# angeladai/sgnn

Measured on AMD Instinct MI355X. Metric: TSDF blocks/sec fwd+bwd (64^3@5% occ, bs32), higher is better.
Workload: dtype f32

## Files before the change

include/sgnn_hip.h:

```cpp
#ifndef SGNN_HIP_H
#define SGNN_HIP_H

#include <stdint.h>

#ifdef __cplusplus
extern "C" {
#endif

#define SGNN_OK 0
#define SGNN_EINVAL (-1)
#define SGNN_EHIP (-2)
#define SGNN_EOVERFLOW (-3)
#define SGNN_ENOWS (-4)

#define SGNN_STATUS_COORD_RANGE 1
#define SGNN_STATUS_DUPLICATE 2
#define SGNN_STATUS_OVERFLOW 4

typedef void *sgnn_stream_t;

const char *sgnn_last_error(void);
int sgnn_version(void);
const char *sgnn_arch(void);


int64_t sgnn_hash_capacity(int64_t n);

int sgnn_coords_from_i64(const int64_t *locs, int64_t n, int32_t *coords, int32_t *status,
                         const int64_t *n_dev, sgnn_stream_t stream);
int sgnn_coords_to_i64(const int32_t *coords, int64_t n, int64_t *locs, const int64_t *n_dev,
                       sgnn_stream_t stream);

int sgnn_hash_build(const int32_t *coords, int64_t n, uint64_t *keys, int32_t *vals, int64_t cap,
                    int32_t *status, const int64_t *n_dev, sgnn_stream_t stream);

int sgnn_hash_lookup(const uint64_t *keys, const int32_t *vals, int64_t cap, const int32_t *query,
                     int64_t m, int32_t *rows, const int64_t *m_dev, sgnn_stream_t stream);

#define SGNN_TUNE_UNKNOWN INT64_MIN
typedef struct sgnn_tune {
  int64_t conv_small;
  int64_t conv_small_rows;
  int64_t conv_unrolled;
  int64_t conv_one_round;
  int64_t conv_wide_epi;
  int64_t conv_dw_blocks;
  int64_t conv_dw_c1;
  int64_t rulebook_multi;
  int64_t scan_inline;
  int64_t chain_merged;
  int64_t prog_fusion;
  int64_t prog_lin_bn;
  int64_t prog_lin_add;
  int64_t bn_fuse;
} sgnn_tune;
int64_t sgnn_tune_set(const char *name, int64_t value);
int64_t sgnn_tune_get(const char *name);
const char *sgnn_tune_names(void);
const sgnn_tune *sgnn_tune_current(void);


int sgnn_rulebook_subm3(const uint64_t *keys, const int32_t *vals, int64_t cap,
                        const int32_t *coords, int64_t n, int32_t *nbr, int64_t ld,
                        const int64_t *n_dev, sgnn_stream_t stream);

#define SGNN_RULEBOOK_MULTI_MAX 4
int sgnn_rulebook_subm3_multi(int count, const uint64_t *const *keys, const int32_t *const *vals, const int64_t *caps,
                              const int32_t *const *coords, const int64_t *ns, int32_t *const *nbrs, const int64_t *lds,
                              const int64_t *const *n_devs, sgnn_stream_t stream);

int sgnn_rulebook_subm3_dense(const uint64_t *keys, const int32_t *vals, int64_t cap, const int32_t *coords, int64_t n,
                              int dim_z, int dim_y, int dim_x, int32_t *volume, int64_t volume_entries, int32_t *nbr,
                              int64_t ld, const int64_t *n_dev, sgnn_stream_t stream);
int sgnn_rulebook_subm3_volume(const int32_t *coords, int64_t n, int dim_z, int dim_y, int dim_x, int32_t *volume,
                               int64_t volume_entries, int32_t *nbr, int64_t ld, const int64_t *n_dev, int32_t *status,
                               sgnn_stream_t stream);

int64_t sgnn_down2_ws_bytes(int64_t nf);
int sgnn_rulebook_down2(const int32_t *fine_coords, int64_t nf, uint64_t *ckeys, int32_t *cvals,
                        int64_t ccap, int32_t *parent, int32_t *coarse_coords, int64_t *n_coarse,
                        void *ws, int64_t ws_bytes, sgnn_stream_t stream);
int sgnn_down2_tables(const int32_t *fine_coords, const int32_t *parent, int64_t nf,
                      int32_t *children, int64_t ldc, int64_t nc, int32_t *ptable, int64_t ldf,
                      const int64_t *nf_dev, const int64_t *nc_dev, sgnn_stream_t stream);

int64_t sgnn_down2_chain_ws_bytes(int64_t cap);
int sgnn_down2_chain(const int32_t *fine_coords, int64_t n0, const int64_t *n0_dev, int64_t cap, int depth,
                     void *const *ckeys, void *const *cvals, int64_t ccap, void *const *parent,
                     void *const *coarse_coords, int64_t *counts_dev, const int64_t *level_caps, int32_t *status,
                     void *ws, int64_t ws_bytes, sgnn_stream_t stream);

int64_t sgnn_down2_chain_tables_ws_bytes(int64_t cap, int depth);
int sgnn_down2_chain_tables(const int32_t *fine_coords, const int64_t *n0_dev, int64_t cap, int depth,
                            void *const *ckeys, void *const *cvals, int64_t ccap, void *const *parent,
                            void *const *coarse_coords, int64_t *counts_dev, const int64_t *level_caps,
                            void *const *children, void *const *ptable, int32_t *status, void *ws, int64_t ws_bytes,
                            sgnn_stream_t stream);

#define SGNN_CONV_TRANSPOSE_W 1
#define SGNN_CONV_FLIP_K 2
int sgnn_conv_fwd(const float *x, int64_t n_in, int cin, const float *w, int K, const int32_t *table,
                  int64_t ld, int64_t n_out, int cout, float *y, int flags, int in_shift,
                  sgnn_stream_t stream);

int sgnn_conv_fwd_ex(const float *x, int64_t n_in, int cin, const float *w, int K, const int32_t *table,
                     int64_t ld, int64_t n_out, int cout, float *y, int flags, int in_shift,
                     const int32_t *kmap, const int32_t *kadd, int in_mul, int groups, int table_rows,
                     sgnn_stream_t stream);
int sgnn_conv_bwd_weight_ex(const float *x, int64_t n_in, int cin, const float *dy, int cout,
                            const int32_t *table, int64_t ld, int K, int64_t n_out, float *dw, int in_shift,
                            const int32_t *kmap, const int32_t *kadd, int in_mul, int groups, int table_rows,
                            void *ws, int64_t ws_bytes, sgnn_stream_t stream);

int64_t sgnn_conv_stats_blocks(int64_t n_out);
int sgnn_conv_fwd_epi(const float *x, int64_t n_in, int cin, int64_t ldx, const float *w, int K,
                      const int32_t *table, int64_t ld, int64_t n_out, int cout, float *y, int64_t ldy, int flags,
                      const float *addend, int64_t ld_add, int stats, double *partial, const float *bn_x,
                      int64_t ld_bnx, const float *mean, const float *invstd, const float *gamma, const float *beta,
                      float leak, sgnn_stream_t stream);

int64_t sgnn_conv_bwd_weight_ws_bytes(int64_t n_out, int K, int cin, int cout);
int sgnn_conv_bwd_weight(const float *x, int64_t n_in, int cin, const float *dy, int cout,
                         const int32_t *table, int64_t ld, int K, int64_t n_out, float *dw, int in_shift, void *ws,
                         int64_t ws_bytes, sgnn_stream_t stream);

int sgnn_expand_weights(const float *w, int cin, int cout, float *wc, sgnn_stream_t stream);
int sgnn_expand_weights_bwd(const float *dwc, int cin, int cout, float *dw, sgnn_stream_t stream);

int64_t sgnn_bn_ws_bytes(int64_t n, int c);
int sgnn_bn_fwd(const float *x, int64_t n, int c, const float *gamma, const float *beta,
                float *running_mean, float *running_var, float eps, float momentum, int training,
                float leak, float *save_mean, float *save_invstd, float *y, void *ws,
                int64_t ws_bytes, sgnn_stream_t stream);
int sgnn_bn_bwd(const float *x, const float *dy, int64_t n, int c, const float *gamma,
                const float *beta, const float *save_mean, const float *save_invstd, int training,
                float leak, float *dx, float *dgamma, float *dbeta, void *ws, int64_t ws_bytes,
                sgnn_stream_t stream);
int sgnn_bn_bwd_add(const float *x, const float *dy, int64_t n, int c, const float *gamma, const float *beta,
                    const float *save_mean, const float *save_invstd, int training, float leak,
                    const float *addend, float *dx, float *dgamma, float *dbeta, void *ws, int64_t ws_bytes,
                    sgnn_stream_t stream);

int sgnn_bn_fwd_ex(const float *x, int64_t ldx, int64_t n, int c, const float *gamma, const float *beta,
                   float *running_mean, float *running_var, float eps, float momentum, int training, float leak,
                   float *save_mean, float *save_invstd, float *y, int64_t ldy, const double *pre_partial,
                   int64_t pre_nblk, void *ws, int64_t ws_bytes, sgnn_stream_t stream);
int sgnn_bn_bwd_ex(const float *x, int64_t ldx, const float *dy, int64_t ld_dy, int64_t n, int c, const float *gamma,
                   const float *beta, const float *save_mean, const float *save_invstd, int training, float leak,
                   const float *addend, int64_t ld_add, float *dx, int64_t ld_dx, float *dgamma, float *dbeta,
                   const double *pre_partial, int64_t pre_nblk, void *ws, int64_t ws_bytes, sgnn_stream_t stream);

int sgnn_copy_multi(void *const *dst, const void *const *src, const int64_t *bytes, int nregions, sgnn_stream_t stream);

int sgnn_gather_rows(const float *src, int c, const int32_t *idx, int64_t m, float *dst,
                     sgnn_stream_t stream);
int sgnn_gather_rows_dn(const float *src, int c, const int32_t *idx, const int64_t *m_dev, int64_t m_cap,
                        float *dst, sgnn_stream_t stream);
int sgnn_concat3_rows(const float *a, int ca, const int32_t *ia, const float *b, int cb, const int32_t *ib,
                      const float *c, int cc, const int32_t *ic, int64_t m, float *dst, sgnn_stream_t stream);
int sgnn_concat3_rows_bwd(const float *ddst, int ca, const int32_t *ia, int cb, const int32_t *ib, int cc,
                          const int32_t *ic, int64_t m, float *da, int64_t na, float *db, int64_t nb, float *dc,
                          int64_t nc, sgnn_stream_t stream);
int sgnn_scatter_rows(const float *src, int c, const int32_t *idx, int64_t m, float *dst,
                      int64_t n_dst, const int64_t *m_dev, sgnn_stream_t stream);
int sgnn_gather_sum(const float *src, int c, const int32_t *table, int64_t ld, int K,
                    int64_t n_out, float *dst, sgnn_stream_t stream);
int sgnn_repeat_rows(const float *src, int c, int64_t n, int rep, float *dst, sgnn_stream_t stream);
int sgnn_sum_groups(const float *src, int c, int64_t n, int rep, float *dst, sgnn_stream_t stream);
int sgnn_concat_rows(const float *a, int ca, const int32_t *ia, const float *b, int cb,
                     const int32_t *ib, int64_t m, float *dst, sgnn_stream_t stream);
int sgnn_concat_rows_bwd(const float *ddst, int ca, const int32_t *ia, int cb, const int32_t *ib,
                         int64_t m, float *da, int64_t na, float *db, int64_t nb,
                         sgnn_stream_t stream);
int sgnn_add(const float *a, const float *b, int64_t count, float *y, sgnn_stream_t stream);

int sgnn_expand8_coords(const int32_t *coords, int64_t n, int32_t *out, const int64_t *n_dev, sgnn_stream_t stream);
int sgnn_expand8_coords_i64(const int32_t *coords, int64_t n, int32_t *out, int64_t *locs, const int64_t *n_dev,
                            sgnn_stream_t stream);
int sgnn_dense_coords(int batch, int d0, int d1, int d2, int32_t *out, sgnn_stream_t stream);
int64_t sgnn_compact_ws_bytes(int64_t n);
int sgnn_compact_sigmoid(const float *logits, int64_t stride, int64_t n, int32_t *sel,
                         int64_t *count, void *ws, int64_t ws_bytes, sgnn_stream_t stream);
int sgnn_compact_dense(const int32_t *coords, int64_t n, const float *vol, int batch, int d0, int d1, int d2,
                       int32_t *sel, int64_t *count, void *ws, int64_t ws_bytes, sgnn_stream_t stream);
int sgnn_compact_mask(const uint8_t *mask, int64_t n, int32_t *sel, int64_t *count, void *ws,
                      int64_t ws_bytes, sgnn_stream_t stream);
int sgnn_compact_sigmoid_cap(const float *logits, int64_t stride, int64_t n, const int64_t *n_dev, int32_t *sel,
                             int64_t *count2, int64_t keep_cap, int32_t *status, void *ws, int64_t ws_bytes,
                             sgnn_stream_t stream);
int sgnn_compact_dense_cap(const int32_t *coords, int64_t n, const int64_t *n_dev, const float *vol, int batch, int d0,
                           int d1, int d2, int32_t *sel, int64_t *count2, int64_t keep_cap, int32_t *status, void *ws,
                           int64_t ws_bytes, sgnn_stream_t stream);
int sgnn_compact_sigmoid_cap_locs(const float *logits, int64_t stride, int64_t n, const int64_t *n_dev,
                                  const int32_t *coords, int32_t *sel, int32_t *locs, int64_t *count2, int64_t keep_cap,
                                  int32_t *status, void *ws, int64_t ws_bytes, sgnn_stream_t stream);
int sgnn_compact_dense_cap_locs(const int32_t *coords, int64_t n, const int64_t *n_dev, const float *vol, int batch, int d0,
                                int d1, int d2, int32_t *sel, int32_t *locs, int64_t *count2, int64_t keep_cap,
                                int32_t *status, void *ws, int64_t ws_bytes, sgnn_stream_t stream);

int sgnn_sparse_to_dense(const float *feats, const int32_t *coords, int64_t n, int c, float *dense,
                         int batch, int d0, int d1, int d2, sgnn_stream_t stream);
int sgnn_dense_to_sparse(const float *dense, const int32_t *coords, int64_t n, int c, float *feats,
                         int batch, int d0, int d1, int d2, sgnn_stream_t stream);

int64_t sgnn_linear_ws_bytes(int64_t n, int cin, int cout);
int sgnn_linear_fwd(const float *x, int64_t n, int cin, const float *w, const float *bias, int cout,
                    float *y, sgnn_stream_t stream);
int sgnn_linear_bwd(const float *x, const float *dy, int64_t n, int cin, const float *w, int cout,
                    float *dx, float *dw, float *dbias, void *ws, int64_t ws_bytes,
                    sgnn_stream_t stream);

int64_t sgnn_loss_ws_bytes(void);
int sgnn_loss_level_fwd(const int64_t *locs, const float *vals, int vstride, int occ_col, int sdf_col,
                        const float *tgt_occ, const float *tgt_sdf, const float *weights,
                        const uint8_t *known, int d0, int d1, int d2, int64_t m, int use_log,
                        int mask_mode, const int64_t *m_dev, double *sums, float *out2, void *ws, int64_t ws_bytes,
                        sgnn_stream_t stream);
int sgnn_loss_level_bwd(const int64_t *locs, const float *vals, int vstride, int occ_col, int sdf_col,
                        const float *tgt_occ, const float *tgt_sdf, const float *weights,
                        const uint8_t *known, int d0, int d1, int d2, int64_t m, int use_log,
                        int mask_mode, const int64_t *m_dev, const double *sums, const float *gout2, float *dvals,
                        sgnn_stream_t stream);

int sgnn_loss_targets(const float *sdf, const uint8_t *known, const int64_t *input_locs, int64_t n_locs,
                      const int64_t *n_locs_dev, int batch,
                      int d0, int d1, int d2, float trunc, int masking, float weight_missing_geo, int ncoarse,
                      void *const *hier_in, float *tsdf, float *hier_last, float *occ_last, float *w_last,
                      void *const *occ, void *const *w, void *const *hier, sgnn_stream_t stream);
int sgnn_loss_combine(const float *out2s, const float *coef_host, int n, float *total, float *cur,
                      sgnn_stream_t stream);
int sgnn_loss_combine_bwd(const float *g, const float *coef_host, int n, float *g2, sgnn_stream_t stream);
int64_t sgnn_loss_multi_ws_bytes(void);
int sgnn_loss_levels_fwd(const int64_t *levels, int n, const float *coef_host, double *sums, float *out2s, float *total,
                         float *cur, void *ws, int64_t ws_bytes, sgnn_stream_t stream);
int sgnn_loss_levels_bwd(const int64_t *levels, int n, const float *coef_host, const double *sums, const float *g,
                         void *const *dvals, sgnn_stream_t stream);

int64_t sgnn_prog_arena_floats(const int32_t *ops, int nops, const int32_t *bufs, int nbuf, int n_ext,
                               const int64_t *lev_n, int nlev, const int32_t *keep, int mode);
int64_t sgnn_prog_ws_bytes(const int32_t *ops, int nops, const int64_t *lev_n, int nlev);
int64_t sgnn_prog_buffer_offset(const int32_t *ops, int nops, const int32_t *bufs, int nbuf, int n_ext,
                                const int64_t *lev_n, int nlev, const int32_t *keep, int infer, int b);
int sgnn_prog_plan(const int32_t *ops, int nops, const int32_t *bufs, int nbuf, int n_ext, const int64_t *lev_n,
                   int nlev, const int32_t *keep, int mode, int32_t *out);
int sgnn_prog_forward(const int32_t *ops, const float *opf, int nops, const int32_t *bufs, int nbuf, int n_ext,
                      const int64_t *lev_n, const int64_t *lev_ld, void *const *lev_nbr,
                      void *const *lev_children, void *const *lev_ptable, void *const *lev_parent,
                      void *const *lev_cnt, int nlev, void *const *params, int nparams,
                      void *const *ext, void *const *idx, int nidx,
                      float *arena, int64_t arena_floats, const int32_t *keep, int training, void *wait_event,
                      void *ws, int64_t ws_bytes, sgnn_stream_t stream);
int sgnn_prog_backward(const int32_t *ops, const float *opf, int nops, const int32_t *bufs, int nbuf, int n_ext,
                       const int64_t *lev_n, const int64_t *lev_ld, void *const *lev_nbr,
                       void *const *lev_children, void *const *lev_ptable, void *const *lev_parent,
                       void *const *lev_cnt, int nlev, void *const *params, void *const *pgrads,
                       int nparams, void *const *ext,
                       void *const *gext, void *const *idx, int nidx, const float *arena, float *garena,
                       int64_t arena_floats, void *const *gout, const int32_t *keep, int training, void *ws,
                       int64_t ws_bytes, sgnn_stream_t stream);

int sgnn_prog_set_side_stream(sgnn_stream_t stream2, void *ws2, int64_t ws2_bytes);
int sgnn_prog_defer_join(int on);
int64_t sgnn_bf16_conv_ws_bytes(int cin, int cout, int K, int expand);
int sgnn_bf16_conv_fwd(const void *x, int64_t n_in, int cin, int64_t ldx, const float *w, int K, const int32_t *table,
                       int64_t ld, int64_t n_out, int cout, void *y, int64_t ldy, const void *addend, int64_t ld_add,
                       const int64_t *n_dev, void *ws, int64_t ws_bytes, sgnn_stream_t stream);
int sgnn_bf16_conv_expand(const void *x, int64_t n, int cin, int64_t ldx, const float *w, const int32_t *nbr, int64_t ld,
                          int cout, void *y, int64_t ldy, const int64_t *n_dev, void *ws, int64_t ws_bytes,
                          sgnn_stream_t stream);
int sgnn_bf16_bn_eval(const void *x, int64_t ldx, int64_t n, int c, const float *gamma, const float *beta,
                      const float *running_mean, const float *running_var, float eps, float leak, void *y, int64_t ldy,
                      const int64_t *n_dev, sgnn_stream_t stream);
int sgnn_bf16_gather_rows(const void *x, int64_t ldx, int c, const int32_t *idx, int64_t m, void *y, int64_t ldy,
                          const int64_t *n_dev, sgnn_stream_t stream);
int sgnn_bf16_add(const void *a, int64_t lda, const void *b, int64_t ldb, int64_t n, int c, void *y, int64_t ldy,
                  const int64_t *n_dev, sgnn_stream_t stream);
int sgnn_bf16_join(const void *a, int64_t lda, int ca, const void *b, int64_t ldb, int cb, int64_t n, void *y, int64_t ldy,
                   const int64_t *n_dev, sgnn_stream_t stream);
int sgnn_bf16_concat3(const float *a, int ca, const int32_t *ia, const float *b, int cb, const int32_t *ib, const float *c,
                      int cc, const int32_t *ic, int64_t m, void *y, int64_t ldy, const int64_t *n_dev, sgnn_stream_t stream);
int sgnn_bf16_linear(const void *x, int64_t ldx, int64_t n, int cin, const float *w, const float *bias, int cout, float *y,
                     const int64_t *n_dev, sgnn_stream_t stream);
int sgnn_bf16_to_f32(const void *x, int64_t ldx, int64_t n, int c, float *y, const int64_t *n_dev, sgnn_stream_t stream);
int sgnn_adam_flat(float *params, const float *grads, float *exp_avg, float *exp_avg_sq, int64_t n, const int64_t *seg,
                   int nseg, const float *lr_dev, float beta1, float beta2, float eps, float weight_decay,
                   float grad_scale, const int32_t *status, sgnn_stream_t stream);
int sgnn_seg_flags(const int64_t *cnt_ptrs, int nseg, float *flags, const int32_t *status, sgnn_stream_t stream);
int sgnn_status_merge(const float *overflow_flag, int32_t *status, sgnn_stream_t stream);

int sgnn_io_layout(const void *bytes, int64_t nbytes, int kind, int64_t *out);
int sgnn_io_flag_entries(const uint32_t *locs_xyz, const float *vals, const float *voxelsize,
                         const int64_t *seg, int nb, int64_t n, float truncation, int64_t max_z,
                         uint8_t *mask, sgnn_stream_t stream);
int sgnn_io_emit_entries(const uint32_t *locs_xyz, const float *vals, const float *voxelsize,
                         const int64_t *seg, int nb, const int32_t *sel, const int64_t *count,
                         int64_t n_max, int64_t *out_locs, float *out_feats, sgnn_stream_t stream);
int sgnn_io_scatter_dense(const uint32_t *locs_xyz, const float *vals, const float *voxelsize,
                          const int64_t *seg, int nb, int64_t n, int d0, int d1, int d2, int64_t max_z,
                          float *dense, sgnn_stream_t stream);

typedef struct sgnn_fuse_frame {
  float m[12];
  float intr[4];
  int32_t box[6];
  int64_t offset;
} sgnn_fuse_frame;
int sgnn_fuse_depth_raw(const uint16_t *raw, int nframes, int h_raw, int w_raw, int h, int w, float depth_shift,
                        float min_depth, float max_depth, float *out, sgnn_stream_t stream);
int sgnn_fuse_bilateral(const float *in, int nframes, int h, int w, float sigma_d, float sigma_r, float *out,
                        sgnn_stream_t stream);
int sgnn_fuse_integrate(float *sdf, uint8_t *weight, int32_t *free_ctr, int dx, int dy, int dz, const float *depth,
                        int h, int w, const sgnn_fuse_frame *frames, int nframes, int chunk, float voxel_size,
                        float depth_min, float depth_max, const float *obb, sgnn_stream_t stream);
int sgnn_fuse_flag(const float *sdf, int dx, int dy, int dz, float keep_abs, float truncation, float voxel_size,
                   int64_t max_z, uint8_t *mask, sgnn_stream_t stream);
int sgnn_fuse_emit_block(const float *sdf, int dx, int dy, const int32_t *sel, const int64_t *count, int64_t n_max,
                         uint32_t *locs_xyz, float *vals, sgnn_stream_t stream);
int sgnn_fuse_emit_rows(const float *sdf, int dx, int dy, float voxel_size, const int32_t *sel, const int64_t *count,
                        int64_t n_max, int64_t *locs, float *feats, sgnn_stream_t stream);
int sgnn_fuse_known(const float *sdf, int64_t n, float voxel_size, uint8_t *known, sgnn_stream_t stream);

int sgnn_chunk_score(const float *sdf_target, const float *sdf_input, int dx, int dy, int dz, float voxel_size,
                     float truncation, float keep_abs, int cz, int cy, int cx, int sz, int sy, int sx, int nwz, int nwy,
                     int nwx, int32_t *bricks, int32_t *table, sgnn_stream_t stream);
int sgnn_chunk_flag(const float *sdf, int dx, int dy, int dz, const int32_t *origins, int nb, int cz, int cy, int cx,
                    float keep_abs, float truncation, float voxel_size, uint8_t *mask, sgnn_stream_t stream);
int sgnn_chunk_emit_rows(const float *sdf, int dx, int dy, int dz, const int32_t *origins, int nb, int cz, int cy,
                         int cx, float voxel_size, const int32_t *sel, const int64_t *count, int64_t n_max,
                         int64_t *locs, float *feats, sgnn_stream_t stream);
int sgnn_chunk_crop(const float *sdf, int dx, int dy, int dz, const int32_t *origins, int nb, int cz, int cy, int cx,
                    int shift, float keep_abs, float voxel_size, float *out, uint8_t *known, sgnn_stream_t stream);

typedef struct sgnn_render_frame {
  float m[12];
  float intr[4];
} sgnn_render_frame;
int sgnn_render_depth(const float *verts, int nverts, const int32_t *faces, int ntri, const sgnn_render_frame *frames,
                      int nframes, int chunk, int h, int w, float z_clip, float depth_min, float depth_max,
                      int wave_pixels, float *out, int32_t *status, int64_t *counters, sgnn_stream_t stream);

int sgnn_meshdist_pack(const float *verts, int nverts, const int32_t *faces, int ntri, float *records, float *boxes,
                       uint8_t *usable, int32_t *status, sgnn_stream_t stream);
int sgnn_meshdist_count(const float *boxes, int ntri, float lox, float loy, float loz, float cell, int nx, int ny,
                        int nz, int32_t *counts, sgnn_stream_t stream);
int sgnn_meshdist_fill(const float *boxes, int ntri, float lox, float loy, float loz, float cell, int nx, int ny,
                       int nz, const int32_t *offsets, int32_t *cursor, int32_t *refs, sgnn_stream_t stream);
int sgnn_meshdist_query(const float *points, int64_t npts, const float *records, const int32_t *offsets,
                        const int32_t *refs, float lox, float loy, float loz, float hix, float hiy, float hiz,
                        float cell, int nx, int ny, int nz, float max_dist, float *dist, int32_t *face,
                        int64_t *counters, sgnn_stream_t stream);
int sgnn_mesh_sample(const float *records, const double *cum, int ntri, int last_usable, int64_t n, int64_t seed,
                     float *pts, int32_t *fid, sgnn_stream_t stream);

int sgnn_iou_counts(const int64_t *locs, const uint8_t *keep, const float *logits, int64_t lstride, int64_t m,
                    const void *tgt, int tgt_is_u8, int nb, int d0, int d1, int d2, int use_mask,
                    int64_t *counters, sgnn_stream_t stream);
int64_t sgnn_l1_tgtsurf_ws_bytes(void);
// ... 42 lines not shown
```

sgnn_amd/csrc/bn.hip:

```cpp
#include "common.h"

#define BN_MAX_BLOCKS 2048
#define BN_FLUSH 2
#ifndef BN_U
#define BN_U 2
#endif
#define BN_FUSE_BLOCKS 4096
#define BN_FUSE_MAXC 64

struct BnGeom {
  int vec;
  int cq;
  int rpb;
};

static BnGeom bn_geom(int c) {
  BnGeom g;
  g.vec = (c % 4 == 0) ? 4 : 1;
  g.cq = c / g.vec;
  g.rpb = 256 / g.cq;
  if (g.rpb < 1) g.rpb = 1;
  return g;
}

static BnGeom bn_geom_scalar(int c) {
  BnGeom g;
  g.vec = 1;
  g.cq = c;
  g.rpb = 256 / c;
  if (g.rpb < 1) g.rpb = 1;
  return g;
}

static int bn_blocks(int64_t n, const BnGeom &g) {
  int64_t b = (n + (int64_t)g.rpb * BN_FLUSH - 1) / ((int64_t)g.rpb * BN_FLUSH);
  if (b < 1) b = 1;
  if (b > BN_MAX_BLOCKS) b = BN_MAX_BLOCKS;
  return (int)b;
}

SGNN_EXPORT int64_t sgnn_bn_ws_bytes(int64_t n, int c) {
  (void)n;
  return (int64_t)BN_MAX_BLOCKS * 2 * c * (int64_t)sizeof(double) + 4 * (int64_t)c * sizeof(float) + 256;
}

template <int VEC>
__device__ __forceinline__ void load_vec(const float *p, float (&v)[VEC]) {
  if constexpr (VEC == 4) {
    const float4 t = *reinterpret_cast<const float4 *>(p);
    v[0] = t.x; v[1] = t.y; v[2] = t.z; v[3] = t.w;
  } else {
    v[0] = *p;
  }
}
template <int VEC>
__device__ __forceinline__ void store_vec(float *p, const float (&v)[VEC]) {
  if constexpr (VEC == 4) {
    *reinterpret_cast<float4 *>(p) = make_float4(v[0], v[1], v[2], v[3]);
  } else {
    *p = v[0];
  }
}

template <int VEC, int MODE, bool LIN = false>
__global__ __launch_bounds__(256) void k_bn_partial(const float *__restrict__ x, int64_t ldx,
                                                   const float *__restrict__ dy, int64_t ld_dy, int64_t n, int c,
                                                   int cq, int rpb, const float *__restrict__ mean,
                                                   const float *__restrict__ invstd,
                                                   const float *__restrict__ gamma,
                                                   const float *__restrict__ beta, float leak,
                                                   double *__restrict__ partial, const int64_t *n_dev, BnLin lin) {
  extern __shared__ double sh[];
  const int tid = threadIdx.x;
  unsigned nblk = gridDim.x;
  if (n_dev) {
    n = sgnn_dyn_n(n, n_dev);
    int64_t b = (n + (int64_t)rpb * BN_FLUSH - 1) / ((int64_t)rpb * BN_FLUSH);
    if (b < 1) b = 1;
    if (b > BN_MAX_BLOCKS) b = BN_MAX_BLOCKS;
    if (b < (int64_t)nblk) nblk = (unsigned)b;
    if (blockIdx.x >= nblk) {
      for (int o = tid; o < 2 * c; o += 256) partial[(size_t)blockIdx.x * 2 * c + o] = 0.0;
      return;
    }
  }
  const int col = tid % cq, rloc = tid / cq;
  const bool active = rloc < rpb;
  double sa[VEC], sb[VEC];
#pragma unroll
  for (int v = 0; v < VEC; ++v) sa[v] = sb[v] = 0.0;
  float m_[VEC], is_[VEC], g_[VEC], b_[VEC];
  float lw[2][VEC];
  if constexpr (LIN) {
#pragma unroll
    for (int o = 0; o < 2; ++o)
#pragma unroll
      for (int v = 0; v < VEC; ++v) lw[o][v] = (active && o < lin.nout) ? lin.w[o][col * VEC + v] : 0.f;
  }
  if (MODE == 1 && active) {
#pragma unroll
    for (int v = 0; v < VEC; ++v) {
      m_[v] = mean[col * VEC + v];
      is_[v] = invstd[col * VEC + v];
      g_[v] = gamma ? gamma[col * VEC + v] : 1.f;
      b_[v] = beta ? beta[col * VEC + v] : 0.f;
    }
  }
  if (active) {
    const int64_t step = (int64_t)nblk * rpb;
    int64_t row = (int64_t)blockIdx.x * rpb + rloc;
    while (row < n) {
      float fa[VEC], fb[VEC];
#pragma unroll
      for (int v = 0; v < VEC; ++v) fa[v] = fb[v] = 0.f;
      float xv[BN_FLUSH][VEC], dv[BN_FLUSH][VEC];
      bool keep[BN_FLUSH];
#pragma unroll
      for (int it = 0; it < BN_FLUSH; ++it) {
        const int64_t rr = row + it * step;
        keep[it] = rr < n;
        const int64_t rc = rr < n ? rr : row;
        load_vec<VEC>(x + rc * ldx + col * VEC, xv[it]);
        if constexpr (LIN) {
#pragma unroll
          for (int v = 0; v < VEC; ++v) dv[it][v] = 0.f;
#pragma unroll
          for (int o = 0; o < 2; ++o)
            if (o < lin.nout) {
              const float gv = lin.g[rc * lin.ldg + o];
#pragma unroll
              for (int v = 0; v < VEC; ++v) dv[it][v] = fmaf(gv, lw[o][v], dv[it][v]);
            }
        } else if (MODE == 1) {
          load_vec<VEC>(dy + rc * ld_dy + col * VEC, dv[it]);
        }
      }
#pragma unroll
      for (int it = 0; it < BN_FLUSH; ++it) {
        if (MODE == 0) {
#pragma unroll
          for (int v = 0; v < VEC; ++v) {
            const float xm = keep[it] ? xv[it][v] : 0.f;
            fa[v] += xm;
            fb[v] = fmaf(xm, xm, fb[v]);
          }
        } else {
#pragma unroll
          for (int v = 0; v < VEC; ++v) {
            const float xh = (xv[it][v] - m_[v]) * is_[v];
            const float yv = fmaf(xh, g_[v], b_[v]);
            const float dz = keep[it] ? (yv > 0.f ? dv[it][v] : dv[it][v] * leak) : 0.f;
            fa[v] += dz;
            fb[v] = fmaf(dz, xh, fb[v]);
          }
        }
      }
      row += (int64_t)BN_FLUSH * step;
#pragma unroll
      for (int v = 0; v < VEC; ++v) {
        sa[v] += (double)fa[v];
        sb[v] += (double)fb[v];
      }
    }
  }
  double *mine = sh + ((size_t)rloc * cq + col) * 2 * VEC;
  if (active) {
#pragma unroll
    for (int v = 0; v < VEC; ++v) {
      mine[v] = sa[v];
      mine[VEC + v] = sb[v];
    }
  }
  __syncthreads();
  const int outs = cq * VEC * 2;
  for (int o = tid; o < outs; o += 256) {
    const int which = o / (cq * VEC);
    const int ch = o % (cq * VEC);
    const int cg = ch / VEC, v = ch % VEC;
    double s = 0.0;
    for (int rr = 0; rr < rpb; ++rr) s += sh[((size_t)rr * cq + cg) * 2 * VEC + which * VEC + v];
    partial[((size_t)blockIdx.x * 2 + which) * c + ch] = s;
  }
}

__device__ __forceinline__ void bn_reduce_channel(const double *__restrict__ partial, int nblk, int c, int ch,
                                                  double *sh, double &s, double &s2) {
  double a = 0.0, b = 0.0;
  for (int blk = threadIdx.x; blk < nblk; blk += 8 * 256) {
    double va[8], vb[8];
#pragma unroll
    for (int u = 0; u < 8; ++u) {
      const int bi = blk + u * 256;
      const bool ok = bi < nblk;
      va[u] = ok ? partial[((size_t)bi * 2 + 0) * c + ch] : 0.0;
      vb[u] = ok ? partial[((size_t)bi * 2 + 1) * c + ch] : 0.0;
    }
#pragma unroll
    for (int u = 0; u < 8; ++u) {
      a += va[u];
      b += vb[u];
    }
  }
  sh[threadIdx.x] = a;
  sh[256 + threadIdx.x] = b;
  __syncthreads();
  for (int d = 128; d > 0; d >>= 1) {
    if (threadIdx.x < d) {
      sh[threadIdx.x] += sh[threadIdx.x + d];
      sh[256 + threadIdx.x] += sh[256 + threadIdx.x + d];
    }
    __syncthreads();
  }
  s = sh[0];
  s2 = sh[256];
}

__global__ __launch_bounds__(256) void k_bn_finalize_fwd(const double *__restrict__ partial, int nblk,
                                                        int64_t n, int c, float eps, float momentum,
                                                        float *__restrict__ running_mean,
                                                        float *__restrict__ running_var,
                                                        float *__restrict__ save_mean,
                                                        float *__restrict__ save_invstd, const int64_t *n_dev) {
  __shared__ double sh[512];
  n = sgnn_dyn_n(n, n_dev);
  const int ch = blockIdx.x;
  double s, s2;
  bn_reduce_channel(partial, nblk, c, ch, sh, s, s2);
  if (threadIdx.x == 0) {
    if (n <= 0) {
      save_mean[ch] = 0.f;
      save_invstd[ch] = 0.f;
      return;
    }
    const double mean = s / (double)n;
    double var = s2 / (double)n - mean * mean;
    if (var < 0.0) var = 0.0;
    save_mean[ch] = (float)mean;
    save_invstd[ch] = (float)(1.0 / sqrt(var + (double)eps));
    if (running_mean) running_mean[ch] = momentum * running_mean[ch] + (1.f - momentum) * (float)mean;
    if (running_var) {
      const double unb = var * ((double)n / (double)(n > 1 ? n - 1 : 1));
      running_var[ch] = momentum * running_var[ch] + (1.f - momentum) * (float)unb;
    }
  }
}

__global__ __launch_bounds__(256) void k_bn_eval_stats(const float *__restrict__ running_mean,
                                                      const float *__restrict__ running_var, int c, float eps,
                                                      float *__restrict__ save_mean,
                                                      float *__restrict__ save_invstd) {
  for (int ch = threadIdx.x; ch < c; ch += 256) {
    save_mean[ch] = running_mean[ch];
    save_invstd[ch] = 1.0f / sqrtf(running_var[ch] + eps);
  }
}


struct BnFuse {
  const double *partial;
  int nblk;
  float eps, momentum;
  float *running_mean, *running_var, *save_mean, *save_invstd;
  float *dgamma, *dbeta;
};

#ifndef BN_TOTALS_WIDE
#define BN_TOTALS_WIDE 1
#endif
typedef double f64x2 __attribute__((ext_vector_type(2)));
__device__ __forceinline__ void bn_fuse_totals(const BnFuse &f, int c, double *scratch, double *tot) {
  const int tid = threadIdx.x;
  const int tpc = 256 / c;
  if (BN_TOTALS_WIDE && (c & 1) == 0 && (((uintptr_t)f.partial) & 15) == 0) {
    const int hp = c >> 1;
    const int p2 = tid % hp, which = (tid / hp) & 1, part = tid / c;
    f64x2 acc = {0.0, 0.0};
    if (part < tpc) {
      constexpr int U = 32;
      for (int blk = part; blk < f.nblk; blk += U * tpc) {
        f64x2 v[U];
#pragma unroll
        for (int u = 0; u < U; ++u) {
          const int bi = blk + u * tpc;
          v[u] = bi < f.nblk ? *reinterpret_cast<const f64x2 *>(f.partial + ((size_t)bi * 2 + which) * c + 2 * p2) : f64x2{0.0, 0.0};
        }
#pragma unroll
        for (int u = 0; u < U; ++u) acc += v[u];
      }
      scratch[which * 256 + part * c + 2 * p2] = acc[0];
      scratch[which * 256 + part * c + 2 * p2 + 1] = acc[1];
    }
  } else {
    const int ch = tid % c, part = tid / c;
    double a = 0.0, b = 0.0;
    if (part < tpc) {
      for (int blk = part; blk < f.nblk; blk += 8 * tpc) {
        double va[8], vb[8];
#pragma unroll
        for (int u = 0; u < 8; ++u) {
          const int bi = blk + u * tpc;
          const bool ok = bi < f.nblk;
          va[u] = ok ? f.partial[((size_t)bi * 2 + 0) * c + ch] : 0.0;
          vb[u] = ok ? f.partial[((size_t)bi * 2 + 1) * c + ch] : 0.0;
        }
#pragma unroll
        for (int u = 0; u < 8; ++u) {
          a += va[u];
          b += vb[u];
        }
      }
      scratch[part * c + ch] = a;
      scratch[256 + part * c + ch] = b;
    }
  }
  __syncthreads();
  if (tid < c) {
    double s1 = 0.0, s2 = 0.0;
    for (int p = 0; p < tpc; ++p) {
      s1 += scratch[p * c + tid];
      s2 += scratch[256 + p * c + tid];
    }
    tot[tid] = s1;
    tot[c + tid] = s2;
  }
  __syncthreads();
}

template <int VEC, bool FUSE>
__global__ __launch_bounds__(256) void k_bn_apply(const float *__restrict__ x, int64_t ldx, int64_t n, int c, int cq,
                                                 int rpb, const float *__restrict__ mean,
                                                 const float *__restrict__ invstd,
                                                 const float *__restrict__ gamma,
                                                 const float *__restrict__ beta, float leak,
                                                 float *__restrict__ y, int64_t ldy, BnFuse fuse,
                                                 const int64_t *n_dev) {
  __shared__ float s_mean[BN_FUSE_MAXC], s_inv[BN_FUSE_MAXC];
  __shared__ double s_scratch[512], s_tot[2 * BN_FUSE_MAXC];
  n = sgnn_dyn_n(n, n_dev);
  if (n <= 0) return;
  if constexpr (FUSE) {
    bn_fuse_totals(fuse, c, s_scratch, s_tot);
    for (int ch = threadIdx.x; ch < c; ch += 256) {
      const double s1 = s_tot[ch], s2 = s_tot[c + ch];
      const double mu = s1 / (double)n;
      double var = s2 / (double)n - mu * mu;
      if (var < 0.0) var = 0.0;
      const float fm = (float)mu, fi = (float)(1.0 / sqrt(var + (double)fuse.eps));
      s_mean[ch] = fm;
      s_inv[ch] = fi;
      if (blockIdx.x == 0) {
        fuse.save_mean[ch] = fm;
        fuse.save_invstd[ch] = fi;
        if (fuse.running_mean) fuse.running_mean[ch] = fuse.momentum * fuse.running_mean[ch] + (1.f - fuse.momentum) * fm;
        if (fuse.running_var) {
          const double unb = var * ((double)n / (double)(n > 1 ? n - 1 : 1));
          fuse.running_var[ch] = fuse.momentum * fuse.running_var[ch] + (1.f - fuse.momentum) * (float)unb;
        }
      }
    }
    __syncthreads();
    mean = s_mean;
    invstd = s_inv;
  }
  const int tid = threadIdx.x;
  const int col = tid % cq, rloc = tid / cq;
  if (rloc >= rpb) return;
  float km[VEC], ki[VEC], kg[VEC], kb[VEC];
#pragma unroll
  for (int v = 0; v < VEC; ++v) {
    const int ch = col * VEC + v;
    km[v] = mean[ch];
    ki[v] = invstd[ch];
    kg[v] = gamma ? gamma[ch] : 1.f;
    kb[v] = beta ? beta[ch] : 0.f;
  }
  const int64_t step = (int64_t)gridDim.x * rpb;
  for (int64_t r0 = (int64_t)blockIdx.x * rpb + rloc; r0 < n; r0 += step * BN_U) {
    float xv[BN_U][VEC];
#pragma unroll
    for (int u = 0; u < BN_U; ++u) {
      const int64_t r = r0 + u * step;
      load_vec<VEC>(x + (r < n ? r : r0) * ldx + col * VEC, xv[u]);
    }
#pragma unroll
    for (int u = 0; u < BN_U; ++u) {
      const int64_t r = r0 + u * step;
      if (r >= n) break;
      float yv[VEC];
#pragma unroll
      for (int v = 0; v < VEC; ++v) yv[v] = sgnn_bn_act(xv[u][v], km[v], ki[v], kg[v], kb[v], leak);
      store_vec<VEC>(y + r * ldy + col * VEC, yv);
    }
  }
}

__global__ __launch_bounds__(256) void k_bn_finalize_bwd(const double *__restrict__ partial, int nblk,
                                                        int64_t n, int c, float *__restrict__ dgamma,
                                                        float *__restrict__ dbeta, float *__restrict__ coef,
                                                        const int64_t *n_dev) {
  __shared__ double sh[512];
  n = sgnn_dyn_n(n, n_dev);
  const int ch = blockIdx.x;
  double s, s2;
  bn_reduce_channel(partial, nblk, c, ch, sh, s, s2);
  if (threadIdx.x == 0) {
    if (dbeta) dbeta[ch] = (float)s;
    if (dgamma) dgamma[ch] = (float)s2;
    coef[ch] = n > 0 ? (float)(s / (double)n) : 0.f;
    coef[c + ch] = n > 0 ? (float)(s2 / (double)n) : 0.f;
  }
}

template <int VEC, bool LIN, bool FUSE>
__global__ __launch_bounds__(256) void k_bn_bwd_apply(const float *__restrict__ x, int64_t ldx,
                                                     const float *__restrict__ dy, int64_t ld_dy, int64_t n, int c,
                                                     int cq, int rpb, const float *__restrict__ mean,
                                                     const float *__restrict__ invstd,
                                                     const float *__restrict__ gamma,
                                                     const float *__restrict__ beta, float leak, int training,
                                                     const float *__restrict__ coef, float *dx, int64_t ld_dx,
                                                     BnFuse fuse, const float *addend, int64_t ld_add,
                                                     const int64_t *n_dev, BnLin lin) {
  __shared__ float s_coef[2 * BN_FUSE_MAXC];
  __shared__ double s_scratch[512], s_tot[2 * BN_FUSE_MAXC];
  n = sgnn_dyn_n(n, n_dev);
  if constexpr (FUSE) {
    bn_fuse_totals(fuse, c, s_scratch, s_tot);
    for (int ch = threadIdx.x; ch < c; ch += 256) {
      const double s1 = s_tot[ch], s2 = s_tot[c + ch];
      s_coef[ch] = n > 0 ? (float)(s1 / (double)n) : 0.f;
      s_coef[c + ch] = n > 0 ? (float)(s2 / (double)n) : 0.f;
      if (blockIdx.x == 0) {
        if (fuse.dbeta) fuse.dbeta[ch] = (float)s1;
        if (fuse.dgamma) fuse.dgamma[ch] = (float)s2;
      }
    }
    __syncthreads();
    coef = s_coef;
  }
  const int tid = threadIdx.x;
  const int col = tid % cq, rloc = tid / cq;
  if (rloc >= rpb) return;
  float km[VEC], ki[VEC], kg[VEC], kb[VEC], k4[VEC], k5[VEC];
#pragma unroll
  for (int v = 0; v < VEC; ++v) {
    const int ch = col * VEC + v;
    km[v] = mean[ch];
    ki[v] = invstd[ch];
    kg[v] = gamma ? gamma[ch] : 1.f;
    kb[v] = beta ? beta[ch] : 0.f;
    k4[v] = training ? coef[ch] : 0.f;
    k5[v] = training ? coef[c + ch] : 0.f;
  }
  float lw[2][VEC];
  if constexpr (LIN) {
#pragma unroll
    for (int o = 0; o < 2; ++o)
#pragma unroll
      for (int v = 0; v < VEC; ++v) lw[o][v] = o < lin.nout ? lin.w[o][col * VEC + v] : 0.f;
  }
  const int64_t step = (int64_t)gridDim.x * rpb;
  for (int64_t r0 = (int64_t)blockIdx.x * rpb + rloc; r0 < n; r0 += step * BN_U) {
    float xv[BN_U][VEC], dv[BN_U][VEC], av[BN_U][VEC];
#pragma unroll
    for (int u = 0; u < BN_U; ++u) {
      const int64_t r = r0 + u * step, rc = (r < n ? r : r0);
      load_vec<VEC>(x + rc * ldx + col * VEC, xv[u]);
      if constexpr (LIN) {
#pragma unroll
        for (int v = 0; v < VEC; ++v) dv[u][v] = 0.f;
#pragma unroll
        for (int o = 0; o < 2; ++o)
          if (o < lin.nout) {
            const float gv = lin.g[rc * lin.ldg + o];
#pragma unroll
            for (int v = 0; v < VEC; ++v) dv[u][v] = fmaf(gv, lw[o][v], dv[u][v]);
          }
      } else {
        load_vec<VEC>(dy + rc * ld_dy + col * VEC, dv[u]);
      }
      if (addend) load_vec<VEC>(addend + rc * ld_add + col * VEC, av[u]);
    }
#pragma unroll
    for (int u = 0; u < BN_U; ++u) {
      const int64_t r = r0 + u * step;
      if (r >= n) break;
      float ov[VEC];
#pragma unroll
      for (int v = 0; v < VEC; ++v) {
        const float xh = (xv[u][v] - km[v]) * ki[v];
        const float t = fmaf(xh, kg[v], kb[v]);
        const float dz = t > 0.f ? dv[u][v] : dv[u][v] * leak;
        float d = dz;
        if (training) d = dz - k4[v] - xh * k5[v];
        ov[v] = d * kg[v] * ki[v];
        if (addend) ov[v] += av[u][v];
      }
      store_vec<VEC>(dx + r * ld_dx + col * VEC, ov);
    }
  }
}

static bool bn_fuse_ok(int64_t nblk, int c, int apply_grid) {
  return c <= BN_FUSE_MAXC && nblk <= BN_FUSE_BLOCKS && nblk * (int64_t)apply_grid * 2 * c * (int64_t)sizeof(double) <= (48ll << 20);
}

static int bn_apply_grid(int64_t n, const BnGeom &g) {
  int64_t b = (n + (int64_t)g.rpb * BN_U - 1) / ((int64_t)g.rpb * BN_U);
  if (b < 1) b = 1;
  if (b > 4096) b = 4096;
  return (int)b;
}

int sgnn_bn_fwd_impl(const float *x, int64_t ldx, int64_t n, int c, const float *gamma, const float *beta,
                     float *running_mean, float *running_var, float eps, float momentum, int training, float leak,
                     float *save_mean, float *save_invstd, float *y, int64_t ldy, const double *pre_partial,
                     int64_t pre_nblk, void *ws, int64_t ws_bytes, sgnn_stream_t stream, const int64_t *n_dev) {
  hipStream_t s = (hipStream_t)stream;
  SGNN_CHECK_ARG(n >= 0 && c >= 1 && (c % 4 == 0 ? c <= 1024 : c <= 256) && save_mean && save_invstd);
  SGNN_CHECK_ARG(training || (running_mean && running_var));
  if (ldx <= 0) ldx = c;
  if (ldy <= 0) ldy = c;
  SGNN_CHECK_ARG(ldx >= c && ldy >= c);
  BnGeom g = bn_geom(c);
  if (g.vec == 4 && (ldx % 4 || ldy % 4 || ((uintptr_t)x & 15) || ((uintptr_t)y & 15))) g = bn_geom_scalar(c);
  if (g.cq > 256) {
    sgnn_set_error("sgnn_bn_fwd: %d channels need 16-byte aligned rows (row strides multiples of 4 floats)", c);
    return SGNN_EINVAL;
  }
  BnFuse fuse{nullptr, 0, 0.f, 0.f, nullptr, nullptr, nullptr, nullptr, nullptr, nullptr};
  if (training && n > 0) {
    SGNN_CHECK_ARG(x);
    const double *partial = pre_partial;
    int64_t nblk = pre_nblk;
    if (!partial) {
      if (!ws || ws_bytes < sgnn_bn_ws_bytes(n, c)) {
        sgnn_set_error("sgnn_bn_fwd: workspace too small");
        return SGNN_ENOWS;
      }
      nblk = bn_blocks(n, g);
      const size_t shbytes = (size_t)g.rpb * g.cq * 2 * g.vec * sizeof(double);
      if (g.vec == 4)
        SGNN_LAUNCH((k_bn_partial<4, 0>), dim3((unsigned)nblk), dim3(256), shbytes, s, x, ldx, nullptr, 0, n, c,
                           g.cq, g.rpb, nullptr, nullptr, nullptr, nullptr, 0.f, (double *)ws, n_dev, BnLin{});
      else
        SGNN_LAUNCH((k_bn_partial<1, 0>), dim3((unsigned)nblk), dim3(256), shbytes, s, x, ldx, nullptr, 0, n, c,
                           g.cq, g.rpb, nullptr, nullptr, nullptr, nullptr, 0.f, (double *)ws, n_dev, BnLin{});
      partial = (const double *)ws;
    }
    if (g_tune.bn_fuse && bn_fuse_ok(nblk, c, bn_apply_grid(n, g)))
      fuse = BnFuse{partial, (int)nblk, eps, momentum, running_mean, running_var, save_mean, save_invstd, nullptr, nullptr};
    else
      SGNN_LAUNCH(k_bn_finalize_fwd, dim3(c), dim3(256), 0, s, partial, (int)nblk, n, c, eps, momentum,
                         running_mean, running_var, save_mean, save_invstd, n_dev);
  } else if (training) {
    SGNN_HIP_TRY(hipMemsetAsync(save_mean, 0, c * sizeof(float), s));
    SGNN_HIP_TRY(hipMemsetAsync(save_invstd, 0, c * sizeof(float), s));
  } else {
    SGNN_LAUNCH(k_bn_eval_stats, dim3(1), dim3(256), 0, s, (const float *)running_mean,
                       (const float *)running_var, c, eps, save_mean, save_invstd);
  }
  if (n > 0) {
    SGNN_CHECK_ARG(x && y);
    const int grid = bn_apply_grid(n, g);
#define BN_APPLY(VECV, FUSEV)                                                                                 \
  SGNN_LAUNCH((k_bn_apply<VECV, FUSEV>), dim3(grid), dim3(256), 0, s, x, ldx, n, c, g.cq, g.rpb,              \
              (const float *)save_mean, (const float *)save_invstd, gamma, beta, leak, y, ldy, fuse, n_dev)
    if (g.vec == 4 && fuse.partial) BN_APPLY(4, true);
    else if (g.vec == 4) BN_APPLY(4, false);
    else if (fuse.partial) BN_APPLY(1, true);
    else BN_APPLY(1, false);
#undef BN_APPLY
  }
  SGNN_CHECK_LAUNCH();
  return SGNN_OK;
}

SGNN_EXPORT int sgnn_bn_fwd(const float *x, int64_t n, int c, const float *gamma, const float *beta,
                            float *running_mean, float *running_var, float eps, float momentum, int training,
                            float leak, float *save_mean, float *save_invstd, float *y, void *ws,
                            int64_t ws_bytes, sgnn_stream_t stream) {
  return sgnn_bn_fwd_impl(x, c, n, c, gamma, beta, running_mean, running_var, eps, momentum, training, leak, save_mean,
                          save_invstd, y, c, nullptr, 0, ws, ws_bytes, stream);
}

SGNN_EXPORT int sgnn_bn_fwd_ex(const float *x, int64_t ldx, int64_t n, int c, const float *gamma, const float *beta,
                               float *running_mean, float *running_var, float eps, float momentum, int training,
                               float leak, float *save_mean, float *save_invstd, float *y, int64_t ldy,
                               const double *pre_partial, int64_t pre_nblk, void *ws, int64_t ws_bytes,
                               sgnn_stream_t stream) {
  return sgnn_bn_fwd_impl(x, ldx, n, c, gamma, beta, running_mean, running_var, eps, momentum, training, leak,
                          save_mean, save_invstd, y, ldy, pre_partial, pre_nblk, ws, ws_bytes, stream);
}

SGNN_EXPORT int sgnn_bn_bwd(const float *x, const float *dy, int64_t n, int c, const float *gamma,
                            const float *beta, const float *save_mean, const float *save_invstd, int training,
                            float leak, float *dx, float *dgamma, float *dbeta, void *ws, int64_t ws_bytes,
                            sgnn_stream_t stream) {
  return sgnn_bn_bwd_impl(x, c, dy, c, n, c, gamma, beta, save_mean, save_invstd, training, leak, nullptr, c, dx, c,
                          dgamma, dbeta, nullptr, 0, ws, ws_bytes, stream);
}

SGNN_EXPORT int sgnn_bn_bwd_add(const float *x, const float *dy, int64_t n, int c, const float *gamma,
                                const float *beta, const float *save_mean, const float *save_invstd, int training,
                                float leak, const float *addend, float *dx, float *dgamma, float *dbeta, void *ws,
                                int64_t ws_bytes, sgnn_stream_t stream) {
  return sgnn_bn_bwd_impl(x, c, dy, c, n, c, gamma, beta, save_mean, save_invstd, training, leak, addend, c, dx, c,
                          dgamma, dbeta, nullptr, 0, ws, ws_bytes, stream);
}

SGNN_EXPORT int sgnn_bn_bwd_ex(const float *x, int64_t ldx, const float *dy, int64_t ld_dy, int64_t n, int c,
                               const float *gamma, const float *beta, const float *save_mean,
                               const float *save_invstd, int training, float leak, const float *addend,
                               int64_t ld_add, float *dx, int64_t ld_dx, float *dgamma, float *dbeta,
                               const double *pre_partial, int64_t pre_nblk, void *ws, int64_t ws_bytes,
                               sgnn_stream_t stream) {
  return sgnn_bn_bwd_impl(x, ldx, dy, ld_dy, n, c, gamma, beta, save_mean, save_invstd, training, leak, addend, ld_add,
                          dx, ld_dx, dgamma, dbeta, pre_partial, pre_nblk, ws, ws_bytes, stream);
}

int sgnn_bn_bwd_impl(const float *x, int64_t ldx, const float *dy, int64_t ld_dy, int64_t n, int c, const float *gamma,
                     const float *beta, const float *save_mean, const float *save_invstd, int training, float leak,
                     const float *addend, int64_t ld_add, float *dx, int64_t ld_dx, float *dgamma, float *dbeta,
                     const double *pre_partial, int64_t pre_nblk, void *ws, int64_t ws_bytes, sgnn_stream_t stream,
                     const int64_t *n_dev, const BnLin *lin) {
  hipStream_t s = (hipStream_t)stream;
  SGNN_CHECK_ARG(n >= 0 && c >= 1 && (c % 4 == 0 ? c <= 1024 : c <= 256) && save_mean && save_invstd);
  SGNN_CHECK_ARG(!lin || (lin->g && lin->nout >= 1 && lin->nout <= 2 && lin->w[0] && (lin->nout < 2 || lin->w[1]) && !pre_partial));
  if (n == 0) {
    if (dgamma) SGNN_HIP_TRY(hipMemsetAsync(dgamma, 0, c * sizeof(float), s));
    if (dbeta) SGNN_HIP_TRY(hipMemsetAsync(dbeta, 0, c * sizeof(float), s));
    return SGNN_OK;
  }
  SGNN_CHECK_ARG(x && (dy || lin) && dx);
  if (ldx <= 0) ldx = c;
  if (ld_dy <= 0) ld_dy = c;
  if (ld_dx <= 0) ld_dx = c;
  if (ld_add <= 0) ld_add = c;
  SGNN_CHECK_ARG(ldx >= c && ld_dy >= c && ld_dx >= c && ld_add >= c);
  if (!ws || ws_bytes < sgnn_bn_ws_bytes(n, c)) {
    sgnn_set_error("sgnn_bn_bwd: workspace too small");
    return SGNN_ENOWS;
  }
  BnGeom g = bn_geom(c);
  if (g.vec == 4 && (ldx % 4 || ld_dy % 4 || ld_dx % 4 || ld_add % 4 || ((uintptr_t)x & 15) || ((uintptr_t)dy & 15) ||
                     ((uintptr_t)dx & 15) || ((uintptr_t)addend & 15)))
    g = bn_geom_scalar(c);
  if (g.cq > 256) {
    sgnn_set_error("sgnn_bn_bwd: %d channels need 16-byte aligned rows (row strides multiples of 4 floats)", c);
    return SGNN_EINVAL;
  }
  const double *partial = pre_partial;
  int64_t nblk = pre_nblk;
  float *coef = (float *)((char *)ws + (size_t)BN_MAX_BLOCKS * 2 * c * sizeof(double));
  if (!partial) {
    nblk = bn_blocks(n, g);
    const size_t shbytes = (size_t)g.rpb * g.cq * 2 * g.vec * sizeof(double);
    if (lin && g.vec == 4)
      SGNN_LAUNCH((k_bn_partial<4, 1, true>), dim3((unsigned)nblk), dim3(256), shbytes, s, x, ldx, dy, ld_dy, n, c, g.cq,
                         g.rpb, save_mean, save_invstd, gamma, beta, leak, (double *)ws, n_dev, *lin);
    else if (lin)
      SGNN_LAUNCH((k_bn_partial<1, 1, true>), dim3((unsigned)nblk), dim3(256), shbytes, s, x, ldx, dy, ld_dy, n, c, g.cq,
                         g.rpb, save_mean, save_invstd, gamma, beta, leak, (double *)ws, n_dev, *lin);
    else if (g.vec == 4)
      SGNN_LAUNCH((k_bn_partial<4, 1>), dim3((unsigned)nblk), dim3(256), shbytes, s, x, ldx, dy, ld_dy, n, c, g.cq,
                         g.rpb, save_mean, save_invstd, gamma, beta, leak, (double *)ws, n_dev, BnLin{});
    else
      SGNN_LAUNCH((k_bn_partial<1, 1>), dim3((unsigned)nblk), dim3(256), shbytes, s, x, ldx, dy, ld_dy, n, c, g.cq,
                         g.rpb, save_mean, save_invstd, gamma, beta, leak, (double *)ws, n_dev, BnLin{});
    partial = (const double *)ws;
  }
  BnFuse fuse{nullptr, 0, 0.f, 0.f, nullptr, nullptr, nullptr, nullptr, nullptr, nullptr};
  if (g_tune.bn_fuse && bn_fuse_ok(nblk, c, bn_apply_grid(n, g)))
    fuse = BnFuse{partial, (int)nblk, 0.f, 0.f, nullptr, nullptr, nullptr, nullptr, dgamma, dbeta};
  else
    SGNN_LAUNCH(k_bn_finalize_bwd, dim3(c), dim3(256), 0, s, partial, (int)nblk, n, c, dgamma, dbeta, coef, n_dev);
  const int grid = bn_apply_grid(n, g);
#define BN_BWD_APPLY(VECV, LINV, FUSEV)                                                                                       \
  SGNN_LAUNCH((k_bn_bwd_apply<VECV, LINV, FUSEV>), dim3(grid), dim3(256), 0, s, x, ldx, dy, ld_dy, n, c, g.cq, g.rpb, save_mean, \
              save_invstd, gamma, beta, leak, training, (const float *)coef, dx, ld_dx, fuse, addend, ld_add, n_dev,              \
              LINV ? *lin : BnLin{})
  const bool fz = fuse.partial != nullptr;
  if (lin && g.vec == 4) { if (fz) BN_BWD_APPLY(4, true, true); else BN_BWD_APPLY(4, true, false); }
  else if (lin) { if (fz) BN_BWD_APPLY(1, true, true); else BN_BWD_APPLY(1, true, false); }
  else if (g.vec == 4) { if (fz) BN_BWD_APPLY(4, false, true); else BN_BWD_APPLY(4, false, false); }
  else { if (fz) BN_BWD_APPLY(1, false, true); else BN_BWD_APPLY(1, false, false); }
#undef BN_BWD_APPLY
  SGNN_CHECK_LAUNCH();
  return SGNN_OK;
}
```

sgnn_amd/csrc/common.h:

```cpp
#pragma once
#include <hip/hip_runtime.h>
#include <stdint.h>
#include <stdio.h>
#include "../../include/sgnn_hip.h"

#define SGNN_EXPORT extern "C" __attribute__((visibility("default")))

extern "C" int sgnn_stamp(const char *label, sgnn_stream_t stream);
extern sgnn_tune g_tune;

void sgnn_set_error(const char *fmt, ...);
int sgnn_prof_begin_launch(int kind, int64_t n_out, int cin, int cout, int K, int flags, hipStream_t s);
void sgnn_prof_end_launch(int slot, hipStream_t s);

__device__ __forceinline__ float sgnn_bn_act(float x, float mean, float invstd, float gamma, float beta, float leak) {
  const float xh = (x - mean) * invstd;
  const float t = fmaf(xh, gamma, beta);
  return t > 0.f ? t : t * leak;
}

struct ConvEpi {
  int64_t ldx, ldy, ld_add;
  const float *addend;
  int stats;
  double *partial;
  const float *bn_x;
  int64_t ld_bnx;
  const float *mean, *invstd, *gamma, *beta;
  float leak;
  const int64_t *n_dev;
};

int sgnn_conv_fwd_impl(const float *x, int64_t n_in, int cin, const float *w, int K, const int32_t *table, int64_t ld,
                       int64_t n_out, int cout, float *y, int flags, int in_shift, const int32_t *kmap,
                       const int32_t *kadd, int in_mul, int groups, int table_rows, const ConvEpi *epi,
                       sgnn_stream_t stream);
int64_t sgnn_conv_grid_blocks(int64_t n_out, int cin, int cout, int K);
struct BnLin {
  const float *g;
  int64_t ldg;
  const float *w[2];
  int nout;
};
int sgnn_bn_fwd_impl(const float *x, int64_t ldx, int64_t n, int c, const float *gamma, const float *beta,
                     float *running_mean, float *running_var, float eps, float momentum, int training, float leak,
                     float *save_mean, float *save_invstd, float *y, int64_t ldy, const double *pre_partial,
                     int64_t pre_nblk, void *ws, int64_t ws_bytes, sgnn_stream_t stream, const int64_t *n_dev = nullptr);
int sgnn_bn_bwd_impl(const float *x, int64_t ldx, const float *dy, int64_t ld_dy, int64_t n, int c, const float *gamma,
                     const float *beta, const float *save_mean, const float *save_invstd, int training, float leak,
                     const float *addend, int64_t ld_add, float *dx, int64_t ld_dx, float *dgamma, float *dbeta,
                     const double *pre_partial, int64_t pre_nblk, void *ws, int64_t ws_bytes, sgnn_stream_t stream,
                     const int64_t *n_dev = nullptr, const struct BnLin *lin = nullptr);
bool sgnn_conv_epi_supported(int cin, int cout);
bool dw_shape_ok(int cin, int cout);
#define DW_BATCH_MAX 28
struct DwDesc {
  const float *partial;
  float *dw;
  int64_t nblk, elems;
  int blk0;
};
struct DwBatch {
  DwDesc d[DW_BATCH_MAX];
  int n;
};
extern DwBatch *sgnn_dw_batch;
int sgnn_dw_batch_flush(DwBatch *b, hipStream_t s);
int sgnn_gather_rows_ld(const float *src, int64_t ld_src, int c, const int32_t *idx, int64_t m, float *dst,
                        int64_t ld_dst, sgnn_stream_t stream, const int64_t *n_dev = nullptr);
int sgnn_gather_sum_ld(const float *src, int64_t ld_src, int c, const int32_t *table, int64_t ld, int K, int64_t n_out,
                       float *dst, int64_t ld_dst, sgnn_stream_t stream, const int64_t *n_dev = nullptr);
int sgnn_add_ld(const float *a, int64_t lda, const float *b, int64_t ldb, int64_t n, int c, float *y, int64_t ldy,
                sgnn_stream_t stream, const int64_t *n_dev = nullptr);
int sgnn_fill32(void *p, uint32_t pattern, int64_t words, hipStream_t s);
int sgnn_fill32_multi(void *const *p, const int64_t *words, int nregions, uint32_t pattern, hipStream_t s);
int sgnn_copy_words(void *dst, const void *src, int64_t words, hipStream_t s);
int sgnn_sum_groups_dn(const float *src, int c, int64_t n, int rep, float *dst, sgnn_stream_t stream, const int64_t *n_dev);
int sgnn_concat_rows_dn(const float *a, int ca, const int32_t *ia, const float *b, int cb, const int32_t *ib, int64_t m,
                        float *dst, sgnn_stream_t stream, const int64_t *n_dev);
int sgnn_concat_rows_bwd_dn(const float *ddst, int ca, const int32_t *ia, int cb, const int32_t *ib, int64_t m, float *da,
                            int64_t na, float *db, int64_t nb, sgnn_stream_t stream, const int64_t *n_dev);
int sgnn_concat3_rows_dn(const float *a, int ca, const int32_t *ia, const float *b, int cb, const int32_t *ib,
                         const float *c, int cc, const int32_t *ic, int64_t m, float *dst, sgnn_stream_t stream,
                         const int64_t *n_dev);
int sgnn_concat3_rows_bwd_dn(const float *ddst, int ca, const int32_t *ia, int cb, const int32_t *ib, int cc,
                             const int32_t *ic, int64_t m, float *da, int64_t na, float *db, int64_t nb, float *dc,
                             int64_t nc, sgnn_stream_t stream, const int64_t *n_dev);
int sgnn_conv_bwd_weight_impl(const float *x, int64_t n_in, int cin, int64_t ldx, const float *dy, int cout, int64_t ld_dy,
                              const int32_t *table, int64_t ld, int K, int64_t n_out, float *dw, int in_shift,
                              const int32_t *kmap, const int32_t *kadd, int in_mul, int groups, int table_rows, void *ws,
                              int64_t ws_bytes, sgnn_stream_t stream, const int64_t *n_dev = nullptr);
int sgnn_expand_maps(const int32_t **S, const int32_t **ST, const int32_t **PAR);
int sgnn_linear_fwd_rows(const float *x, int64_t n, int cin, const float *const *w, const float *const *b, int cout,
                         float *y, sgnn_stream_t stream, const int64_t *n_dev = nullptr);
int sgnn_linear_bwd_rows(const float *x, const float *dy, int64_t n, int cin, const float *const *w, int cout,
                         float *dx, float *const *dw, float *const *db, void *ws, int64_t ws_bytes,
                         sgnn_stream_t stream, const int64_t *n_dev = nullptr, const float *addend = nullptr,
                         int64_t ld_add = 0);

extern long long sgnn_launch_counter;
#define SGNN_LAUNCH(...)           \
  do {                             \
    ++sgnn_launch_counter;         \
    hipLaunchKernelGGL(__VA_ARGS__); \
  } while (0)

#define SGNN_CHECK_ARG(cond)                                                    \
  do {                                                                          \
    if (!(cond)) {                                                              \
      sgnn_set_error("%s: invalid argument: %s", __func__, #cond);              \
      return SGNN_EINVAL;                                                       \
    }                                                                           \
  } while (0)

#define SGNN_CHECK_LAUNCH()                                                     \
  do {                                                                          \
    hipError_t e_ = hipGetLastError();                                          \
    if (e_ != hipSuccess) {                                                     \
      sgnn_set_error("%s: HIP error: %s", __func__, hipGetErrorString(e_));     \
      return SGNN_EHIP;                                                         \
    }                                                                           \
  } while (0)

#define SGNN_HIP_TRY(expr)                                                      \
  do {                                                                          \
    hipError_t e_ = (expr);                                                     \
    if (e_ != hipSuccess) {                                                     \
      sgnn_set_error("%s: %s failed: %s", __func__, #expr, hipGetErrorString(e_)); \
      return SGNN_EHIP;                                                         \
    }                                                                           \
  } while (0)

__device__ __forceinline__ int64_t sgnn_dyn_n(int64_t n_host, const int64_t *n_dev) {
  if (!n_dev) return n_host;
  const int64_t v = *n_dev;
  return v < n_host ? (v < 0 ? 0 : v) : n_host;
}

static inline int sgnn_grid_for(int64_t work, int block, int cap = 1 << 20) {
  int64_t g = (work + block - 1) / block;
  if (g < 1) g = 1;
  if (g > cap) g = cap;
  return (int)g;
}

__device__ __forceinline__ unsigned sgnn_xcd_tile(unsigned b, unsigned nwg) {
  const unsigned q = nwg >> 3, r = nwg & 7u, xcd = b & 7u, i = b >> 3;
  return (xcd < r ? xcd * (q + 1) : r * (q + 1) + (xcd - r) * q) + i;
}

#define SGNN_EMPTY_KEY 0xFFFFFFFFFFFFFFFFull

__device__ __forceinline__ uint64_t sgnn_pack_key(int z, int y, int x, int b) {
  return ((uint64_t)(uint32_t)b << 48) | ((uint64_t)(uint32_t)z << 32) | ((uint64_t)(uint32_t)y << 16) |
         (uint64_t)(uint32_t)x;
}

__device__ __forceinline__ uint64_t sgnn_hash64(uint64_t k) {
  k ^= k >> 33;
  k *= 0xff51afd7ed558ccdull;
  k ^= k >> 33;
  k *= 0xc4ceb9fe1a85ec53ull;
  k ^= k >> 33;
  return k;
}

__device__ __forceinline__ int32_t sgnn_hash_find(const uint64_t *__restrict__ keys,
                                                  const int32_t *__restrict__ vals, uint64_t mask,
                                                  uint64_t key) {
  uint64_t slot = sgnn_hash64(key) & mask;
  while (true) {
    uint64_t k = keys[slot];
    if (k == key) return vals[slot];
    if (k == SGNN_EMPTY_KEY) return -1;
    slot = (slot + 1) & mask;
  }
}

__device__ __forceinline__ uint8_t sgnn_known_code(float s, float vs) {
  if (s < -vs) {
    const float q = __fdiv_rn(-s, vs);
    return !(q < 2147483648.0f) ? 2 : (uint8_t)max(2, min(255, (int)q + 1));
  }
  return s <= vs ? 1 : 0;
}

__device__ __forceinline__ int sgnn_block_rank256(bool flag, int *lds4, int &total) {
  const int lane = threadIdx.x & 63, wave = threadIdx.x >> 6;
  unsigned long long bal = __ballot(flag);
  int prefix = __popcll(bal & ((1ull << lane) - 1ull));
  if (lane == 0) lds4[wave] = __popcll(bal);
  __syncthreads();
  int w0 = lds4[0], w1 = lds4[1], w2 = lds4[2], w3 = lds4[3];
  __syncthreads();
  int base = (wave > 0 ? w0 : 0) + (wave > 1 ? w1 : 0) + (wave > 2 ? w2 : 0);
  total = w0 + w1 + w2 + w3;
  return base + prefix;
}
```

sgnn_amd/csrc/conv.hip:

```cpp
#include <stdlib.h>
#include "common.h"

#include "conv_common.h"

#define CONV_SMALL_GRID ((int64_t)((g_tune.conv_small_rows + CONV_ROWS_PER_BLOCK - 1) / CONV_ROWS_PER_BLOCK))

template <int CIN, int COUT, int M, bool EX, bool WEPI>
__device__ __forceinline__ void conv_fwd_body(const float *__restrict__ x, int64_t n_in,
                                              const float *__restrict__ w, const int32_t *__restrict__ table,
                                              int64_t ld, int K, int64_t n_out, float *y, int flags,
                                              int in_shift, const ConvEx &ex, const ConvEpi &epi, int wg_cap) {
  using C = ConvCfg<CIN, COUT>;
  constexpr int V = C::V, CINP = C::CINP, NT = C::NT, KC = C::KC;
  constexpr int RPW = 16 * M;
  __shared__ __attribute__((aligned(16))) float wl[KC * C::PER_K];
  __shared__ double sred[4 * 2 * NT * 16];
  static_assert(!WEPI || (NT == 1 && M == 4 && !EX && COUT % 4 == 0), "wide epilogue: one column tile of whole 16-byte chunks");
  __shared__ float ecst[WEPI ? 64 : 1];

  const int tid = threadIdx.x, lane = tid & 63, wave = tid >> 6;
  const int r = lane & 15, q = lane >> 4;
  const unsigned groups = EX ? (unsigned)ex.groups : 1u;
  unsigned nwg = gridDim.x;
  if (epi.n_dev) n_out = sgnn_dyn_n(n_out, epi.n_dev);
  int J = 1;
  if constexpr (!EX) {
    if (wg_cap > 0) {
      const int64_t w1 = (n_out + 4 * RPW - 1) / (4 * RPW);
      J = (int)((w1 + wg_cap - 1) / wg_cap);
      if (J < 1) J = 1;
    }
  }
  if (epi.n_dev || J > 1) {
    const int64_t rows_wg = (int64_t)4 * RPW * J;
    nwg = (unsigned)((n_out + rows_wg - 1) / rows_wg) * groups;
    if (blockIdx.x >= nwg) {
      if (!EX && epi.stats)
        for (int o = tid; o < 2 * COUT; o += 256) epi.partial[(size_t)blockIdx.x * 2 * COUT + o] = 0.0;
      return;
    }
  }
  const unsigned lin = sgnn_xcd_tile(blockIdx.x, nwg);
  const unsigned tile = lin / groups, grp = lin % groups;
  int64_t row0 = ((int64_t)tile * J * 4 + wave) * RPW;
  const int32_t *kmap = nullptr, *kadd_g = nullptr;
  if constexpr (EX) {
    w += (int64_t)grp * K * CIN * COUT;
    kmap = ex.kmap ? ex.kmap + grp * K : nullptr;
    kadd_g = ex.kadd ? ex.kadd + grp * K : nullptr;
  }
  const int table_rows = EX ? ex.table_rows : K;
  const bool transpose = flags & SGNN_CONV_TRANSPOSE_W, flip = flags & SGNN_CONV_FLIP_K;

  const uint32_t ldx4 = (uint32_t)epi.ldx * 4u;
  const __amdgpu_buffer_rsrc_t rs_x = make_rsrc(x, (uint32_t)(((n_in - 1) * epi.ldx + CIN) * 4));
  const __amdgpu_buffer_rsrc_t rs_t = make_rsrc(table, (uint32_t)((int64_t)table_rows * ld * 4));
  uint32_t lane_off = (uint32_t)(row0 + (lane & (RPW - 1))) * 4u;
  const uint32_t ld4 = (uint32_t)ld * 4u;
  int perm[M];
#pragma unroll
  for (int m = 0; m < M; ++m) perm[m] = (m * 16 + r) * 4;

  f32x4 acc[M][NT];
  double s1[NT], s2[NT];
#pragma unroll
  for (int nt = 0; nt < NT; ++nt) s1[nt] = s2[nt] = 0.0;
  if constexpr (WEPI) conv_epi_wide_constants<COUT>(ecst, epi, epi.stats);

  auto load_idx = [&](int k) -> int32_t {
    if constexpr (EX) {
      const int trow = kmap ? kmap[k] : k;
      int32_t id = (int32_t)__builtin_amdgcn_raw_buffer_load_b32(rs_t, lane_off, trow * ld4, 0);
      return (id >> in_shift) * ex.in_mul + ((kadd_g && id >= 0) ? kadd_g[k] : 0);
    } else {
      return (int32_t)__builtin_amdgcn_raw_buffer_load_b32(rs_t, lane_off, k * ld4, 0) >> in_shift;
    }
  };
  auto gather = [&](int32_t iv, float(&a)[M][V]) {
#pragma unroll
    for (int m = 0; m < M; ++m) {
      const int32_t id = __builtin_amdgcn_ds_bpermute(perm[m], iv);
      buf_load_floats<V>(rs_x, (uint32_t)id * ldx4 + (uint32_t)(q * V * 4), a[m]);
    }
  };
  auto stage = [&](int k) {
    conv_stage_weights<CIN, COUT>(wl, w, K, k, (K - k) < KC ? (K - k) : KC, transpose, flip);
  };
  auto load_b = [&](int kk, float(&b)[NT][V]) {
#pragma unroll
    for (int nt = 0; nt < NT; ++nt) {
      const float *bp = wl + (kk * NT * 16 + nt * 16 + r) * CINP + q * V;
#pragma unroll
      for (int s = 0; s < V; ++s) b[nt][s] = bp[s];
    }
  };
  auto mma_b = [&](float(&a)[M][V], const float(&b)[NT][V]) {
    if constexpr (CINP != CIN) {
#pragma unroll
      for (int m = 0; m < M; ++m)
#pragma unroll
        for (int s = 0; s < V; ++s)
          if (3 * V + s >= CIN) a[m][s] = (q >= conv_first_pad_quarter<CIN, V>(s)) ? 0.f : a[m][s];
    }
#pragma unroll
    for (int s = 0; s < V; ++s)
#pragma unroll
      for (int m = 0; m < M; ++m)
#pragma unroll
        for (int nt = 0; nt < NT; ++nt)
          acc[m][nt] = __builtin_amdgcn_mfma_f32_16x16x4f32(a[m][s], b[nt][s], acc[m][nt], 0, 0, 0);
  };
  auto mma = [&](int kk, float(&a)[M][V]) {
    float b[NT][V];
    load_b(kk, b);
    mma_b(a, b);
  };

  const int klast = K - 1;
  auto idx_at = [&](int k) { return load_idx(k < klast ? k : klast); };
  for (int j = 0; j < J; ++j) {
  if (j > 0) {
    const int64_t wg_row0 = ((int64_t)tile * J + j) * 4 * RPW;
    if (wg_row0 >= n_out) break;
    row0 = wg_row0 + wave * RPW;
    lane_off = (uint32_t)(row0 + (lane & (RPW - 1))) * 4u;
  }
  const bool restage = j == 0 || K > KC;
  EpiRows<WEPI ? M : 1> erows;
#pragma unroll
  for (int m = 0; m < M; ++m)
#pragma unroll
    for (int nt = 0; nt < NT; ++nt) acc[m][nt] = f32x4{0.f, 0.f, 0.f, 0.f};
  if constexpr (V <= 4 && (NT >= 2 || M == 1)) {
    float a0[M][V], a1[M][V], a2[M][V];
    for (int k0 = 0; k0 < K; k0 += KC) {
      const int kc = (K - k0) < KC ? (K - k0) : KC;
      if (restage) stage(k0);
      gather(idx_at(k0), a0);
      gather(idx_at(k0 + 1), a1);
      int32_t iv2 = idx_at(k0 + 2), iv3 = idx_at(k0 + 3), iv4 = idx_at(k0 + 4);
      int kk = 0;
      for (; kk + 2 < kc; kk += 3) {
        gather(iv2, a2);
        iv2 = idx_at(k0 + kk + 5);
        __builtin_amdgcn_sched_barrier(0);
        mma(kk, a0);
        __builtin_amdgcn_sched_barrier(0);
        gather(iv3, a0);
        iv3 = idx_at(k0 + kk + 6);
        __builtin_amdgcn_sched_barrier(0);
        mma(kk + 1, a1);
        __builtin_amdgcn_sched_barrier(0);
        gather(iv4, a1);
        iv4 = idx_at(k0 + kk + 7);
        __builtin_amdgcn_sched_barrier(0);
        mma(kk + 2, a2);
        __builtin_amdgcn_sched_barrier(0);
      }
      if (kk < kc) mma(kk, a0);
      if (kk + 1 < kc) mma(kk + 1, a1);
    }
  } else {
    float a0[M][V], a1[M][V], b0[NT][V], b1[NT][V];
    for (int k0 = 0; k0 < (WEPI ? 1 : K); k0 += KC) {
      const int kc = (K - k0) < KC ? (K - k0) : KC;
      if (restage) stage(k0);
      int32_t iv1 = idx_at(k0 + 1), iv2 = idx_at(k0 + 2);
      gather(idx_at(k0), a0);
      load_b(0, b0);
      int kk = 0;
      for (; kk + 1 < kc; kk += 2) {
        gather(iv1, a1);
        const int32_t iv3 = idx_at(k0 + kk + 3);
        load_b(kk + 1, b1);
        __builtin_amdgcn_sched_barrier(0);
        mma_b(a0, b0);
        __builtin_amdgcn_sched_barrier(0);
        gather(iv2, a0);
        iv1 = iv3;
        iv2 = idx_at(k0 + kk + 4);
        load_b(kk + 2 < kc ? kk + 2 : kc - 1, b0);
        __builtin_amdgcn_sched_barrier(0);
        mma_b(a1, b1);
        __builtin_amdgcn_sched_barrier(0);
      }
      if constexpr (WEPI) {
        __builtin_amdgcn_sched_barrier(0);
        if constexpr (SGNN_WEPI_EARLY != 0) conv_epi_wide_prefetch<COUT, M>(erows, row0, n_out, epi, epi.stats, x, SGNN_WEPI_EARLY);
        __builtin_amdgcn_sched_barrier(0);
      }
      if (kk < kc) mma_b(a0, b0);
    }
  }

  if constexpr (WEPI)
    conv_epi_wide_finish<COUT, M>(acc, erows, row0, n_out, y, epi, epi.stats, ecst, s1, s2, x);
  else
    conv_epilogue_rows<COUT, M, NT>(acc, row0, n_out, groups, grp, y, epi, EX ? 0 : epi.stats, x, s1, s2);
  }
  conv_epilogue_stats<COUT, NT>(s1, s2, epi, EX ? 0 : epi.stats, sred, blockIdx.x);
}

template <int CIN, int COUT, int M, bool EX>
__global__ __launch_bounds__(256) void k_conv_fwd(const float *__restrict__ x, int64_t n_in,
                                                 const float *__restrict__ w, const int32_t *__restrict__ table,
                                                 int64_t ld, int K, int64_t n_out, float *y, int flags,
                                                 int in_shift, ConvEx ex, ConvEpi epi, int wg_cap) {
  conv_fwd_body<CIN, COUT, M, EX, false>(x, n_in, w, table, ld, K, n_out, y, flags, in_shift, ex, epi, wg_cap);
}

template <int CIN, int COUT>
__global__ __launch_bounds__(256) __attribute__((amdgpu_waves_per_eu(4, 8))) void k_conv_fwd_w(
    const float *__restrict__ x, int64_t n_in, const float *__restrict__ w, const int32_t *__restrict__ table, int64_t ld,
    int K, int64_t n_out, float *y, int flags, int in_shift, ConvEx ex, ConvEpi epi, int wg_cap) {
  conv_fwd_body<CIN, COUT, CONV_MREP, false, true>(x, n_in, w, table, ld, K, n_out, y, flags, in_shift, ex, epi, wg_cap);
}

template <int CIN, int COUT>
__global__ __launch_bounds__(256) void k_conv_small(const float *__restrict__ x, int64_t n_in,
                                                   const float *__restrict__ w, const int32_t *__restrict__ table,
                                                   int64_t ld, int K, int64_t n_out, float *y, int flags, int in_shift,
                                                   ConvEpi epi) {
  using C = ConvCfg<CIN, COUT>;
  constexpr int V = C::V, CINP = C::CINP, NT = C::NT;
  constexpr int KW = 7;
  __shared__ float red[4][NT * 256];
  __shared__ double sred[4][2][NT * 16];
  const int tid = threadIdx.x, lane = tid & 63, wave = tid >> 6;
  const int r = lane & 15, q = lane >> 4;
  const int64_t row0 = (int64_t)blockIdx.x * 16;
  if (epi.n_dev) {
    n_out = sgnn_dyn_n(n_out, epi.n_dev);
    if (row0 >= n_out) {
      if (epi.stats)
        for (int o = tid; o < 2 * COUT; o += 256) epi.partial[(size_t)blockIdx.x * 2 * COUT + o] = 0.0;
      return;
    }
  }
  const bool transpose = flags & SGNN_CONV_TRANSPOSE_W, flip = flags & SGNN_CONV_FLIP_K;
  const int per = (K + 3) >> 2;
  const int k0 = wave * per;
  const int nk = (K - k0) < per ? ((K - k0) > 0 ? (K - k0) : 0) : per;

  const uint32_t ldx4 = (uint32_t)epi.ldx * 4u, ldy4 = (uint32_t)epi.ldy * 4u;
  const __amdgpu_buffer_rsrc_t rs_x = make_rsrc(x, (uint32_t)(((n_in - 1) * epi.ldx + CIN) * 4));
  const __amdgpu_buffer_rsrc_t rs_t = make_rsrc(table, (uint32_t)((int64_t)K * ld * 4));
  const __amdgpu_buffer_rsrc_t rs_y = make_rsrc(y, (uint32_t)(((n_out - 1) * epi.ldy + COUT) * 4));
  const uint32_t lane_off = (uint32_t)(row0 + r) * 4u;
  const uint32_t ld4 = (uint32_t)ld * 4u;

  int32_t id[KW];
#pragma unroll
  for (int kk = 0; kk < KW; ++kk) {
    const int k = k0 + (kk < nk ? kk : (nk > 0 ? nk - 1 : 0));
    id[kk] = (int32_t)__builtin_amdgcn_raw_buffer_load_b32(rs_t, lane_off, (k < K ? k : K - 1) * ld4, 0) >> in_shift;
  }
  float a[KW][V];
#pragma unroll
  for (int kk = 0; kk < KW; ++kk) buf_load_floats<V>(rs_x, (uint32_t)id[kk] * ldx4 + (uint32_t)(q * V * 4), a[kk]);
  float b[KW][NT][V];
  if (transpose) {
    const __amdgpu_buffer_rsrc_t rs_w = make_rsrc(w, (uint32_t)((int64_t)K * CIN * COUT * 4));
#pragma unroll
    for (int kk = 0; kk < KW; ++kk) {
      const int k = k0 + kk;
      const int ks = flip ? (K - 1 - k) : k;
#pragma unroll
      for (int nt = 0; nt < NT; ++nt) {
        const int n = nt * 16 + r;
        const bool okw = kk < nk && n < COUT;
        buf_load_floats<V>(rs_w, okw ? (uint32_t)((ks * COUT + n) * CIN + q * V) * 4u : 0xFFFFF800u, b[kk][nt]);
        if constexpr (CINP != CIN) {
#pragma unroll
          for (int s = 0; s < V; ++s)
            if (3 * V + s >= CIN) b[kk][nt][s] = (q >= conv_first_pad_quarter<CIN, V>(s)) ? 0.f : b[kk][nt][s];
        }
      }
    }
  } else if constexpr (V == 4 && CIN <= 16 && (CIN * COUT) % 4 == 0) {
    constexpr int SL = CIN * COUT, G4 = SL / 4, NL = (G4 + 63) / 64;
    static_assert(SL <= NT * 256, "the weight slice must fit the wave's partial-tile buffer");
    float *ws = red[wave];
    const __amdgpu_buffer_rsrc_t rs_w = make_rsrc(w, (uint32_t)((int64_t)K * SL * 4));
    float g[KW][NL][4];
#pragma unroll
    for (int kk = 0; kk < KW; ++kk) {
      const int k = k0 + kk;
      const int ks = flip ? (K - 1 - k) : k;
#pragma unroll
      for (int l = 0; l < NL; ++l) {
        const int e4 = l * 64 + lane;
        buf_load_floats<4>(rs_w, (kk < nk && e4 < G4) ? (uint32_t)(ks * SL + e4 * 4) * 4u : 0xFFFFF800u, g[kk][l]);
      }
    }
    auto wave_sync = [] {
      __builtin_amdgcn_fence(__ATOMIC_RELEASE, "wavefront");
      __builtin_amdgcn_wave_barrier();
      __builtin_amdgcn_fence(__ATOMIC_ACQUIRE, "wavefront");
    };
#pragma unroll
    for (int kk = 0; kk < KW; ++kk) {
      wave_sync();
#pragma unroll
      for (int l = 0; l < NL; ++l) {
        const int e4 = l * 64 + lane;
        if (e4 < G4) {
#pragma unroll
          for (int j = 0; j < 4; ++j) ws[e4 * 4 + j] = g[kk][l][j];
        }
      }
      wave_sync();
#pragma unroll
      for (int nt = 0; nt < NT; ++nt) {
        const int n = nt * 16 + r;
#pragma unroll
        for (int s = 0; s < V; ++s) {
          const int c = q * V + s;
          b[kk][nt][s] = (c < CIN && n < COUT) ? ws[c * COUT + n] : 0.f;
        }
      }
    }
  } else {
#pragma unroll
    for (int kk = 0; kk < KW; ++kk) {
      const int k = k0 + kk;
      const int ks = flip ? (K - 1 - k) : k;
#pragma unroll
      for (int nt = 0; nt < NT; ++nt) {
        const int n = nt * 16 + r;
#pragma unroll
        for (int s = 0; s < V; ++s) {
          const int c = q * V + s;
          float v = 0.f;
          if (kk < nk && c < CIN && n < COUT) v = w[((int64_t)ks * CIN + c) * COUT + n];
          b[kk][nt][s] = v;
        }
      }
    }
  }
  if constexpr (CINP != CIN) {
#pragma unroll
    for (int kk = 0; kk < KW; ++kk)
#pragma unroll
      for (int s = 0; s < V; ++s)
        if (3 * V + s >= CIN) a[kk][s] = (q >= conv_first_pad_quarter<CIN, V>(s)) ? 0.f : a[kk][s];
  }
  f32x4 acc[2][NT];
#pragma unroll
  for (int h = 0; h < 2; ++h)
#pragma unroll
    for (int nt = 0; nt < NT; ++nt) acc[h][nt] = f32x4{0.f, 0.f, 0.f, 0.f};
#pragma unroll
  for (int kk = 0; kk < KW; ++kk) {
    if (kk < nk) {
#pragma unroll
      for (int s = 0; s < V; ++s)
#pragma unroll
        for (int nt = 0; nt < NT; ++nt)
          acc[kk & 1][nt] = __builtin_amdgcn_mfma_f32_16x16x4f32(a[kk][s], b[kk][nt][s], acc[kk & 1][nt], 0, 0, 0);
    }
  }
#pragma unroll
  for (int nt = 0; nt < NT; ++nt)
#pragma unroll
    for (int i = 0; i < 4; ++i) red[wave][nt * 256 + (q * 4 + i) * 16 + r] = acc[0][nt][i] + acc[1][nt][i];
  __syncthreads();

  const bool has_add = epi.addend != nullptr;
  const __amdgpu_buffer_rsrc_t rs_a =
      make_rsrc(has_add ? epi.addend : x, has_add ? (uint32_t)(((n_out - 1) * epi.ld_add + COUT) * 4) : 0u);
  const uint32_t lda4 = (uint32_t)epi.ld_add * 4u;
  const int stats = epi.stats;
  const __amdgpu_buffer_rsrc_t rs_b =
      make_rsrc(stats == 2 ? epi.bn_x : x, stats == 2 ? (uint32_t)(((n_out - 1) * epi.ld_bnx + COUT) * 4) : 0u);
  const uint32_t ldb4 = (uint32_t)epi.ld_bnx * 4u;
  const int orow_l = tid >> 4, ocol_l = tid & 15;
  const int64_t row = row0 + orow_l;
#pragma unroll
  for (int nt = 0; nt < NT; ++nt) {
    const int col = nt * 16 + ocol_l;
    const bool ok = col < COUT && row < n_out;
    const int e = nt * 256 + orow_l * 16 + ocol_l;
    float v = (red[0][e] + red[1][e]) + (red[2][e] + red[3][e]);
    const uint32_t orow = (uint32_t)row;
    if (has_add) v += __uint_as_float(__builtin_amdgcn_raw_buffer_load_b32(rs_a, ok ? orow * lda4 + col * 4u : 0xFFFFFFFFu, 0, 0));
    __builtin_amdgcn_raw_buffer_store_b32(__float_as_uint(v), rs_y, ok ? orow * ldy4 + col * 4u : 0xFFFFFFFFu, 0, 0);
    if (stats) {
      double f1 = 0.0, f2 = 0.0;
      if (stats == 1) {
        f1 = ok ? (double)v : 0.0;
        f2 = f1 * f1;
      } else {
        float cm = 0.f, ci = 0.f, cg = 1.f, cb = 0.f;
        if (col < COUT) {
          cm = epi.mean[col];
          ci = epi.invstd[col];
          cg = epi.gamma ? epi.gamma[col] : 1.f;
          cb = epi.beta ? epi.beta[col] : 0.f;
        }
        const float xb = __uint_as_float(__builtin_amdgcn_raw_buffer_load_b32(rs_b, ok ? orow * ldb4 + col * 4u : 0xFFFFFFFFu, 0, 0));
        const float xh = (xb - cm) * ci;
        const float t = fmaf(xh, cg, cb);
        const float dz = ok ? (t > 0.f ? v : v * epi.leak) : 0.f;
        f1 = (double)dz;
        f2 = (double)dz * (double)xh;
      }
      f1 += __shfl_xor(f1, 16); f2 += __shfl_xor(f2, 16);
      f1 += __shfl_xor(f1, 32); f2 += __shfl_xor(f2, 32);
      if (lane < 16) {
        sred[wave][0][nt * 16 + lane] = f1;
        sred[wave][1][nt * 16 + lane] = f2;
      }
    }
  }
  if (stats) {
    __syncthreads();
    for (int o = tid; o < 2 * NT * 16; o += 256) {
      const int which = o / (NT * 16), col = o % (NT * 16);
      if (col < COUT)
        epi.partial[((size_t)blockIdx.x * 2 + which) * COUT + col] =
            (sred[0][which][col] + sred[1][which][col]) + (sred[2][which][col] + sred[3][which][col]);
    }
  }
}

__global__ __launch_bounds__(256) void k_conv_fwd_generic(const float *__restrict__ x, int cin,
                                                         const float *__restrict__ w, int K,
                                                         const int32_t *__restrict__ table, int64_t ld,
                                                         int64_t n_out, int cout, float *__restrict__ y,
                                                         int flags, int in_shift, ConvEx ex, const int64_t *n_dev) {
  n_out = sgnn_dyn_n(n_out, n_dev);
  const int64_t t = (int64_t)blockIdx.x * 256 + threadIdx.x;
  if (t >= n_out * ex.groups * cout) return;
  const int64_t orow = t / cout;
  const int n = (int)(t - orow * cout);
  const int64_t row = orow / ex.groups;
  const int grp = (int)(orow - row * ex.groups);
  w += (int64_t)grp * K * cin * cout;
  const bool transpose = flags & SGNN_CONV_TRANSPOSE_W, flip = flags & SGNN_CONV_FLIP_K;
  float acc = 0.f;
  for (int k = 0; k < K; ++k) {
    const int32_t idx = table[(int64_t)(ex.kmap ? ex.kmap[grp * K + k] : k) * ld + row];
    if (idx < 0) continue;
    const float *xr = x + ((int64_t)(idx >> in_shift) * ex.in_mul + (ex.kadd ? ex.kadd[grp * K + k] : 0)) * cin;
    const int ks = flip ? (K - 1 - k) : k;
    for (int c = 0; c < cin; ++c) {
      const float wv = transpose ? w[((int64_t)ks * cout + n) * cin + c] : w[((int64_t)ks * cin + c) * cout + n];
      acc = fmaf(xr[c], wv, acc);
    }
  }
  y[t] = acc;
}

#define CONV_EX_CASES(X) \
  X(48, 16) X(16, 48) X(24, 8) X(8, 24) X(16, 24) X(24, 16) X(24, 32) X(32, 24) X(64, 32) X(32, 64) X(56, 28) X(28, 56)

#define CONV_FWD_CASES(X) \
  X(1, 8) X(8, 8) X(8, 12) X(12, 12) X(12, 16) X(16, 16) X(34, 16) X(30, 16) X(26, 16) X(48, 16) \
  X(8, 1) X(12, 8) X(16, 12) X(16, 34) X(16, 30) X(16, 26) X(16, 48) X(32, 16) X(16, 32) X(4, 16) X(16, 4) \
  X(16, 24) X(24, 16) X(24, 32) X(32, 24) X(64, 32) X(32, 64) X(56, 28) X(28, 56) X(32, 32) X(28, 16) X(16, 28)

int64_t sgnn_conv_grid_blocks(int64_t n_out, int cin, int cout, int K) {
  const int64_t grid4 = (n_out + CONV_ROWS_PER_BLOCK - 1) / CONV_ROWS_PER_BLOCK;
  if (grid4 < CONV_SMALL_GRID) return (n_out + 15) / 16;
  return grid4;
}


bool sgnn_conv_u_supported(int cin, int cout, int K);
bool sgnn_conv_u_launch(const float *x, int64_t n_in, int cin, const float *w, int K, const int32_t *table, int64_t ld,
                        int64_t n_out, int cout, float *y, int flags, int in_shift, const ConvEpi &epi, hipStream_t s);

bool conv_wide_epi_ok(const ConvEpi &epi, const float *y, int K) {
  if (!g_tune.conv_wide_epi || K > 27 || (epi.ldy & 3) || ((uintptr_t)y & 15)) return false;
  if (epi.addend && ((epi.ld_add & 3) || ((uintptr_t)epi.addend & 15))) return false;
  if (epi.stats == 2 && ((epi.ld_bnx & 3) || ((uintptr_t)epi.bn_x & 15))) return false;
  return true;
}
template <int CI, int CO, bool EXV>
static void conv_launch_big(unsigned grid4, hipStream_t s, const float *x, int64_t n_in, const float *w, const int32_t *table,
                            int64_t ld, int K, int64_t n_out, float *y, int flags, int in_shift, const ConvEx &ex,
                            const ConvEpi &epi) {
  if constexpr (!EXV && CO % 4 == 0 && CO <= 16 && CI <= 16) {
    static_assert(ConvCfg<CI, CO>::KC >= 27, "one weight chunk holds a 3x3x3 filter");
    if (conv_wide_epi_ok(epi, y, K)) {
      SGNN_LAUNCH((k_conv_fwd_w<CI, CO>), dim3(grid4), dim3(256), 0, s, x, n_in, w, table, ld, K, n_out, y, flags, in_shift,
                  ex, epi, !g_tune.conv_one_round ? 0 : conv_wg_capacity<k_conv_fwd_w<CI, CO>>());
      return;
    }
  }
  SGNN_LAUNCH((k_conv_fwd<CI, CO, CONV_MREP, EXV>), dim3(grid4), dim3(256), 0, s, x, n_in, w, table, ld, K, n_out, y,
              flags, in_shift, ex, epi,
              (EXV || !g_tune.conv_one_round) ? 0 : conv_wg_capacity<k_conv_fwd<CI, CO, CONV_MREP, EXV>>());
}

bool sgnn_conv_epi_supported(int cin, int cout) {
#define X(CI, CO) \
  if (cin == CI && cout == CO) return true;
  CONV_FWD_CASES(X)
#undef X
  return false;
}

int sgnn_conv_fwd_impl(const float *x, int64_t n_in, int cin, const float *w, int K, const int32_t *table, int64_t ld,
                       int64_t n_out, int cout, float *y, int flags, int in_shift, const int32_t *kmap,
                       const int32_t *kadd, int in_mul, int groups, int table_rows, const ConvEpi *epi_in,
                       sgnn_stream_t stream) {
  SGNN_CHECK_ARG(cin >= 1 && cout >= 1 && K >= 1 && K <= 64 && n_out >= 0 && ld >= n_out && in_shift >= 0 &&
                 in_shift < 31 && in_mul >= 1 && groups >= 1 && groups <= 64 && table_rows >= 1 &&
                 table_rows <= 64 && (kmap || table_rows >= K));
  if (n_out == 0) return SGNN_OK;
  SGNN_CHECK_ARG(x && w && table && y && n_in >= 1);
  SGNN_CHECK_ARG(ld % CONV_ROWS_PER_BLOCK == 0);
  ConvEpi epi{};
  if (epi_in) epi = *epi_in;
  if (epi.ldx <= 0) epi.ldx = cin;
  if (epi.ldy <= 0) epi.ldy = cout;
  if (epi.ld_add <= 0) epi.ld_add = cout;
  if (epi.ld_bnx <= 0) epi.ld_bnx = cout;
  const bool plain = !kmap && !kadd && in_mul == 1 && groups == 1 && table_rows == K;
  const bool has_epi = epi.ldx != cin || epi.ldy != cout || epi.addend || epi.stats;
  SGNN_CHECK_ARG(epi.ldx >= cin && epi.ldx <= 1024 && epi.ldy >= cout && epi.ldy <= 1024 && epi.ld_add >= cout &&
                 epi.ld_add <= 1024 && epi.ld_bnx >= cout && epi.ld_bnx <= 1024);
  SGNN_CHECK_ARG(epi.stats >= 0 && epi.stats <= 2 && (!epi.stats || (plain && epi.partial)));
  SGNN_CHECK_ARG(epi.stats != 2 || (epi.bn_x && epi.mean && epi.invstd));
  SGNN_CHECK_ARG(!epi.stats || K <= 28);
  const int64_t lmax = epi.ldy > epi.ld_add ? (epi.ldy > epi.ld_bnx ? epi.ldy : epi.ld_bnx)
                                            : (epi.ld_add > epi.ld_bnx ? epi.ld_add : epi.ld_bnx);
  if (n_in * epi.ldx * 4 > 0xFFFFF000ll || n_out * groups * lmax * 4 > 0xFFFFF000ll ||
      (int64_t)table_rows * ld * 4 > 0xFFFFF000ll) {
    sgnn_set_error("sgnn_conv_fwd: a slab exceeds the 4 GiB raw-buffer window (n_in=%lld cin=%d n_out=%lld cout=%d)",
                   (long long)n_in, cin, (long long)n_out, cout);
    return SGNN_EOVERFLOW;
  }
  hipStream_t s = (hipStream_t)stream;
  const ConvEx ex{kmap, kadd, in_mul, groups, table_rows};
  const unsigned grid4 = (unsigned)((n_out + CONV_ROWS_PER_BLOCK - 1) / CONV_ROWS_PER_BLOCK) * (unsigned)groups;
  const unsigned grid1 = (unsigned)((n_out + 63) / 64) * (unsigned)groups;
  const bool small = grid4 < CONV_SMALL_GRID;
  bool done = false;
  const int prof = sgnn_prof_begin_launch(0, n_out * groups, cin, cout, K, flags, s);
#define LAUNCH_FWD(CI, CO, EXV)                                                                         \
  do {                                                                                                  \
    if (small && !EXV && K <= 28 && (g_tune.conv_small || epi.stats))                                      \
      SGNN_LAUNCH((k_conv_small<CI, CO>), dim3((unsigned)((n_out + 15) / 16)), dim3(256), 0, s,         \
                         x, n_in, w, table, ld, K, n_out, y, flags, in_shift, epi);                     \
    else if (small)                                                                                     \
      SGNN_LAUNCH((k_conv_fwd<CI, CO, 1, EXV>), dim3(grid1), dim3(256), 0, s, x, n_in, w, table,        \
                         ld, K, n_out, y, flags, in_shift, ex, epi, 0);                                 \
    else                                                                                                \
      conv_launch_big<CI, CO, EXV>(grid4, s, x, n_in, w, table, ld, K, n_out, y, flags, in_shift, ex, epi); \
    done = true;                                                                                        \
  } while (0)
  if (plain && !small && g_tune.conv_unrolled && sgnn_conv_u_supported(cin, cout, K))
    done = sgnn_conv_u_launch(x, n_in, cin, w, K, table, ld, n_out, cout, y, flags, in_shift, epi, s);
#define X(CI, CO) \
  if (!done && plain && cin == CI && cout == CO) LAUNCH_FWD(CI, CO, false);
  CONV_FWD_CASES(X)
#undef X
#define X(CI, CO) \
  if (!done && !plain && cin == CI && cout == CO) LAUNCH_FWD(CI, CO, true);
  CONV_EX_CASES(X)
#undef X
  if (!done) {
    if (has_epi) {
      sgnn_set_error("sgnn_conv_fwd_epi: strided / fused epilogues need one of the compiled (cin, cout) shapes, got (%d, %d)", cin, cout);
      return SGNN_EINVAL;
    }
    const int64_t total = n_out * groups * cout;
    SGNN_LAUNCH(k_conv_fwd_generic, dim3((unsigned)((total + 255) / 256)), dim3(256), 0, s, x, cin, w, K,
                       table, ld, n_out, cout, y, flags, in_shift, ex, epi.n_dev);
  }
  sgnn_prof_end_launch(prof, s);
  SGNN_CHECK_LAUNCH();
  return SGNN_OK;
}

SGNN_EXPORT int sgnn_conv_fwd_ex(const float *x, int64_t n_in, int cin, const float *w, int K, const int32_t *table,
                                 int64_t ld, int64_t n_out, int cout, float *y, int flags, int in_shift,
                                 const int32_t *kmap, const int32_t *kadd, int in_mul, int groups,
                                 int table_rows, sgnn_stream_t stream) {
  return sgnn_conv_fwd_impl(x, n_in, cin, w, K, table, ld, n_out, cout, y, flags, in_shift, kmap, kadd, in_mul,
                            groups, table_rows, nullptr, stream);
}

SGNN_EXPORT int sgnn_conv_fwd(const float *x, int64_t n_in, int cin, const float *w, int K, const int32_t *table,
                              int64_t ld, int64_t n_out, int cout, float *y, int flags, int in_shift,
                              sgnn_stream_t stream) {
  return sgnn_conv_fwd_impl(x, n_in, cin, w, K, table, ld, n_out, cout, y, flags, in_shift, nullptr, nullptr, 1, 1,
                            K, nullptr, stream);
}

SGNN_EXPORT int64_t sgnn_conv_stats_blocks(int64_t n_out) { return n_out > 0 ? sgnn_conv_grid_blocks(n_out, 0, 0, 0) : 0; }

SGNN_EXPORT int sgnn_conv_fwd_epi(const float *x, int64_t n_in, int cin, int64_t ldx, const float *w, int K,
                                  const int32_t *table, int64_t ld, int64_t n_out, int cout, float *y, int64_t ldy,
                                  int flags, const float *addend, int64_t ld_add, int stats, double *partial,
                                  const float *bn_x, int64_t ld_bnx, const float *mean, const float *invstd,
                                  const float *gamma, const float *beta, float leak, sgnn_stream_t stream) {
  ConvEpi epi{ldx, ldy, ld_add, addend, stats, partial, bn_x, ld_bnx, mean, invstd, gamma, beta, leak, nullptr};
  return sgnn_conv_fwd_impl(x, n_in, cin, w, K, table, ld, n_out, cout, y, flags, 0, nullptr, nullptr, 1, 1, K, &epi,
                            stream);
}

__device__ int32_t g_expand_maps[192];

int sgnn_expand_maps(const int32_t **S, const int32_t **ST, const int32_t **PAR) {
  static const int32_t *base = nullptr;
  if (!base) {
    int32_t host[192];
    for (int g = 0; g < 8; ++g)
      for (int i = 0; i < 8; ++i) {
        const int o0 = ((i >> 2) & 1) - 1 + ((g >> 2) & 1), o1 = ((i >> 1) & 1) - 1 + ((g >> 1) & 1),
                  o2 = (i & 1) - 1 + (g & 1);
        const int srow = (o0 + 1) * 9 + (o1 + 1) * 3 + (o2 + 1);
        host[g * 8 + i] = srow;
        host[64 + g * 8 + i] = 26 - srow;
        host[128 + g * 8 + i] = g;
      }
    SGNN_HIP_TRY(hipMemcpyToSymbol(HIP_SYMBOL(g_expand_maps), host, sizeof(host)));
    void *p = nullptr;
    SGNN_HIP_TRY(hipGetSymbolAddress(&p, HIP_SYMBOL(g_expand_maps)));
    base = (const int32_t *)p;
  }
  *S = base;
  *ST = base + 64;
  *PAR = base + 128;
  return SGNN_OK;
}

__device__ __forceinline__ void axis_taps(int j, int i, int &lo, int &hi) {
  if (j == 0) { lo = i ? 0 : -1; hi = i ? 1 : -1; }
  else        { lo = i ? 1 : -1; hi = i ? 1 : 0; }
}

__global__ __launch_bounds__(256) void k_expand_weights(const float *__restrict__ w, int cc, float *__restrict__ wc) {
  const int t = blockIdx.x * 256 + threadIdx.x;
  if (t >= 64 * cc) return;
  const int gi = t / cc, e = t - gi * cc, g = gi >> 3, i = gi & 7;
  int l0, h0, l1, h1, l2, h2;
  axis_taps((g >> 2) & 1, (i >> 2) & 1, l0, h0);
  axis_taps((g >> 1) & 1, (i >> 1) & 1, l1, h1);
  axis_taps(g & 1, i & 1, l2, h2);
  float acc = 0.f;
  for (int dz = l0; dz <= h0; ++dz)
    for (int dy = l1; dy <= h1; ++dy)
      for (int dx = l2; dx <= h2; ++dx) acc += w[(size_t)((dz + 1) * 9 + (dy + 1) * 3 + (dx + 1)) * cc + e];
  wc[t] = acc;
}

__global__ __launch_bounds__(256) void k_expand_weights_bwd(const float *__restrict__ dwc, int cc,
                                                           float *__restrict__ dw) {
  const int t = blockIdx.x * 256 + threadIdx.x;
  if (t >= 27 * cc) return;
  const int tap = t / cc, e = t - tap * cc;
  const int d0 = tap / 9 - 1, d1 = (tap / 3) % 3 - 1, d2 = tap % 3 - 1;
  float acc = 0.f;
  for (int g = 0; g < 8; ++g) {
    const int j0 = (g >> 2) & 1, j1 = (g >> 1) & 1, j2 = g & 1;
    const int i0 = j0 ? (d0 > 0) : (d0 >= 0), i1 = j1 ? (d1 > 0) : (d1 >= 0), i2 = j2 ? (d2 > 0) : (d2 >= 0);
    acc += dwc[(size_t)(g * 8 + i0 * 4 + i1 * 2 + i2) * cc + e];
  }
  dw[t] = acc;
}

SGNN_EXPORT int sgnn_expand_weights(const float *w, int cin, int cout, float *wc, sgnn_stream_t stream) {
  SGNN_CHECK_ARG(w && wc && cin >= 1 && cout >= 1);
  const int cc = cin * cout;
  SGNN_LAUNCH(k_expand_weights, dim3((64 * cc + 255) / 256), dim3(256), 0, (hipStream_t)stream, w, cc, wc);
  SGNN_CHECK_LAUNCH();
  return SGNN_OK;
}

SGNN_EXPORT int sgnn_expand_weights_bwd(const float *dwc, int cin, int cout, float *dw, sgnn_stream_t stream) {
  SGNN_CHECK_ARG(dwc && dw && cin >= 1 && cout >= 1);
  const int cc = cin * cout;
  SGNN_LAUNCH(k_expand_weights_bwd, dim3((27 * cc + 255) / 256), dim3(256), 0, (hipStream_t)stream, dwc, cc, dw);
  SGNN_CHECK_LAUNCH();
  return SGNN_OK;
}

template <int CIN, int COUT>
struct DwCfg {
  static constexpr int MT = (CIN + 15) / 16, NT = (COUT + 15) / 16;
  static constexpr int KPB = (MT * NT == 1) ? 9 : ((MT * NT <= 3) ? 5 : 3);
};

#ifndef DW_PAIR
#define DW_PAIR 1
#endif
template <int CIN, int COUT, bool EX, int KPBT = 0>
__global__ __launch_bounds__(256) void k_conv_dw(const float *__restrict__ x, int64_t n_in,
                                                const float *__restrict__ dy, const int32_t *__restrict__ table,
                                                int64_t ld, int K, int64_t n_out, float *__restrict__ partial,
                                                int64_t rows_per_block, int in_shift, ConvEx ex, int64_t ldx,
                                                int64_t ld_dy, const int64_t *n_dev) {
  if (n_dev) {
    n_out = sgnn_dyn_n(n_out, n_dev);
    const int64_t per = (n_out + gridDim.x - 1) / gridDim.x;
    rows_per_block = ((per + 255) / 256) * 256;
    if (rows_per_block < 256) rows_per_block = 256;
  }
  constexpr int MT = (CIN + 15) / 16, NT = (COUT + 15) / 16;
  constexpr int DW_KPB = KPBT > 0 ? KPBT : DwCfg<CIN, COUT>::KPB;
  constexpr int V = (CIN + 3) / 4, CINP = 4 * V;
  constexpr int W = (COUT + 3) / 4, COUTP = 4 * W;
  constexpr int XS = 64 * CINP, YS = 64 * COUTP;
  constexpr bool PAIR = DW_PAIR && MT * NT == 1 && CIN == 8 && KPBT == 0 && !EX;
  constexpr int XT = PAIR ? 2 : 1;
  constexpr int RED = DW_KPB * MT * 16 * NT * 16;
  constexpr int LDS_FLOATS = (4 * (XT * XS + YS) > RED) ? 4 * (XT * XS + YS) : RED;
  __shared__ __attribute__((aligned(16))) float lds[LDS_FLOATS];

  const int tid = threadIdx.x, lane = tid & 63, wave = tid >> 6;
  const int i16 = lane & 15, q = lane >> 4;
  const unsigned lin = sgnn_xcd_tile(blockIdx.y * gridDim.x + blockIdx.x, gridDim.x * gridDim.y);
  const unsigned bx = lin / gridDim.y, by = lin % gridDim.y;
  const unsigned groups = EX ? (unsigned)ex.groups : 1u;
  const unsigned kgroups = gridDim.y / groups;
  const unsigned grp = by / kgroups;
  const int k0 = (by % kgroups) * DW_KPB;
  const int32_t *kmap = (EX && ex.kmap) ? ex.kmap + grp * K : nullptr;
  const int table_rows = EX ? ex.table_rows : K;
  const int kc = (K - k0) < DW_KPB ? (K - k0) : DW_KPB;
  const int64_t blk_row0 = (int64_t)bx * rows_per_block;
  int64_t blk_row1 = blk_row0 + rows_per_block;
  if (blk_row1 > n_out) blk_row1 = n_out;

  const uint32_t ldx4 = (uint32_t)ldx * 4u;
  const __amdgpu_buffer_rsrc_t rs_x = make_rsrc(x, (uint32_t)(((n_in - 1) * ldx + CIN) * 4));
  const __amdgpu_buffer_rsrc_t rs_t = make_rsrc(table, (uint32_t)((int64_t)table_rows * ld * 4));
  const __amdgpu_buffer_rsrc_t rs_dy = make_rsrc(dy, (uint32_t)(((n_out * groups - 1) * ld_dy + COUT) * 4));
  const uint32_t ld4 = (uint32_t)ld * 4u;
  float *xs = lds + wave * (XT * XS + YS);
  float *ys = xs + XT * XS;

  constexpr int NP = (DW_KPB + 1) / 2;
  f32x4 accp[PAIR ? NP : 1];
#pragma unroll
  for (int p = 0; p < (PAIR ? NP : 1); ++p) accp[p] = f32x4{0.f, 0.f, 0.f, 0.f};
  f32x4 acc[DW_KPB][MT][NT];
#pragma unroll
  for (int kk = 0; kk < DW_KPB; ++kk)
#pragma unroll
    for (int mt = 0; mt < MT; ++mt)
#pragma unroll
      for (int nt = 0; nt < NT; ++nt) acc[kk][mt][nt] = f32x4{0.f, 0.f, 0.f, 0.f};

  constexpr bool RCX = (CIN == 16 || CIN == 8);
  constexpr int LPR = RCX ? CIN / 4 : 1, RPI = 64 / LPR, NI = RCX ? LPR : 4, GW = RCX ? 4 : V;
  const int rc_row = lane / LPR, rc_chunk = lane % LPR;
  auto gather = [&](int32_t iv, float(&g)[NI][GW]) {
#pragma unroll
    for (int m = 0; m < NI; ++m) {
      const int32_t id = __builtin_amdgcn_ds_bpermute((RCX ? m * RPI + rc_row : m * 16 + i16) * 4, iv);
      buf_load_floats<GW>(rs_x, (uint32_t)id * ldx4 + (uint32_t)(RCX ? rc_chunk * 16 : q * V * 4), g[m]);
    }
  };
  auto norm_rows = [&](float(&g)[NI][GW]) {
    if constexpr (CINP != CIN) {
#pragma unroll
      for (int m = 0; m < NI; ++m)
#pragma unroll
        for (int s = 0; s < GW; ++s)
          if (3 * V + s >= CIN) g[m][s] = (q == 3) ? 0.f : g[m][s];
    }
  };
  auto store_rows = [&](const float(&g)[NI][GW]) {
#pragma unroll
    for (int m = 0; m < NI; ++m) {
      float *p = RCX ? xs + (m * RPI + rc_row) * CINP + rc_chunk * 4 : xs + (m * 16 + i16) * CINP + q * V;
#pragma unroll
      for (int s = 0; s < GW; ++s) p[s] = g[m][s];
    }
  };
  auto store_rows_to = [&](const float(&g)[NI][GW], float *tile) {
#pragma unroll
    for (int m = 0; m < NI; ++m) {
      float *p = tile + (m * RPI + rc_row) * CINP + rc_chunk * 4;
#pragma unroll
      for (int s = 0; s < GW; ++s) p[s] = g[m][s];
    }
  };
  auto mma_pair = [&](int p, const float(&b)[16][NT]) {
    const float *src = xs + (i16 >> 3) * XS + (i16 & 7);
#pragma unroll
    for (int t = 0; t < 16; ++t) {
      const float a = ((i16 & 7) < CINP) ? src[(4 * t + q) * CINP] : 0.f;
      accp[p] = __builtin_amdgcn_mfma_f32_16x16x4f32(a, b[t][0], accp[p], 0, 0, 0);
    }
  };
  auto mma_chunk = [&](int kk, const float(&b)[16][NT]) {
#pragma unroll
    for (int t = 0; t < 16; ++t) {
      float a[MT];
#pragma unroll
      for (int mt = 0; mt < MT; ++mt) {
        const int ch = mt * 16 + i16;
        a[mt] = (ch < CINP) ? xs[(4 * t + q) * CINP + ch] : 0.f;
      }
#pragma unroll
      for (int mt = 0; mt < MT; ++mt)
#pragma unroll
        for (int nt = 0; nt < NT; ++nt)
          acc[kk][mt][nt] = __builtin_amdgcn_mfma_f32_16x16x4f32(a[mt], b[t][nt], acc[kk][mt][nt], 0, 0, 0);
    }
  };

  for (int64_t base = blk_row0 + wave * 64; base < blk_row1; base += 256) {
    int32_t idxv[DW_KPB];
#pragma unroll
    for (int kk = 0; kk < DW_KPB; ++kk) {
      const int ko = k0 + (kk < kc ? kk : kc - 1);
      int32_t id;
      if constexpr (EX) {
        const int trow = kmap ? kmap[ko] : ko;
        id = (int32_t)__builtin_amdgcn_raw_buffer_load_b32(rs_t, (uint32_t)(base + lane) * 4u, trow * ld4, 0);
        id = (id >> in_shift) * ex.in_mul + ((ex.kadd && id >= 0) ? ex.kadd[grp * K + ko] : 0);
      } else {
        id = (int32_t)__builtin_amdgcn_raw_buffer_load_b32(rs_t, (uint32_t)(base + lane) * 4u, ko * ld4, 0) >> in_shift;
      }
      idxv[kk] = (kk < kc) ? id : -1;
    }
    if constexpr (COUT == 16 || COUT == 8) {
      constexpr int LY = COUT / 4, RY = 64 / LY;
      const int yr = lane / LY, yc = lane % LY;
      float g[LY][4];
#pragma unroll
      for (int m = 0; m < LY; ++m) {
        const int64_t row = base + m * RY + yr;
        const uint32_t off = (row < blk_row1) ? (uint32_t)((row * groups + grp) * ld_dy + yc * 4) * 4u : 0xFFFFF800u;
        buf_load_floats<4>(rs_dy, off, g[m]);
      }
#pragma unroll
      for (int m = 0; m < LY; ++m) {
        float *p = ys + (m * RY + yr) * COUTP + yc * 4;
#pragma unroll
        for (int s = 0; s < 4; ++s) p[s] = g[m][s];
      }
    } else {
      float g[4][W];
#pragma unroll
      for (int m = 0; m < 4; ++m) {
        const int64_t row = base + m * 16 + i16;
        const uint32_t off =
            (row < blk_row1) ? (uint32_t)((row * groups + grp) * ld_dy + q * W) * 4u : 0xFFFFF800u;
        buf_load_floats<W>(rs_dy, off, g[m]);
        if constexpr (COUTP != COUT) {
#pragma unroll
          for (int s = 0; s < W; ++s)
            if (3 * W + s >= COUT) g[m][s] = (q == 3) ? 0.f : g[m][s];
        }
      }
#pragma unroll
      for (int m = 0; m < 4; ++m) {
        float *p = ys + (m * 16 + i16) * COUTP + q * W;
#pragma unroll
// ... 391 lines not shown
```

sgnn_amd/csrc/prog.hip:

```cpp
#include <mutex>
#include <vector>
#include "common.h"

enum {
  OP_CONV_SUBM = 0, OP_CONV_DOWN = 1, OP_UNPOOL = 2, OP_BN = 3, OP_ADD = 4, OP_JOIN = 5,
  OP_CONCAT_IN = 6,
  OP_EXPAND = 7,
  OP_LINEAR = 8
};
#define OPW 12
#define EXPAND_DX_SPLIT 4

extern "C" int sgnn_expand_weights(const float *w, int cin, int cout, float *wc, sgnn_stream_t stream);
extern "C" int sgnn_expand_weights_bwd(const float *dwc, int cin, int cout, float *dw, sgnn_stream_t stream);
int64_t sgnn_bf16_wfrag_bytes(int cin, int cout, int K, int groups);
int sgnn_bf16_conv_prepare(const float *w, int cin, int cout, int K, int groups, void *wf, sgnn_stream_t stream);
int sgnn_bf16_conv_run(const void *x, int64_t n_in, int cin, int64_t ldx, const float *w, const void *wf, int K,
                       const int32_t *table, int64_t ld, int64_t n_out, int cout, void *y, int64_t ldy,
                       const void *addend, int64_t ld_add, const int32_t *kmap, int groups, int table_rows,
                       const int64_t *n_dev, sgnn_stream_t stream);
int sgnn_bf16_conv_expand_impl(const void *x, int64_t n, int cin, int64_t ldx, const float *w, const int32_t *nbr,
                               int64_t ld, int cout, void *y, int64_t ldy, const int64_t *n_dev, void *ws,
                               sgnn_stream_t stream);
int sgnn_bf16_linear_rows(const void *x, int64_t ldx, int64_t n, int cin, const float *const *w, const float *const *b,
                          int cout, float *y, const int64_t *n_dev, sgnn_stream_t stream);

namespace {

struct Op {
  int32_t type, in0, in1, out, par, lev, cin, cout, in2, ia, ib, ic;
  bool is_conv() const { return type == OP_CONV_SUBM || type == OP_CONV_DOWN; }
  int K() const { return type == OP_CONV_DOWN ? 8 : 27; }
  int out_class() const { return type == OP_CONV_DOWN ? lev + 1 : lev; }
  template <class F>
  void for_inputs(F f) const {
    f(in0);
    if (type == OP_ADD || type == OP_JOIN || type == OP_CONCAT_IN) f(in1);
    if (type == OP_CONCAT_IN) f(in2);
  }
};
static_assert(sizeof(Op) == sizeof(int32_t[OPW]), "Op mirrors one record of the caller's int32 array");

struct View {
  const int32_t *ops;
  const float *opf;
  int nops;
  const int32_t *bufs;
  int nbuf, n_ext;
  const int64_t *lev_n, *lev_ld;
  void *const *lev_nbr, *const *lev_children, *const *lev_ptable, *const *lev_parent;
  int nlev;
  const Op &op(int i) const { return reinterpret_cast<const Op *>(ops)[i]; }
};

enum Kind { TRAINING, INFERENCE, INFERENCE_BF16 };

Kind kind_of_mode(int mode) { return mode == 3 ? INFERENCE_BF16 : mode == 2 ? INFERENCE : TRAINING; }

inline int64_t round64(int64_t v) { return (v + 63) & ~int64_t(63); }

struct ConvSetup {
  bool ok = false;
  int K = 0, cnt_class = 0;
  int64_t n = 0, n_out = 0;
  const int32_t *tab_f = nullptr, *tab_b = nullptr;
  int64_t ld_f = 0, ld_b = 0;
  int flags_b = 0;
  ConvSetup(const View &v, const Op &o) {
    const bool down = o.type == OP_CONV_DOWN;
    K = o.K();
    cnt_class = o.out_class();
    ok = o.lev >= 0 && cnt_class < v.nlev;
    if (!ok) return;
    n = v.lev_n[o.lev];
    n_out = v.lev_n[cnt_class];
    if (!v.lev_ld) return;
    tab_f = (const int32_t *)(down ? v.lev_children[o.lev] : v.lev_nbr[o.lev]);
    ld_f = v.lev_ld[cnt_class];
    tab_b = (const int32_t *)(down ? v.lev_ptable[o.lev] : v.lev_nbr[o.lev]);
    ld_b = v.lev_ld[o.lev];
    flags_b = down ? SGNN_CONV_TRANSPOSE_W : (SGNN_CONV_TRANSPOSE_W | SGNN_CONV_FLIP_K);
  }
};

std::vector<int> count_readers(const View &v) {
  std::vector<int> r(v.nbuf, 0);
  for (int i = 0; i < v.nops; ++i)
    v.op(i).for_inputs([&](int b) {
      if (b >= 0 && b < v.nbuf) ++r[b];
    });
  return r;
}

#define g_fuse (g_tune.prog_fusion != 0)
#define g_lin_add (g_tune.prog_lin_add != 0)
#define g_lin_bn (g_tune.prog_lin_bn != 0)
struct Plan {
  std::vector<int> add_dst;
  std::vector<int> add_src;
  std::vector<char> skip;
  std::vector<int> root, col;
  std::vector<int64_t> ld;
  std::vector<char> join_view;
  std::vector<int> lin_bn;
  Kind kind = TRAINING;
  std::vector<char> f32;
  bool bf16() const { return kind == INFERENCE_BF16; }
};

inline int64_t round8(int64_t v) { return (v + 7) & ~int64_t(7); }

bool strided_conv_ok(const Op &o) {
  return sgnn_conv_epi_supported(o.cin, o.cout) && sgnn_conv_epi_supported(o.cout, o.cin) && dw_shape_ok(o.cin, o.cout);
}

void make_plan(const View &v, const int32_t *keep, Plan &P, Kind kind) {
  P.kind = kind;
  P.f32.assign(v.nbuf, P.bf16() ? 0 : 1);
  if (P.bf16())
    for (int i = 0; i < v.nops; ++i)
      if (v.op(i).type == OP_LINEAR && v.op(i).out >= 0 && v.op(i).out < v.nbuf) P.f32[v.op(i).out] = 1;
  auto row_ld = [&](int r) -> int64_t { return P.f32[r] ? v.bufs[2 * r + 1] : round8(v.bufs[2 * r + 1]); };
  P.add_dst.assign(v.nops, -1);
  P.add_src.assign(v.nops, -1);
  P.skip.assign(v.nops, 0);
  P.join_view.assign(v.nops, 0);
  P.lin_bn.assign(v.nops, -1);
  P.root.resize(v.nbuf);
  P.col.assign(v.nbuf, 0);
  P.ld.resize(v.nbuf);
  for (int b = 0; b < v.nbuf; ++b) {
    P.root[b] = b;
    P.ld[b] = row_ld(b);
  }
  if (!g_fuse) return;
  std::vector<int> readers = count_readers(v);
  if (keep)
    for (int b = 0; b < v.nbuf; ++b)
      if (keep[b]) ++readers[b];
  if (g_lin_bn)
    for (int i = 0; i < v.nops; ++i) {
      const Op &o = v.op(i);
      if (o.type != OP_LINEAR || o.cout > 2 || readers[o.in0] != 1) continue;
      for (int j = 0; j < i; ++j) {
        const Op &b = v.op(j);
        if (b.type == OP_BN && b.out == o.in0 && b.lev == o.lev) P.lin_bn[i] = j;
      }
    }
  for (int i = 0; i + 1 < v.nops; ++i) {
    const Op &o = v.op(i), &a = v.op(i + 1);
    if (!o.is_conv() || a.type != OP_ADD) continue;
    if (!sgnn_conv_epi_supported(o.cin, o.cout) || ConvSetup(v, o).n_out <= 0 || readers[o.out] != 1) continue;
    if ((a.in0 != o.out && a.in1 != o.out) || a.in0 == a.in1) continue;
    P.add_dst[i] = a.out;
    P.add_src[i] = a.in0 == o.out ? a.in1 : a.in0;
    P.skip[i + 1] = 1;
  }
  std::vector<int> prod(v.nbuf, -1), last_reader(v.nbuf, -1);
  std::vector<char> strided_ok(v.nbuf, 1);
  for (int i = 0; i < v.nops; ++i) {
    const Op &o = v.op(i);
    if (!P.skip[i]) prod[P.add_dst[i] >= 0 ? P.add_dst[i] : o.out] = i;
    auto reads = [&](int b, bool ok) {
      if (b < 0) return;
      last_reader[b] = i;
      if (!ok) strided_ok[b] = 0;
    };
    auto join_read = [&](int b) { return last_reader[b] >= 0 && v.op(last_reader[b]).type == OP_JOIN; };
    switch (o.type) {
      case OP_CONV_SUBM:
      case OP_CONV_DOWN: reads(o.in0, strided_conv_ok(o)); break;
      case OP_BN:
      case OP_UNPOOL: reads(o.in0, true); break;
      case OP_JOIN:
        reads(o.in0, !join_read(o.in0));
        reads(o.in1, !join_read(o.in1));
        break;
      case OP_ADD: reads(o.in0, P.skip[i] != 0); reads(o.in1, P.skip[i] != 0); break;
      default: o.for_inputs([&](int b) { reads(b, false); }); break;
    }
  }
  for (int i = 0; i < v.nops; ++i) {
    const Op &o = v.op(i);
    if (o.type != OP_JOIN || v.lev_n[o.lev] <= 0) continue;
    bool ok = true;
    for (int side = 0; side < 2 && ok; ++side) {
      const int q = side ? o.in1 : o.in0;
      ok = q >= v.n_ext && !(keep && keep[q]) && P.root[q] == q && strided_ok[q] && last_reader[q] == i && prod[q] >= 0;
      if (!ok) break;
      const Op &p = v.op(prod[q]);
      ok = (p.is_conv() && strided_conv_ok(p)) || p.type == OP_BN || p.type == OP_UNPOOL;
    }
    if (!ok || o.in0 == o.in1) continue;
    if (P.bf16() && (o.cin & 1)) continue;
    P.join_view[i] = 1;
    P.skip[i] = 1;
    P.root[o.in0] = o.out;
    P.col[o.in0] = 0;
    P.root[o.in1] = o.out;
    P.col[o.in1] = o.cin;
  }
  for (int b = 0; b < v.nbuf; ++b) {
    int r = b, c = 0;
    while (P.root[r] != r) {
      c += P.col[r];
      r = P.root[r];
    }
    P.root[b] = r;
    P.col[b] = c;
    P.ld[b] = row_ld(r);
  }
}

struct Layout {
  std::vector<int64_t> buf_off, buf_floats, aux_off;
  int64_t max_buf = 0, total = 0, fwd_total = 0, scratch0 = 0, scratch1 = 0, bextra = 0;
  std::vector<char> shadow;
  std::vector<int> first;
};

int64_t aux_floats(const Op &o, Kind kind) {
  const int64_t slices = round64(64 * (int64_t)o.cin * o.cout);
  if (kind == INFERENCE_BF16) {
    if (o.is_conv()) return round64(sgnn_bf16_wfrag_bytes(o.cin, o.cout, o.K(), 1) / 4);
    return o.type == OP_EXPAND ? slices + round64(sgnn_bf16_wfrag_bytes(o.cin, o.cout, 8, 8) / 4) : 0;
  }
  return o.type == OP_BN ? round64(2 * (int64_t)o.cin) : o.type == OP_EXPAND ? slices : 0;
}

int64_t place_aux(const View &v, Kind kind, Layout &L, int64_t off) {
  for (int i = 0; i < v.nops; ++i) {
    const int64_t a = aux_floats(v.op(i), kind);
    if (a <= 0) continue;
    L.aux_off[i] = off;
    off += a;
  }
  return off;
}

int make_layout_infer(const View &v, const Plan &P, const int32_t *keep, Layout &L) {
  const int never = v.nops + 1;
  std::vector<int> first(v.nbuf, never), last(v.nbuf, -1);
  auto in_arena = [&](int b) { return b >= v.n_ext || L.shadow[b]; };
  for (int i = 0; i < v.nops; ++i) {
    auto touch = [&](int b) {
      if (b < 0 || b >= v.nbuf || !in_arena(b)) return;
      const int r = P.root[b];
      if (i < first[r]) first[r] = i;
      if (i > last[r]) last[r] = i;
    };
    v.op(i).for_inputs(touch);
    touch(P.add_dst[i] >= 0 ? P.add_dst[i] : v.op(i).out);
  }
  for (int b = v.n_ext; b < v.nbuf; ++b)
    if (keep && keep[b]) last[P.root[b]] = never;
  std::vector<std::pair<int64_t, int64_t>> free_list;
  int64_t top = place_aux(v, P.kind, L, 0);
  auto release = [&](int64_t o, int64_t n) {
    if (n <= 0) return;
    size_t k = 0;
    while (k < free_list.size() && free_list[k].first < o) ++k;
    free_list.insert(free_list.begin() + k, std::make_pair(o, n));
    if (k + 1 < free_list.size() && free_list[k].first + free_list[k].second == free_list[k + 1].first) {
      free_list[k].second += free_list[k + 1].second;
      free_list.erase(free_list.begin() + k + 1);
    }
    if (k > 0 && free_list[k - 1].first + free_list[k - 1].second == free_list[k].first) {
      free_list[k - 1].second += free_list[k].second;
      free_list.erase(free_list.begin() + k);
    }
  };
  auto take = [&](int64_t n) -> int64_t {
    if (n <= 0) return 0;
    size_t best = free_list.size();
    for (size_t k = 0; k < free_list.size(); ++k)
      if (free_list[k].second >= n && (best == free_list.size() || free_list[k].second < free_list[best].second)) best = k;
    if (best < free_list.size()) {
      const int64_t o = free_list[best].first;
      free_list[best].first += n;
      free_list[best].second -= n;
      if (free_list[best].second == 0) free_list.erase(free_list.begin() + best);
      return o;
    }
    if (!free_list.empty() && free_list.back().first + free_list.back().second == top) {
      const int64_t o = free_list.back().first;
      free_list.pop_back();
      top = o + n;
      return o;
    }
    const int64_t o = top;
    top += n;
    return o;
  };
  for (int i = 0; i < v.nops; ++i) {
    for (int b = 0; b < v.nbuf; ++b)
      if (in_arena(b) && P.root[b] == b && L.buf_off[b] >= 0 && last[b] == i - 1) release(L.buf_off[b], round64(L.buf_floats[b]));
    for (int b = 0; b < v.nbuf; ++b)
      if (in_arena(b) && P.root[b] == b && first[b] == i) L.buf_off[b] = take(round64(L.buf_floats[b]));
  }
  for (int b = v.n_ext; b < v.nbuf; ++b) {
    if (P.root[b] == b && L.buf_off[b] < 0) L.buf_off[b] = 0;
  }
  for (int b = v.n_ext; b < v.nbuf; ++b)
    if (P.root[b] != b) L.buf_off[b] = P.bf16() ? L.buf_off[P.root[b]] : L.buf_off[P.root[b]] + P.col[b];
  L.first = first;
  L.fwd_total = L.total = top;
  L.scratch0 = L.scratch1 = L.bextra = top;
  return 0;
}

int make_layout(const View &v, const Plan &P, Layout &L, const int32_t *keep) {
  L.buf_off.assign(v.nbuf, -1);
  L.buf_floats.resize(v.nbuf);
  L.aux_off.assign(v.nops, -1);
  L.shadow.assign(v.nbuf, 0);
  for (int b = 0; b < v.nbuf; ++b) {
    const int lev = v.bufs[2 * b], ch = v.bufs[2 * b + 1];
    if (lev < 0 || lev >= v.nlev || ch < 1) return -1;
    const int64_t elems = v.lev_n[lev] * (int64_t)(P.root[b] == b ? P.ld[b] : ch);
    L.buf_floats[b] = P.f32[b] ? elems : (elems + 1) / 2;
    if (L.buf_floats[b] > L.max_buf) L.max_buf = L.buf_floats[b];
  }
  if (P.kind != TRAINING) {
    if (P.bf16())
      for (int i = 0; i < v.nops; ++i) {
        if (v.op(i).type == OP_CONCAT_IN) continue;
        v.op(i).for_inputs([&](int b) {
          if (b >= 0 && b < v.n_ext) L.shadow[b] = 1;
        });
      }
    return make_layout_infer(v, P, keep, L);
  }
  int64_t off = 0;
  for (int b = v.n_ext; b < v.nbuf; ++b) {
    if (P.root[b] != b) continue;
    L.buf_off[b] = off;
    off += round64(L.buf_floats[b]);
  }
  for (int b = v.n_ext; b < v.nbuf; ++b)
    if (P.root[b] != b) L.buf_off[b] = L.buf_off[P.root[b]] + P.col[b];
  off = place_aux(v, TRAINING, L, off);
  int64_t bextra = 0;
  for (int i = 0; i < v.nops; ++i) {
    const Op &o = v.op(i);
    if (o.type != OP_EXPAND) continue;
    const int64_t need = aux_floats(o, TRAINING) + round64(v.lev_n[o.lev] * EXPAND_DX_SPLIT * (int64_t)o.cin);
    if (need > bextra) bextra = need;
  }
  L.fwd_total = off;
  L.scratch0 = off;
  off += round64(L.max_buf);
  L.scratch1 = off;
  off += round64(L.max_buf);
  L.bextra = off;
  off += bextra;
  L.total = off;
  return 0;
}

inline int64_t expand_dwc_bytes(int cin, int cout) { return (64 * (int64_t)cin * cout * 4 + 255) & ~int64_t(255); }

int64_t dw_slice(const View &v, int i) {
  const Op &o = v.op(i);
  int64_t w = 0;
  if (o.is_conv()) w = sgnn_conv_bwd_weight_ws_bytes(ConvSetup(v, o).n_out, o.K(), o.cin, o.cout);
  if (o.type == OP_EXPAND)
    w = ((sgnn_conv_bwd_weight_ws_bytes(v.lev_n[o.lev], 64, o.cin, o.cout) + 255) & ~int64_t(255)) + expand_dwc_bytes(o.cin, o.cout);
  return (w + 255) & ~int64_t(255);
}

int64_t dw_ws_need(const View &v) {
  int64_t need = 0;
  for (int i = 0; i < v.nops; ++i) need += dw_slice(v, i);
  return need;
}

int64_t ws_main(const View &v) {
  int64_t need = 0;
  for (int i = 0; i < v.nops; ++i) {
    const Op &o = v.op(i);
    int64_t w = 0;
    if (o.type == OP_BN) w = sgnn_bn_ws_bytes(v.lev_n[o.lev], o.cin);
    if (o.type == OP_LINEAR) w = sgnn_linear_ws_bytes(v.lev_n[o.lev], o.cin, o.cout);
    if (w > need) need = w;
  }
  const int64_t dw = dw_ws_need(v);
  if (dw > need) need = dw;
  return (need + 255) & ~int64_t(255);
}

int64_t ws_stats(const View &v) {
  int64_t need = 0;
  for (int i = 0; i < v.nops; ++i) {
    const Op &o = v.op(i);
    if (!o.is_conv()) continue;
    const ConvSetup cs(v, o);
    const int64_t a = ((cs.n_out > 0 ? cs.n_out : 1) + 15) / 16 * 2 * o.cout * (int64_t)sizeof(double);
    const int64_t b = ((cs.n > 0 ? cs.n : 1) + 15) / 16 * 2 * o.cin * (int64_t)sizeof(double);
    if (a > need) need = a;
    if (b > need) need = b;
  }
  return (need + 255) & ~int64_t(255);
}

int64_t ws_need(const View &v) { return ws_main(v) + ws_stats(v); }

struct SideLane {
  hipStream_t stream = nullptr;
  void *ws = nullptr;
  int64_t ws_bytes = 0;
  hipEvent_t fork = nullptr, join = nullptr;
} g_side;
std::mutex g_side_mu;
bool g_defer_join = false;

#define PROG_TRY(call)           \
  do {                           \
    const int rc_ = (call);      \
    if (rc_ != SGNN_OK) return rc_; \
  } while (0)

struct Ctx {
  View v;
  void *const *params, *const *idx, *const *lev_cnt;
  int nparams, nidx, training;
  void *ws;
  int64_t ws_bytes;
  sgnn_stream_t stream;
  Plan P;
  Layout L;
  std::vector<const double *> pre;
  std::vector<int64_t> pre_nblk;
  double *stats_ws;

  bool prepare(Kind kind, const int32_t *keep) {
    make_plan(v, keep, P, kind);
    if (make_layout(v, P, L, keep) != 0) return false;
    pre = std::vector<const double *>(v.nops, nullptr);
    pre_nblk = std::vector<int64_t>(v.nops, 0);
    stats_ws = (double *)((char *)ws + ws_main(v));
    return true;
  }
  int ch(int b) const { return b < 0 ? 0 : v.bufs[2 * b + 1]; }
  int cls(int b) const { return v.bufs[2 * b]; }
  int64_t rows(int b) const { return v.lev_n[cls(b)]; }
  int64_t ld(int b) const { return P.ld[b]; }
  float *param(int p) const { return (p >= 0 && p < nparams) ? (float *)params[p] : nullptr; }
  const int32_t *index(int i) const { return (i >= 0 && i < nidx && idx) ? (const int32_t *)idx[i] : nullptr; }
  const int64_t *count(int c) const { return (lev_cnt && c >= 0 && c < v.nlev) ? (const int64_t *)lev_cnt[c] : nullptr; }
  int wait_once(void *&wait_event) const {
    if (!wait_event) return SGNN_OK;
    sgnn_stamp("down-wait<", stream);
    SGNN_HIP_TRY(hipStreamWaitEvent((hipStream_t)stream, (hipEvent_t)wait_event, 0));
    sgnn_stamp("down-wait>", stream);
    wait_event = nullptr;
    return SGNN_OK;
  }
};

}

SGNN_EXPORT int sgnn_prog_set_side_stream(sgnn_stream_t stream2, void *ws2, int64_t ws2_bytes) {
  std::lock_guard<std::mutex> hold(g_side_mu);
  if (stream2 && !g_side.fork) {
    SGNN_HIP_TRY(hipEventCreateWithFlags(&g_side.fork, hipEventDisableTiming));
    SGNN_HIP_TRY(hipEventCreateWithFlags(&g_side.join, hipEventDisableTiming));
  }
  g_side.stream = (hipStream_t)stream2;
  g_side.ws = stream2 ? ws2 : nullptr;
  g_side.ws_bytes = stream2 ? ws2_bytes : 0;
  return SGNN_OK;
}

SGNN_EXPORT int sgnn_prog_defer_join(int on) {
  const int prev = g_defer_join ? 1 : 0;
  g_defer_join = on != 0;
  return prev;
}

SGNN_EXPORT int64_t sgnn_prog_arena_floats(const int32_t *ops, int nops, const int32_t *bufs, int nbuf, int n_ext,
                                           const int64_t *lev_n, int nlev, const int32_t *keep, int mode) {
  View v{ops, nullptr, nops, bufs, nbuf, n_ext, lev_n, nullptr, nullptr, nullptr, nullptr, nullptr, nlev};
  if (mode < 0 || mode > 3) return -1;
  Plan P;
  make_plan(v, keep, P, kind_of_mode(mode));
  Layout L;
  if (make_layout(v, P, L, keep) != 0) return -1;
  return mode == 0 ? L.total : L.fwd_total;
}

SGNN_EXPORT int64_t sgnn_prog_ws_bytes(const int32_t *ops, int nops, const int64_t *lev_n, int nlev) {
  View v{ops, nullptr, nops, nullptr, 0, 0, lev_n, nullptr, nullptr, nullptr, nullptr, nullptr, nlev};
  return ws_need(v);
}

SGNN_EXPORT int64_t sgnn_prog_buffer_offset(const int32_t *ops, int nops, const int32_t *bufs, int nbuf, int n_ext,
                                            const int64_t *lev_n, int nlev, const int32_t *keep, int infer, int b) {
  View v{ops, nullptr, nops, bufs, nbuf, n_ext, lev_n, nullptr, nullptr, nullptr, nullptr, nullptr, nlev};
  if (infer < 0 || infer > 2) return -1;
  const Kind kind = infer == 2 ? INFERENCE_BF16 : infer == 1 ? INFERENCE : TRAINING;
  Plan P;
  make_plan(v, keep, P, kind);
  Layout L;
  if (make_layout(v, P, L, keep) != 0 || b < 0 || b >= nbuf || b < n_ext) return -1;
  return P.root[b] == b ? L.buf_off[b] : -1;
}

SGNN_EXPORT int sgnn_prog_plan(const int32_t *ops, int nops, const int32_t *bufs, int nbuf, int n_ext, const int64_t *lev_n,
                               int nlev, const int32_t *keep, int mode, int32_t *out) {
  SGNN_CHECK_ARG(ops && bufs && lev_n && out && nops >= 0 && nbuf >= 1 && nlev >= 1 && n_ext >= 0 && n_ext <= nbuf &&
                 mode >= 0 && mode <= 3);
  View v{ops, nullptr, nops, bufs, nbuf, n_ext, lev_n, nullptr, nullptr, nullptr, nullptr, nullptr, nlev};
  Plan P;
  make_plan(v, keep, P, kind_of_mode(mode));
  for (int i = 0; i < nops; ++i) {
    out[4 * i] = P.skip[i];
    out[4 * i + 1] = P.add_dst[i];
    out[4 * i + 2] = P.join_view[i];
    out[4 * i + 3] = P.lin_bn[i];
  }
  for (int b = 0; b < nbuf; ++b) {
    out[4 * nops + 3 * b] = P.root[b];
    out[4 * nops + 3 * b + 1] = P.col[b];
    out[4 * nops + 3 * b + 2] = (int32_t)P.ld[b];
  }
  return SGNN_OK;
}

static int forward_bf16(const Ctx &c, void *const *ext, float *arena, void *wait_event) {
  const View &v = c.v;
  const Plan &PL = c.P;
  const Layout &L = c.L;
  const sgnn_stream_t stream = c.stream;
  const int n_ext = v.n_ext, nbuf = v.nbuf, nlev = v.nlev;
  auto B = [&](int b) -> void * {
    if (b < 0) return nullptr;
    if (b < n_ext && !L.shadow[b]) return ext[b];
    const int r = PL.root[b];
    return (char *)arena + 4 * L.buf_off[r] + (PL.f32[r] ? 4 : 2) * (int64_t)PL.col[b];
  };
  auto EXT = [&](int b) -> const float * { return b < 0 ? nullptr : (const float *)ext[b]; };
  for (int i = 0; i < v.nops; ++i) {
    const Op &o = v.op(i);
    const int in0 = o.in0, in1 = o.in1, out = o.out, par = o.par, lev = o.lev, cin = o.cin, cout = o.cout;
    SGNN_CHECK_ARG(out >= n_ext && out < nbuf && lev >= 0 && lev < nlev && in0 < nbuf && in1 < nbuf);
    SGNN_CHECK_ARG(o.type == OP_CONCAT_IN || in0 >= 0);
    SGNN_CHECK_ARG(o.type == OP_LINEAR || !PL.f32[out]);
    const int64_t n = v.lev_n[lev];
    for (int b = 0; b < n_ext; ++b)
      if (L.shadow[b] && L.first[b] == i)
        PROG_TRY(sgnn_bf16_concat3(EXT(b), c.ch(b), nullptr, nullptr, 0, nullptr, nullptr, 0, nullptr, c.rows(b), B(b), c.ld(b),
                                   c.count(c.cls(b)), stream));
    if (PL.skip[i]) continue;
    if (o.type == OP_CONV_DOWN) PROG_TRY(c.wait_once(wait_event));
    switch (o.type) {
      case OP_CONV_SUBM:
      case OP_CONV_DOWN: {
        const ConvSetup cs(v, o);
        SGNN_CHECK_ARG(cs.ok);
        int dst = out;
        const void *addend = nullptr;
        int64_t ld_add = 0;
        if (PL.add_dst[i] >= 0) {
          addend = B(PL.add_src[i]);
          ld_add = c.ld(PL.add_src[i]);
          dst = PL.add_dst[i];
        }
        void *wf = arena + L.aux_off[i];
        PROG_TRY(sgnn_bf16_conv_prepare(c.param(par), cin, cout, cs.K, 1, wf, stream));
        PROG_TRY(sgnn_bf16_conv_run(B(in0), c.rows(in0), cin, c.ld(in0), c.param(par), wf, cs.K, cs.tab_f, cs.ld_f, cs.n_out, cout,
                                    B(dst), c.ld(dst), addend, ld_add, nullptr, 1, cs.K, c.count(cs.cnt_class), stream));
        break;
      }
      case OP_UNPOOL:
        SGNN_CHECK_ARG(lev + 1 < nlev);
        PROG_TRY(sgnn_bf16_gather_rows(B(in0), c.ld(in0), cin, (const int32_t *)v.lev_parent[lev], n, B(out), c.ld(out),
                                       c.count(lev), stream));
        break;
      case OP_BN:
        PROG_TRY(sgnn_bf16_bn_eval(B(in0), c.ld(in0), n, cin, c.param(par), c.param(par + 1), c.param(par + 2), c.param(par + 3),
                                   v.opf[4 * i], v.opf[4 * i + 2], B(out), c.ld(out), c.count(lev), stream));
        break;
      case OP_ADD:
        SGNN_CHECK_ARG(in1 >= 0);
        PROG_TRY(sgnn_bf16_add(B(in0), c.ld(in0), B(in1), c.ld(in1), n, cin, B(out), c.ld(out), c.count(lev), stream));
        break;
      case OP_JOIN:
        SGNN_CHECK_ARG(in1 >= 0);
        PROG_TRY(sgnn_bf16_join(B(in0), c.ld(in0), cin, B(in1), c.ld(in1), cout, n, B(out), c.ld(out), c.count(lev), stream));
        break;
      case OP_CONCAT_IN: {
        const int in2 = o.in2;
        SGNN_CHECK_ARG(in2 < nbuf && in0 < n_ext && in1 < n_ext && in2 < n_ext && c.ch(in0) + c.ch(in1) + c.ch(in2) == c.ch(out));
        PROG_TRY(sgnn_bf16_concat3(EXT(in0), c.ch(in0), c.index(o.ia), EXT(in1), c.ch(in1), c.index(o.ib), EXT(in2), c.ch(in2),
                                   c.index(o.ic), n, B(out), c.ld(out), c.count(lev), stream));
        break;
      }
      case OP_EXPAND:
        SGNN_CHECK_ARG(c.rows(out) == 8 * n);
        PROG_TRY(sgnn_bf16_conv_expand_impl(B(in0), n, cin, c.ld(in0), c.param(par), (const int32_t *)v.lev_nbr[lev], v.lev_ld[lev],
                                            cout, B(out), c.ld(out), c.count(lev), arena + L.aux_off[i], stream));
        break;
      case OP_LINEAR: {
        SGNN_CHECK_ARG(cout >= 1 && cout <= 4 && PL.f32[out] && c.ld(out) == cout);
        const float *w[4] = {}, *b[4] = {};
        for (int q = 0; q < cout; ++q) {
          w[q] = c.param(par + 2 * q);
          b[q] = c.param(par + 2 * q + 1);
        }
        PROG_TRY(sgnn_bf16_linear_rows(B(in0), c.ld(in0), n, cin, w, b, cout, (float *)B(out), c.count(lev), stream));
        break;
      }
      default:
        sgnn_set_error("sgnn_prog_forward: unknown op %d", o.type);
        return SGNN_EINVAL;
    }
  }
  return SGNN_OK;
}

SGNN_EXPORT int sgnn_prog_forward(const int32_t *ops, const float *opf, int nops, const int32_t *bufs, int nbuf, int n_ext,
                                  const int64_t *lev_n, const int64_t *lev_ld, void *const *lev_nbr,
                                  void *const *lev_children, void *const *lev_ptable, void *const *lev_parent,
                                  void *const *lev_cnt, int nlev, void *const *params, int nparams,
                                  void *const *ext, void *const *idx,
                                  int nidx, float *arena, int64_t arena_floats, const int32_t *keep, int training,
                                  void *wait_event, void *ws, int64_t ws_bytes, sgnn_stream_t stream) {
  SGNN_CHECK_ARG(ops && opf && bufs && lev_n && lev_ld && params && arena && nops >= 0 && nbuf >= 1 && nlev >= 1 &&
                 n_ext >= 0 && n_ext <= nbuf && (n_ext == 0 || ext));
  const Kind kind = (training & 4) ? INFERENCE_BF16 : (training & 2) ? INFERENCE : TRAINING;
  if ((training & 4) && (training & 3) != 2) {
    sgnn_set_error("sgnn_prog_forward: bf16 storage needs the inference layout in eval mode (training = 2 | 4)");
    return SGNN_EINVAL;
  }
  training &= 1;
  Ctx c{View{ops, opf, nops, bufs, nbuf, n_ext, lev_n, lev_ld, lev_nbr, lev_children, lev_ptable, lev_parent, nlev},
        params, idx, lev_cnt, nparams, nidx, training, ws, ws_bytes, stream};
  SGNN_CHECK_ARG(c.prepare(kind, keep));
  const View &v = c.v;
  const Plan &PL = c.P;
  const Layout &L = c.L;
  if (arena_floats < L.fwd_total) {
    sgnn_set_error("sgnn_prog_forward: arena too small (%lld < %lld floats)", (long long)arena_floats,
                   (long long)L.fwd_total);
    return SGNN_ENOWS;
  }
  if (ws_bytes < ws_need(v)) {
    sgnn_set_error("sgnn_prog_forward: workspace too small");
    return SGNN_ENOWS;
  }
  if (kind == INFERENCE_BF16) return forward_bf16(c, ext, arena, wait_event);
  auto B = [&](int b) -> float * { return b < 0 ? nullptr : (b < n_ext ? (float *)ext[b] : arena + L.buf_off[b]); };
  for (int i = 0; i < nops; ++i) {
    const Op &o = v.op(i);
    const int in0 = o.in0, in1 = o.in1, out = o.out, par = o.par, lev = o.lev, cin = o.cin, cout = o.cout;
    SGNN_CHECK_ARG(out >= n_ext && out < nbuf && lev >= 0 && lev < nlev && in0 < nbuf && in1 < nbuf);
    SGNN_CHECK_ARG(o.type == OP_CONCAT_IN || in0 >= 0);
    const int64_t n = lev_n[lev];
    if (PL.skip[i]) continue;
    if (o.type == OP_CONV_DOWN) PROG_TRY(c.wait_once(wait_event));
    switch (o.type) {
      case OP_CONV_SUBM:
      case OP_CONV_DOWN: {
        const ConvSetup cs(v, o);
        SGNN_CHECK_ARG(cs.ok);
        ConvEpi epi{};
        int dst_buf = out;
        if (PL.add_dst[i] >= 0) {
          epi.addend = B(PL.add_src[i]);
          epi.ld_add = c.ld(PL.add_src[i]);
          dst_buf = PL.add_dst[i];
        }
        const int j = i + 1 + (PL.add_dst[i] >= 0 ? 1 : 0);
        if (g_fuse && training && cs.n_out > 0 && j < nops && v.op(j).type == OP_BN && v.op(j).in0 == dst_buf &&
            sgnn_conv_epi_supported(cin, cout)) {
          epi.stats = 1;
          epi.partial = c.stats_ws;
          c.pre[j] = c.stats_ws;
          c.pre_nblk[j] = sgnn_conv_grid_blocks(cs.n_out, cin, cout, cs.K);
        }
        epi.ldx = c.ld(in0);
        epi.ldy = c.ld(dst_buf);
        epi.n_dev = c.count(cs.cnt_class);
        PROG_TRY(sgnn_conv_fwd_impl(B(in0), n, cin, c.param(par), cs.K, cs.tab_f, cs.ld_f, cs.n_out, cout, B(dst_buf), 0, 0,
                                    nullptr, nullptr, 1, 1, cs.K, &epi, stream));
        break;
      }
      case OP_UNPOOL:
        SGNN_CHECK_ARG(lev + 1 < nlev);
        PROG_TRY(sgnn_gather_rows_ld(B(in0), c.ld(in0), cin, (const int32_t *)lev_parent[lev], n, B(out), c.ld(out), stream,
                                     c.count(lev)));
        break;
      case OP_BN: {
        float *save = arena + L.aux_off[i];
        PROG_TRY(sgnn_bn_fwd_impl(B(in0), c.ld(in0), n, cin, c.param(par), c.param(par + 1), c.param(par + 2), c.param(par + 3),
                                  opf[4 * i], opf[4 * i + 1], training, opf[4 * i + 2], save, save + cin, B(out), c.ld(out),
                                  c.pre[i], c.pre_nblk[i], ws, ws_bytes, stream, c.count(lev)));
        break;
      }
      case OP_ADD:
        SGNN_CHECK_ARG(in1 >= 0);
        PROG_TRY(sgnn_add_ld(B(in0), c.ld(in0), B(in1), c.ld(in1), n, cin, B(out), c.ld(out), stream, c.count(lev)));
        break;
      case OP_JOIN:
        SGNN_CHECK_ARG(in1 >= 0 && c.ld(in0) == cin && c.ld(in1) == cout && c.ld(out) == cin + cout);
        PROG_TRY(sgnn_concat_rows_dn(B(in0), cin, nullptr, B(in1), cout, nullptr, n, B(out), stream, c.count(lev)));
        break;
      case OP_CONCAT_IN: {
        const int in2 = o.in2;
        SGNN_CHECK_ARG(in2 < nbuf && c.ch(in0) + c.ch(in1) + c.ch(in2) == c.ch(out) && c.ld(out) == c.ch(out));
        PROG_TRY(sgnn_concat3_rows_dn(B(in0), c.ch(in0), c.index(o.ia), B(in1), c.ch(in1), c.index(o.ib), B(in2), c.ch(in2),
                                      c.index(o.ic), n, B(out), stream, c.count(lev)));
        break;
      }
      case OP_EXPAND: {
        SGNN_CHECK_ARG(c.rows(out) == 8 * n && c.ld(in0) == cin && c.ld(out) == cout);
        const int32_t *S, *ST, *PAR;
        PROG_TRY(sgnn_expand_maps(&S, &ST, &PAR));
        float *wc = arena + L.aux_off[i];
        PROG_TRY(sgnn_expand_weights(c.param(par), cin, cout, wc, stream));
        ConvEpi xepi{};
        xepi.n_dev = c.count(lev);
        PROG_TRY(sgnn_conv_fwd_impl(B(in0), n, cin, wc, 8, (const int32_t *)lev_nbr[lev], lev_ld[lev], n, cout, B(out), 0,
                                    0, S, nullptr, 1, 8, 27, &xepi, stream));
        break;
      }
      case OP_LINEAR: {
        SGNN_CHECK_ARG(cout >= 1 && cout <= 4 && c.ld(in0) == cin);
        const float *w[4] = {}, *b[4] = {};
        for (int q = 0; q < cout; ++q) {
          w[q] = c.param(par + 2 * q);
          b[q] = c.param(par + 2 * q + 1);
        }
        PROG_TRY(sgnn_linear_fwd_rows(B(in0), n, cin, w, b, cout, B(out), stream, c.count(lev)));
        break;
      }
      default:
        sgnn_set_error("sgnn_prog_forward: unknown op %d", o.type);
        return SGNN_EINVAL;
    }
  }
  return SGNN_OK;
}

namespace {

struct Grads {
  enum State : char { NONE, HELD, ALIAS, CALLER };
  const Ctx &c;
  void *const *pgrads, *const *ext, *const *gext, *const *gout;
  const float *arena;
  float *garena;
  std::vector<State> state;
  std::vector<int> alias;
  std::vector<int> lazy_lin;
  std::vector<char> viewed;
  float *scratch[2];

  Grads(const Ctx &c_, void *const *pgrads_, void *const *ext_, void *const *gext_, void *const *gout_, const float *arena_,
        float *garena_)
      : c(c_), pgrads(pgrads_), ext(ext_), gext(gext_), gout(gout_), arena(arena_), garena(garena_),
        state(c_.v.nbuf, NONE), alias(c_.v.nbuf, -1), lazy_lin(c_.v.nbuf, -1), viewed(c_.v.nbuf, 0),
        scratch{garena_ + c_.L.scratch0, garena_ + c_.L.scratch1} {
    for (int b = 0; b < c.v.nbuf; ++b)
      if (c.P.root[b] != b) viewed[b] = viewed[c.P.root[b]] = 1;
  }
  const float *X(int b) const { return b < 0 ? nullptr : (b < c.v.n_ext ? (const float *)ext[b] : arena + c.L.buf_off[b]); }
  float *G(int b) const { return b < c.v.n_ext ? (float *)gext[b] : garena + c.L.buf_off[b]; }
  float *PG(int p) const { return (p >= 0 && p < c.nparams) ? (float *)pgrads[p] : nullptr; }
  bool wants(int b) const { return b >= c.v.n_ext || gext[b] != nullptr; }
  bool has(int b) const { return state[b] != NONE; }
  const float *held(int b) const { return state[b] == CALLER ? (const float *)gout[b] : G(b); }
  int64_t held_ld(int b) const { return state[b] == CALLER ? (int64_t)c.ch(b) : c.ld(b); }
  const float *read(int b) const { return state[b] == ALIAS ? held(alias[b]) : held(b); }
  int64_t read_ld(int b) const { return state[b] == ALIAS ? held_ld(alias[b]) : held_ld(b); }
  void written(int b) {
    state[b] = HELD;
    alias[b] = -1;
  }
  float *target(int b, int which) const { return state[b] == HELD ? scratch[which] : G(b); }
  int64_t target_ld(int b, const float *t) const { return t == G(b) ? c.ld(b) : c.ch(b); }
  int commit(int b, float *wrote) {
    const int64_t n = c.rows(b);
    const int ch = c.ch(b);
    const int64_t *cnt = c.count(c.cls(b));
    if (wrote != G(b)) return sgnn_add_ld(G(b), c.ld(b), wrote, ch, n, ch, G(b), c.ld(b), c.stream, cnt);
    if (state[b] == ALIAS || state[b] == CALLER) {
      const float *other = read(b);
      const int64_t ldo = read_ld(b);
      written(b);
      return sgnn_add_ld(G(b), c.ld(b), other, ldo, n, ch, G(b), c.ld(b), c.stream, cnt);
    }
    written(b);
    return SGNN_OK;
  }
  int adopt_outputs() {
    for (int b = c.v.n_ext; b < c.v.nbuf; ++b) {
      if (!gout[b]) continue;
      if (viewed[b] || !g_fuse) {
        if (c.L.buf_floats[b] > 0) PROG_TRY(sgnn_copy_words(G(b), gout[b], c.L.buf_floats[b], (hipStream_t)c.stream));
        state[b] = HELD;
      } else {
        state[b] = CALLER;
      }
    }
    return SGNN_OK;
  }
  int finish_externals() {
    for (int b = 0; b < c.v.n_ext; ++b) {
      if (!gext[b] || c.L.buf_floats[b] == 0) continue;
      if (state[b] == ALIAS)
        PROG_TRY(sgnn_copy_words(G(b), read(b), c.L.buf_floats[b], (hipStream_t)c.stream));
      else if (state[b] == NONE)
        PROG_TRY(sgnn_fill32(G(b), 0u, c.L.buf_floats[b], (hipStream_t)c.stream));
    }
    return SGNN_OK;
  }
};

struct Lane {
  struct PendingExpand { const float *dwc; int cin, cout; float *dw; };
  std::unique_lock<std::mutex> lock;
  hipStream_t hs;
  bool side, forked = false;
  char *ws;
  int64_t off = 0;
  DwBatch batch{};
  std::vector<PendingExpand> pending_expand;

  Lane(const Ctx &c, hipStream_t hs_) : lock(g_side_mu, std::try_to_lock), hs(hs_) {
    side = lock.owns_lock() && g_side.stream && g_side.stream != hs && g_side.ws && g_side.ws_bytes >= dw_ws_need(c.v);
    ws = (char *)(side ? g_side.ws : c.ws);
    sgnn_dw_batch = side ? &batch : nullptr;
  }
  ~Lane() { sgnn_dw_batch = nullptr; }
  hipStream_t stream() const { return side ? g_side.stream : hs; }
  hipStream_t fork() {
    if (!side) return hs;
    (void)hipEventRecord(g_side.fork, hs);
    (void)hipStreamWaitEvent(g_side.stream, g_side.fork, 0);
    forked = true;
    return g_side.stream;
  }
  int finish() {
    PROG_TRY(sgnn_dw_batch_flush(&batch, stream()));
    for (const PendingExpand &pe : pending_expand)
      PROG_TRY(sgnn_expand_weights_bwd(pe.dwc, pe.cin, pe.cout, pe.dw, (sgnn_stream_t)stream()));
    if (forked && !g_defer_join) {
      SGNN_HIP_TRY(hipEventRecord(g_side.join, g_side.stream));
      SGNN_HIP_TRY(hipStreamWaitEvent(hs, g_side.join, 0));
    }
    return SGNN_OK;
  }
};

int bwd_unreached(const Ctx &c, const Grads &g, const Op &o) {
  const hipStream_t hs = (hipStream_t)c.stream;
  if (o.is_conv() || o.type == OP_EXPAND) PROG_TRY(sgnn_fill32(g.PG(o.par), 0u, (int64_t)o.K() * o.cin * o.cout, hs));
  if (o.type == OP_BN) {
    void *zp[2] = {g.PG(o.par), g.PG(o.par + 1)};
    const int64_t zw[2] = {o.cin, o.cin};
    PROG_TRY(sgnn_fill32_multi(zp, zw, 2, 0u, hs));
  }
  if (o.type == OP_LINEAR)
    for (int q = 0; q < o.cout; ++q) {
      void *zp[2] = {g.PG(o.par + 2 * q), g.PG(o.par + 2 * q + 1)};
      const int64_t zw[2] = {o.cin, 1};
      PROG_TRY(sgnn_fill32_multi(zp, zw, 2, 0u, hs));
    }
  return SGNN_OK;
}

int bwd_conv(Ctx &c, Grads &g, Lane &lane, int i) {
  const Op &o = c.v.op(i);
  const ConvSetup cs(c.v, o);
  SGNN_CHECK_ARG(cs.ok);
  const int in0 = o.in0, cin = o.cin, cout = o.cout;
  const float *dy = g.read(o.out);
  const int64_t ld_dy = g.read_ld(o.out);
  const hipStream_t ls = lane.fork();
  if (g.wants(in0)) {
    if (g_fuse && sgnn_conv_epi_supported(cout, cin) && cs.n > 0) {
      ConvEpi epi{};
      if (g.has(in0)) {
        epi.addend = g.read(in0);
        epi.ld_add = g.read_ld(in0);
      }
      if (i > 0 && c.v.op(i - 1).type == OP_BN && c.v.op(i - 1).out == in0 && c.v.op(i - 1).cin == cin) {
        const Op &bo = c.v.op(i - 1);
        const float *save = g.arena + c.L.aux_off[i - 1];
        epi.stats = 2;
        epi.partial = c.stats_ws;
        epi.bn_x = g.X(bo.in0);
        epi.ld_bnx = c.ld(bo.in0);
        epi.mean = save;
        epi.invstd = save + cin;
        epi.gamma = c.param(bo.par);
        epi.beta = c.param(bo.par + 1);
        epi.leak = c.v.opf[4 * (i - 1) + 2];
        c.pre[i - 1] = c.stats_ws;
        c.pre_nblk[i - 1] = sgnn_conv_grid_blocks(cs.n, cout, cin, cs.K);
      }
      epi.ldx = ld_dy;
      epi.ldy = c.ld(in0);
      epi.n_dev = c.count(o.lev);
      PROG_TRY(sgnn_conv_fwd_impl(dy, cs.n_out, cout, c.param(o.par), cs.K, cs.tab_b, cs.ld_b, cs.n, cin, g.G(in0), cs.flags_b, 0,
                                  nullptr, nullptr, 1, 1, cs.K, &epi, c.stream));
      g.written(in0);
    } else {
      SGNN_CHECK_ARG(ld_dy == cout);
      float *t = g.target(in0, 0);
      ConvEpi pepi{};
      pepi.n_dev = c.count(o.lev);
      PROG_TRY(sgnn_conv_fwd_impl(dy, cs.n_out, cout, c.param(o.par), cs.K, cs.tab_b, cs.ld_b, cs.n, cin, t, cs.flags_b, 0, nullptr,
                                  nullptr, 1, 1, cs.K, &pepi, c.stream));
      PROG_TRY(g.commit(in0, t));
    }
  }
  const int64_t slice = dw_slice(c.v, i);
  PROG_TRY(sgnn_conv_bwd_weight_impl(g.X(in0), cs.n, cin, c.ld(in0), dy, cout, ld_dy, cs.tab_f, cs.ld_f, cs.K, cs.n_out,
                                     g.PG(o.par), 0, nullptr, nullptr, 1, 1, cs.K, lane.ws + lane.off, slice, (sgnn_stream_t)ls,
                                     c.count(cs.cnt_class)));
  if (ls != lane.hs) sgnn_stamp("dw>", (sgnn_stream_t)ls);
  lane.off += slice;
  return SGNN_OK;
}

int bwd_unpool(Ctx &c, Grads &g, Lane &, int i) {
  const Op &o = c.v.op(i);
  if (!g.wants(o.in0)) return SGNN_OK;
  float *t = g.target(o.in0, 0);
  PROG_TRY(sgnn_gather_sum_ld(g.read(o.out), g.read_ld(o.out), o.cin, (const int32_t *)c.v.lev_children[o.lev],
                              c.v.lev_ld[o.lev + 1], 8, c.v.lev_n[o.lev + 1], t, g.target_ld(o.in0, t), c.stream,
                              c.count(o.lev + 1)));
  return g.commit(o.in0, t);
}

int bwd_bn(Ctx &c, Grads &g, Lane &, int i) {
  const Op &o = c.v.op(i);
  const int in0 = o.in0, cin = o.cin;
  const float *save = g.arena + c.L.aux_off[i];
  const float *addend = nullptr;
  int64_t ld_add = cin;
  if (g.wants(in0) && g.has(in0)) {
    addend = g.read(in0);
    ld_add = g.read_ld(in0);
  }
  float *t = g.wants(in0) ? g.G(in0) : g.scratch[0];
  BnLin bl{};
  const bool lazy = g.lazy_lin[o.out] >= 0;
  if (lazy) {
    const Op &lo = c.v.op(g.lazy_lin[o.out]);
    bl.g = g.read(lo.out);
    bl.ldg = g.read_ld(lo.out);
    bl.nout = lo.cout;
    for (int q = 0; q < lo.cout; ++q) bl.w[q] = c.param(lo.par + 2 * q);
  }
  PROG_TRY(sgnn_bn_bwd_impl(g.X(in0), c.ld(in0), lazy ? nullptr : g.read(o.out), g.read_ld(o.out), c.v.lev_n[o.lev], cin,
                            c.param(o.par), c.param(o.par + 1), save, save + cin, c.training, c.v.opf[4 * i + 2], addend, ld_add,
                            t, g.wants(in0) ? c.ld(in0) : cin, g.PG(o.par), g.PG(o.par + 1), c.pre[i], c.pre_nblk[i], c.ws,
                            c.ws_bytes, c.stream, c.count(o.lev), lazy ? &bl : nullptr));
  if (g.wants(in0)) g.written(in0);
  return SGNN_OK;
}

int bwd_add(Ctx &c, Grads &g, Lane &, int i) {
  const Op &o = c.v.op(i);
  const int64_t n = c.v.lev_n[o.lev];
  const float *dy = g.read(o.out);
  const int64_t ld_dy = g.read_ld(o.out);
  const int src = g.state[o.out] == Grads::ALIAS ? g.alias[o.out] : o.out;
  for (int b : {o.in0, o.in1}) {
    if (!g.wants(b)) continue;
    if (g.state[b] == Grads::HELD) {
      PROG_TRY(sgnn_add_ld(g.G(b), c.ld(b), dy, ld_dy, n, o.cin, g.G(b), c.ld(b), c.stream, c.count(o.lev)));
    } else if (g.has(b)) {
      PROG_TRY(sgnn_add_ld(g.read(b), g.read_ld(b), dy, ld_dy, n, o.cin, g.G(b), c.ld(b), c.stream, c.count(o.lev)));
      g.written(b);
    } else {
      g.state[b] = Grads::ALIAS;
      g.alias[b] = src;
    }
  }
  return SGNN_OK;
}

int bwd_join(Ctx &c, Grads &g, Lane &, int i) {
  const Op &o = c.v.op(i);
  const int in0 = o.in0, in1 = o.in1;
  if (c.P.join_view[i]) {
    if (g.state[o.out] != Grads::HELD || g.has(in0) || g.has(in1)) {
      sgnn_set_error("sgnn_prog_backward: in-place JoinTable met an unexpected gradient state");
      return SGNN_EINVAL;
    }
    g.written(in0);
    g.written(in1);
    return SGNN_OK;
  }
  const int64_t n = c.v.lev_n[o.lev];
  SGNN_CHECK_ARG(g.read_ld(o.out) == o.cin + o.cout && c.ld(in0) == o.cin && c.ld(in1) == o.cout);
// ... 136 lines not shown
```

sgnn_amd/csrc/tune.hip:

```cpp
#include <string.h>
#include "common.h"

sgnn_tune g_tune = {
     1,
     160 * 256,
     1,
     1,
     1,
     256,
     1,
     1,
     1,
     1,
     1,
     1,
     1,
     1,
};

namespace {
struct Field {
  const char *name;
  int64_t sgnn_tune::*ptr;
  int64_t lo, hi;
  bool boolean;
};
const Field kFields[] = {
    {"conv_small", &sgnn_tune::conv_small, 0, 1, true},
    {"conv_small_rows", &sgnn_tune::conv_small_rows, 0, (int64_t)1 << 36, false},
    {"conv_unrolled", &sgnn_tune::conv_unrolled, 0, 1, true},
    {"conv_one_round", &sgnn_tune::conv_one_round, 0, 1, true},
    {"conv_wide_epi", &sgnn_tune::conv_wide_epi, 0, 1, true},
    {"conv_dw_blocks", &sgnn_tune::conv_dw_blocks, 1, 4096, false},
    {"conv_dw_c1", &sgnn_tune::conv_dw_c1, 0, 1, true},
    {"rulebook_multi", &sgnn_tune::rulebook_multi, 0, 1, true},
    {"scan_inline", &sgnn_tune::scan_inline, 0, 1, true},
    {"chain_merged", &sgnn_tune::chain_merged, 0, 1, true},
    {"prog_fusion", &sgnn_tune::prog_fusion, 0, 1, true},
    {"prog_lin_bn", &sgnn_tune::prog_lin_bn, 0, 1, true},
    {"prog_lin_add", &sgnn_tune::prog_lin_add, 0, 1, true},
    {"bn_fuse", &sgnn_tune::bn_fuse, 0, 1, true},
};
const Field *find(const char *name) {
  if (!name) return nullptr;
  for (const Field &f : kFields)
    if (strcmp(f.name, name) == 0) return &f;
  return nullptr;
}
}

SGNN_EXPORT int64_t sgnn_tune_get(const char *name) {
  const Field *f = find(name);
  if (!f) {
    sgnn_set_error("sgnn_tune_get: no switch named '%s' (sgnn_tune_names lists them)", name ? name : "(null)");
    return SGNN_TUNE_UNKNOWN;
  }
  return g_tune.*(f->ptr);
}

SGNN_EXPORT int64_t sgnn_tune_set(const char *name, int64_t value) {
  const Field *f = find(name);
  if (!f) {
    sgnn_set_error("sgnn_tune_set: no switch named '%s' (sgnn_tune_names lists them)", name ? name : "(null)");
    return SGNN_TUNE_UNKNOWN;
  }
  const int64_t prev = g_tune.*(f->ptr);
  if (f->boolean) value = value != 0;
  if (value < f->lo || value > f->hi) {
    sgnn_set_error("sgnn_tune_set: %s = %lld is outside [%lld, %lld]", name, (long long)value, (long long)f->lo, (long long)f->hi);
    return SGNN_TUNE_UNKNOWN;
  }
  g_tune.*(f->ptr) = value;
  return prev;
}

SGNN_EXPORT const char *sgnn_tune_names(void) {
  static char buf[512];
  if (!buf[0]) {
    size_t n = 0;
    for (const Field &f : kFields) n += (size_t)snprintf(buf + n, sizeof(buf) - n, "%s%s", n ? "," : "", f.name);
  }
  return buf;
}

SGNN_EXPORT const sgnn_tune *sgnn_tune_current(void) { return &g_tune; }
```

Baseline: 5448.

## Fold training BatchNorm apply into the following small submanifold conv kernel

When a training-mode BN feeds directly into a small submanifold conv at the same level, the BN apply kernel is skipped. The conv kernel itself reduces the BN partial stats, applies normalization and activation to its gathered inputs, and writes the BN output rows. This removes one kernel launch and one full read/write pass over the activations. In exchange, every conv block redundantly reduces the stats partials, and a second stats workspace is added for the case where the conv's own epilogue stats would collide with the first.

Result: faster. 5532, median of 6 (+1.6%).

```diff
diff --git a/include/sgnn_hip.h b/include/sgnn_hip.h
--- a/include/sgnn_hip.h
+++ b/include/sgnn_hip.h
@@ -53,6 +53,7 @@
   int64_t prog_lin_bn;
   int64_t prog_lin_add;
   int64_t bn_fuse;
+  int64_t prog_bn_conv_fold;
 } sgnn_tune;
 int64_t sgnn_tune_set(const char *name, int64_t value);
 int64_t sgnn_tune_get(const char *name);
diff --git a/sgnn_amd/csrc/bn.hip b/sgnn_amd/csrc/bn.hip
--- a/sgnn_amd/csrc/bn.hip
+++ b/sgnn_amd/csrc/bn.hip
@@ -1,12 +1,11 @@
 #include "common.h"
+#include "bn_fuse.h"
 
 #define BN_MAX_BLOCKS 2048
 #define BN_FLUSH 2
 #ifndef BN_U
 #define BN_U 2
 #endif
-#define BN_FUSE_BLOCKS 4096
-#define BN_FUSE_MAXC 64
 
 struct BnGeom {
   int vec;
@@ -256,76 +255,6 @@
 }
 
 
-struct BnFuse {
-  const double *partial;
-  int nblk;
-  float eps, momentum;
-  float *running_mean, *running_var, *save_mean, *save_invstd;
-  float *dgamma, *dbeta;
-};
-
-#ifndef BN_TOTALS_WIDE
-#define BN_TOTALS_WIDE 1
-#endif
-typedef double f64x2 __attribute__((ext_vector_type(2)));
-__device__ __forceinline__ void bn_fuse_totals(const BnFuse &f, int c, double *scratch, double *tot) {
-  const int tid = threadIdx.x;
-  const int tpc = 256 / c;
-  if (BN_TOTALS_WIDE && (c & 1) == 0 && (((uintptr_t)f.partial) & 15) == 0) {
-    const int hp = c >> 1;
-    const int p2 = tid % hp, which = (tid / hp) & 1, part = tid / c;
-    f64x2 acc = {0.0, 0.0};
-    if (part < tpc) {
-      constexpr int U = 32;
-      for (int blk = part; blk < f.nblk; blk += U * tpc) {
-        f64x2 v[U];
-#pragma unroll
-        for (int u = 0; u < U; ++u) {
-          const int bi = blk + u * tpc;
-          v[u] = bi < f.nblk ? *reinterpret_cast<const f64x2 *>(f.partial + ((size_t)bi * 2 + which) * c + 2 * p2) : f64x2{0.0, 0.0};
-        }
-#pragma unroll
-        for (int u = 0; u < U; ++u) acc += v[u];
-      }
-      scratch[which * 256 + part * c + 2 * p2] = acc[0];
-      scratch[which * 256 + part * c + 2 * p2 + 1] = acc[1];
-    }
-  } else {
-    const int ch = tid % c, part = tid / c;
-    double a = 0.0, b = 0.0;
-    if (part < tpc) {
-      for (int blk = part; blk < f.nblk; blk += 8 * tpc) {
-        double va[8], vb[8];
-#pragma unroll
-        for (int u = 0; u < 8; ++u) {
-          const int bi = blk + u * tpc;
-          const bool ok = bi < f.nblk;
-          va[u] = ok ? f.partial[((size_t)bi * 2 + 0) * c + ch] : 0.0;
-          vb[u] = ok ? f.partial[((size_t)bi * 2 + 1) * c + ch] : 0.0;
-        }
-#pragma unroll
-        for (int u = 0; u < 8; ++u) {
-          a += va[u];
-          b += vb[u];
-        }
-      }
-      scratch[part * c + ch] = a;
-      scratch[256 + part * c + ch] = b;
-    }
-  }
-  __syncthreads();
-  if (tid < c) {
-    double s1 = 0.0, s2 = 0.0;
-    for (int p = 0; p < tpc; ++p) {
-      s1 += scratch[p * c + tid];
-      s2 += scratch[256 + p * c + tid];
-    }
-    tot[tid] = s1;
-    tot[c + tid] = s2;
-  }
-  __syncthreads();
-}
-
 template <int VEC, bool FUSE>
 __global__ __launch_bounds__(256) void k_bn_apply(const float *__restrict__ x, int64_t ldx, int64_t n, int c, int cq,
                                                  int rpb, const float *__restrict__ mean,
@@ -340,24 +269,7 @@
   if (n <= 0) return;
   if constexpr (FUSE) {
     bn_fuse_totals(fuse, c, s_scratch, s_tot);
-    for (int ch = threadIdx.x; ch < c; ch += 256) {
-      const double s1 = s_tot[ch], s2 = s_tot[c + ch];
-      const double mu = s1 / (double)n;
-      double var = s2 / (double)n - mu * mu;
-      if (var < 0.0) var = 0.0;
-      const float fm = (float)mu, fi = (float)(1.0 / sqrt(var + (double)fuse.eps));
-      s_mean[ch] = fm;
-      s_inv[ch] = fi;
-      if (blockIdx.x == 0) {
-        fuse.save_mean[ch] = fm;
-        fuse.save_invstd[ch] = fi;
-        if (fuse.running_mean) fuse.running_mean[ch] = fuse.momentum * fuse.running_mean[ch] + (1.f - fuse.momentum) * fm;
-        if (fuse.running_var) {
-          const double unb = var * ((double)n / (double)(n > 1 ? n - 1 : 1));
-          fuse.running_var[ch] = fuse.momentum * fuse.running_var[ch] + (1.f - fuse.momentum) * (float)unb;
-        }
-      }
-    }
+    bn_fuse_finalize_fwd(fuse, c, n, s_tot, s_mean, s_inv);
     __syncthreads();
     mean = s_mean;
     invstd = s_inv;
@@ -501,10 +413,6 @@
   }
 }
 
-static bool bn_fuse_ok(int64_t nblk, int c, int apply_grid) {
-  return c <= BN_FUSE_MAXC && nblk <= BN_FUSE_BLOCKS && nblk * (int64_t)apply_grid * 2 * c * (int64_t)sizeof(double) <= (48ll << 20);
-}
-
 static int bn_apply_grid(int64_t n, const BnGeom &g) {
   int64_t b = (n + (int64_t)g.rpb * BN_U - 1) / ((int64_t)g.rpb * BN_U);
   if (b < 1) b = 1;
@@ -515,8 +423,10 @@
 int sgnn_bn_fwd_impl(const float *x, int64_t ldx, int64_t n, int c, const float *gamma, const float *beta,
                      float *running_mean, float *running_var, float eps, float momentum, int training, float leak,
                      float *save_mean, float *save_invstd, float *y, int64_t ldy, const double *pre_partial,
-                     int64_t pre_nblk, void *ws, int64_t ws_bytes, sgnn_stream_t stream, const int64_t *n_dev) {
+                     int64_t pre_nblk, void *ws, int64_t ws_bytes, sgnn_stream_t stream, const int64_t *n_dev,
+                     ConvBnFold *fold, int64_t fold_grid) {
   hipStream_t s = (hipStream_t)stream;
+  if (fold) fold->fuse.partial = nullptr;
   SGNN_CHECK_ARG(n >= 0 && c >= 1 && (c % 4 == 0 ? c <= 1024 : c <= 256) && save_mean && save_invstd);
   SGNN_CHECK_ARG(training || (running_mean && running_var));
   if (ldx <= 0) ldx = c;
@@ -560,6 +470,11 @@
     SGNN_LAUNCH(k_bn_eval_stats, dim3(1), dim3(256), 0, s, (const float *)running_mean,
                        (const float *)running_var, c, eps, save_mean, save_invstd);
   }
+  if (fold && fuse.partial && y && bn_fuse_ok(fuse.nblk, c, fold_grid)) {
+    *fold = ConvBnFold{fuse, gamma, beta, leak, y, ldy};
+    SGNN_CHECK_LAUNCH();
+    return SGNN_OK;
+  }
   if (n > 0) {
     SGNN_CHECK_ARG(x && y);
     const int grid = bn_apply_grid(n, g);
diff --git a/sgnn_amd/csrc/bn_fuse.h b/sgnn_amd/csrc/bn_fuse.h
--- /dev/null
+++ b/sgnn_amd/csrc/bn_fuse.h
@@ -0,0 +1,110 @@
+#pragma once
+#include "common.h"
+
+#define BN_FUSE_BLOCKS 4096
+#define BN_FUSE_MAXC 64
+
+
+struct BnFuse {
+  const double *partial;
+  int nblk;
+  float eps, momentum;
+  float *running_mean, *running_var, *save_mean, *save_invstd;
+  float *dgamma, *dbeta;
+};
+
+struct ConvBnFold {
+  BnFuse fuse;
+  const float *gamma, *beta;
+  float leak;
+  float *y;
+  int64_t ldy;
+};
+
+static inline bool bn_fuse_ok(int64_t nblk, int c, int64_t apply_grid) {
+  return c <= BN_FUSE_MAXC && nblk <= BN_FUSE_BLOCKS && nblk * apply_grid * 2 * c * (int64_t)sizeof(double) <= (48ll << 20);
+}
+
+#ifndef BN_TOTALS_WIDE
+#define BN_TOTALS_WIDE 1
+#endif
+typedef double f64x2 __attribute__((ext_vector_type(2)));
+__device__ __forceinline__ void bn_fuse_totals(const BnFuse &f, int c, double *scratch, double *tot) {
+  const int tid = threadIdx.x;
+  const int tpc = 256 / c;
+  if (BN_TOTALS_WIDE && (c & 1) == 0 && (((uintptr_t)f.partial) & 15) == 0) {
+    const int hp = c >> 1;
+    const int p2 = tid % hp, which = (tid / hp) & 1, part = tid / c;
+    f64x2 acc = {0.0, 0.0};
+    if (part < tpc) {
+      constexpr int U = 32;
+      for (int blk = part; blk < f.nblk; blk += U * tpc) {
+        f64x2 v[U];
+#pragma unroll
+        for (int u = 0; u < U; ++u) {
+          const int bi = blk + u * tpc;
+          v[u] = bi < f.nblk ? *reinterpret_cast<const f64x2 *>(f.partial + ((size_t)bi * 2 + which) * c + 2 * p2) : f64x2{0.0, 0.0};
+        }
+#pragma unroll
+        for (int u = 0; u < U; ++u) acc += v[u];
+      }
+      scratch[which * 256 + part * c + 2 * p2] = acc[0];
+      scratch[which * 256 + part * c + 2 * p2 + 1] = acc[1];
+    }
+  } else {
+    const int ch = tid % c, part = tid / c;
+    double a = 0.0, b = 0.0;
+    if (part < tpc) {
+      for (int blk = part; blk < f.nblk; blk += 8 * tpc) {
+        double va[8], vb[8];
+#pragma unroll
+        for (int u = 0; u < 8; ++u) {
+          const int bi = blk + u * tpc;
+          const bool ok = bi < f.nblk;
+          va[u] = ok ? f.partial[((size_t)bi * 2 + 0) * c + ch] : 0.0;
+          vb[u] = ok ? f.partial[((size_t)bi * 2 + 1) * c + ch] : 0.0;
+        }
+#pragma unroll
+        for (int u = 0; u < 8; ++u) {
+          a += va[u];
+          b += vb[u];
+        }
+      }
+      scratch[part * c + ch] = a;
+      scratch[256 + part * c + ch] = b;
+    }
+  }
+  __syncthreads();
+  if (tid < c) {
+    double s1 = 0.0, s2 = 0.0;
+    for (int p = 0; p < tpc; ++p) {
+      s1 += scratch[p * c + tid];
+      s2 += scratch[256 + p * c + tid];
+    }
+    tot[tid] = s1;
+    tot[c + tid] = s2;
+  }
+  __syncthreads();
+}
+
+__device__ __forceinline__ void bn_fuse_finalize_fwd(const BnFuse &fuse, int c, int64_t n, const double *tot, float *s_mean,
+                                                     float *s_inv) {
+  for (int ch = threadIdx.x; ch < c; ch += 256) {
+    const double s1 = tot[ch], s2 = tot[c + ch];
+    const double mu = s1 / (double)n;
+    double var = s2 / (double)n - mu * mu;
+    if (var < 0.0) var = 0.0;
+    const float fm = (float)mu, fi = (float)(1.0 / sqrt(var + (double)fuse.eps));
+    s_mean[ch] = fm;
+    s_inv[ch] = fi;
+    if (blockIdx.x == 0) {
+      fuse.save_mean[ch] = fm;
+      fuse.save_invstd[ch] = fi;
+      if (fuse.running_mean) fuse.running_mean[ch] = fuse.momentum * fuse.running_mean[ch] + (1.f - fuse.momentum) * fm;
+      if (fuse.running_var) {
+        const double unb = var * ((double)n / (double)(n > 1 ? n - 1 : 1));
+        fuse.running_var[ch] = fuse.momentum * fuse.running_var[ch] + (1.f - fuse.momentum) * (float)unb;
+      }
+    }
+  }
+}
diff --git a/sgnn_amd/csrc/common.h b/sgnn_amd/csrc/common.h
--- a/sgnn_amd/csrc/common.h
+++ b/sgnn_amd/csrc/common.h
@@ -34,7 +34,8 @@
 int sgnn_conv_fwd_impl(const float *x, int64_t n_in, int cin, const float *w, int K, const int32_t *table, int64_t ld,
                        int64_t n_out, int cout, float *y, int flags, int in_shift, const int32_t *kmap,
                        const int32_t *kadd, int in_mul, int groups, int table_rows, const ConvEpi *epi,
-                       sgnn_stream_t stream);
+                       sgnn_stream_t stream, const struct ConvBnFold *bnf = nullptr);
+int64_t sgnn_conv_bn_fold_grid(int64_t n_out, int cin, int cout, int K);
 int64_t sgnn_conv_grid_blocks(int64_t n_out, int cin, int cout, int K);
 struct BnLin {
   const float *g;
@@ -45,7 +46,8 @@
 int sgnn_bn_fwd_impl(const float *x, int64_t ldx, int64_t n, int c, const float *gamma, const float *beta,
                      float *running_mean, float *running_var, float eps, float momentum, int training, float leak,
                      float *save_mean, float *save_invstd, float *y, int64_t ldy, const double *pre_partial,
-                     int64_t pre_nblk, void *ws, int64_t ws_bytes, sgnn_stream_t stream, const int64_t *n_dev = nullptr);
+                     int64_t pre_nblk, void *ws, int64_t ws_bytes, sgnn_stream_t stream, const int64_t *n_dev = nullptr,
+                     struct ConvBnFold *fold = nullptr, int64_t fold_grid = 0);
 int sgnn_bn_bwd_impl(const float *x, int64_t ldx, const float *dy, int64_t ld_dy, int64_t n, int c, const float *gamma,
                      const float *beta, const float *save_mean, const float *save_invstd, int training, float leak,
                      const float *addend, int64_t ld_add, float *dx, int64_t ld_dx, float *dgamma, float *dbeta,
diff --git a/sgnn_amd/csrc/conv.hip b/sgnn_amd/csrc/conv.hip
--- a/sgnn_amd/csrc/conv.hip
+++ b/sgnn_amd/csrc/conv.hip
@@ -2,6 +2,7 @@
 #include "common.h"
 
 #include "conv_common.h"
+#include "bn_fuse.h"
 
 #define CONV_SMALL_GRID ((int64_t)((g_tune.conv_small_rows + CONV_ROWS_PER_BLOCK - 1) / CONV_ROWS_PER_BLOCK))
 
@@ -216,16 +217,19 @@
   conv_fwd_body<CIN, COUT, CONV_MREP, false, true>(x, n_in, w, table, ld, K, n_out, y, flags, in_shift, ex, epi, wg_cap);
 }
 
-template <int CIN, int COUT>
-__global__ __launch_bounds__(256) void k_conv_small(const float *__restrict__ x, int64_t n_in,
-                                                   const float *__restrict__ w, const int32_t *__restrict__ table,
-                                                   int64_t ld, int K, int64_t n_out, float *y, int flags, int in_shift,
-                                                   ConvEpi epi) {
+template <int CIN, int COUT, bool FOLD>
+__device__ __forceinline__ void conv_small_body(const float *__restrict__ x, int64_t n_in, const float *__restrict__ w,
+                                                const int32_t *__restrict__ table, int64_t ld, int K, int64_t n_out,
+                                                float *y, int flags, int in_shift, const ConvEpi &epi,
+                                                const ConvBnFold &bnf) {
   using C = ConvCfg<CIN, COUT>;
   constexpr int V = C::V, CINP = C::CINP, NT = C::NT;
   constexpr int KW = 7;
-  __shared__ float red[4][NT * 256];
+  __shared__ __attribute__((aligned(16))) float red[4][NT * 256];
   __shared__ double sred[4][2][NT * 16];
+  static_assert(!FOLD || CIN <= BN_FUSE_MAXC, "the folded BatchNorm keeps its constants in BN_FUSE_MAXC LDS slots");
+  __shared__ double bn_tot[FOLD ? 2 * BN_FUSE_MAXC : 1];
+  __shared__ float bn_mean[FOLD ? BN_FUSE_MAXC : 1], bn_inv[FOLD ? BN_FUSE_MAXC : 1];
   const int tid = threadIdx.x, lane = tid & 63, wave = tid >> 6;
   const int r = lane & 15, q = lane >> 4;
   const int64_t row0 = (int64_t)blockIdx.x * 16;
@@ -255,9 +259,39 @@
     const int k = k0 + (kk < nk ? kk : (nk > 0 ? nk - 1 : 0));
     id[kk] = (int32_t)__builtin_amdgcn_raw_buffer_load_b32(rs_t, lane_off, (k < K ? k : K - 1) * ld4, 0) >> in_shift;
   }
+  constexpr int NJ = (CIN + 15) / 16;
+  float bn_g[V], bn_b[V], bn_gj[NJ], bn_bj[NJ];
+  if constexpr (FOLD) {
+#pragma unroll
+    for (int s = 0; s < V; ++s) {
+      const int ch = q * V + s;
+      bn_g[s] = (ch < CIN && bnf.gamma) ? bnf.gamma[ch] : 1.f;
+      bn_b[s] = (ch < CIN && bnf.beta) ? bnf.beta[ch] : 0.f;
+    }
+#pragma unroll
+    for (int j = 0; j < NJ; ++j) {
+      const int ch = (tid & 15) + 16 * j;
+      bn_gj[j] = (ch < CIN && bnf.gamma) ? bnf.gamma[ch] : 1.f;
+      bn_bj[j] = (ch < CIN && bnf.beta) ? bnf.beta[ch] : 0.f;
+    }
+    static_assert(sizeof(red) >= 512 * sizeof(double), "bn_fuse_totals needs 512 doubles of scratch");
+    bn_fuse_totals(bnf.fuse, CIN, reinterpret_cast<double *>(&red[0][0]), bn_tot);
+    bn_fuse_finalize_fwd(bnf.fuse, CIN, n_out, bn_tot, bn_mean, bn_inv);
+    __syncthreads();
+  }
   float a[KW][V];
 #pragma unroll
   for (int kk = 0; kk < KW; ++kk) buf_load_floats<V>(rs_x, (uint32_t)id[kk] * ldx4 + (uint32_t)(q * V * 4), a[kk]);
+  float own[NJ];
+  if constexpr (FOLD) {
+    const int64_t orow = row0 + (tid >> 4);
+#pragma unroll
+    for (int j = 0; j < NJ; ++j) {
+      const int ch = (tid & 15) + 16 * j;
+      own[j] = __uint_as_float(__builtin_amdgcn_raw_buffer_load_b32(
+          rs_x, (ch < CIN && orow < n_out) ? (uint32_t)orow * ldx4 + (uint32_t)ch * 4u : 0xFFFFFFFFu, 0, 0));
+    }
+  }
   float b[KW][NT][V];
   if (transpose) {
     const __amdgpu_buffer_rsrc_t rs_w = make_rsrc(w, (uint32_t)((int64_t)K * CIN * COUT * 4));
@@ -336,6 +370,28 @@
           b[kk][nt][s] = v;
         }
       }
+    }
+  }
+  if constexpr (FOLD) {
+    float km[V], ki[V];
+#pragma unroll
+    for (int s = 0; s < V; ++s) {
+      km[s] = bn_mean[(q * V + s) & (BN_FUSE_MAXC - 1)];
+      ki[s] = bn_inv[(q * V + s) & (BN_FUSE_MAXC - 1)];
+    }
+#pragma unroll
+    for (int kk = 0; kk < KW; ++kk)
+#pragma unroll
+      for (int s = 0; s < V; ++s)
+        a[kk][s] = id[kk] >= 0 ? sgnn_bn_act(a[kk][s], km[s], ki[s], bn_g[s], bn_b[s], bnf.leak) : 0.f;
+    const __amdgpu_buffer_rsrc_t rs_o = make_rsrc(bnf.y, (uint32_t)(((n_out - 1) * bnf.ldy + CIN) * 4));
+    const int64_t orow = row0 + (tid >> 4);
+#pragma unroll
+    for (int j = 0; j < NJ; ++j) {
+      const int ch = (tid & 15) + 16 * j;
+      const bool ok = ch < CIN && orow < n_out;
+      const float v = sgnn_bn_act(own[j], bn_mean[ch & (BN_FUSE_MAXC - 1)], bn_inv[ch & (BN_FUSE_MAXC - 1)], bn_gj[j], bn_bj[j], bnf.leak);
+      __builtin_amdgcn_raw_buffer_store_b32(__float_as_uint(v), rs_o, ok ? (uint32_t)orow * (uint32_t)bnf.ldy * 4u + (uint32_t)ch * 4u : 0xFFFFFFFFu, 0, 0);
     }
   }
   if constexpr (CINP != CIN) {
@@ -424,6 +480,22 @@
   }
 }
 
+template <int CIN, int COUT>
+__global__ __launch_bounds__(256) void k_conv_small(const float *__restrict__ x, int64_t n_in,
+                                                   const float *__restrict__ w, const int32_t *__restrict__ table,
+                                                   int64_t ld, int K, int64_t n_out, float *y, int flags, int in_shift,
+                                                   ConvEpi epi) {
+  conv_small_body<CIN, COUT, false>(x, n_in, w, table, ld, K, n_out, y, flags, in_shift, epi, ConvBnFold{});
+}
+
+template <int CIN, int COUT>
+__global__ __launch_bounds__(256) void k_conv_small_bn(const float *__restrict__ x, int64_t n_in,
+                                                      const float *__restrict__ w, const int32_t *__restrict__ table,
+                                                      int64_t ld, int K, int64_t n_out, float *y, int flags,
+                                                      int in_shift, ConvEpi epi, ConvBnFold bnf) {
+  conv_small_body<CIN, COUT, true>(x, n_in, w, table, ld, K, n_out, y, flags, in_shift, epi, bnf);
+}
+
 __global__ __launch_bounds__(256) void k_conv_fwd_generic(const float *__restrict__ x, int cin,
                                                          const float *__restrict__ w, int K,
                                                          const int32_t *__restrict__ table, int64_t ld,
@@ -458,7 +530,8 @@
 #define CONV_FWD_CASES(X) \
   X(1, 8) X(8, 8) X(8, 12) X(12, 12) X(12, 16) X(16, 16) X(34, 16) X(30, 16) X(26, 16) X(48, 16) \
   X(8, 1) X(12, 8) X(16, 12) X(16, 34) X(16, 30) X(16, 26) X(16, 48) X(32, 16) X(16, 32) X(4, 16) X(16, 4) \
-  X(16, 24) X(24, 16) X(24, 32) X(32, 24) X(64, 32) X(32, 64) X(56, 28) X(28, 56) X(32, 32) X(28, 16) X(16, 28)
+  X(16, 24) X(24, 16) X(24, 32) X(32, 24) X(64, 32) X(32, 64) X(56, 28) X(28, 56) X(32, 32) X(28, 16) X(16, 28) \
+  X(5, 8)
 
 int64_t sgnn_conv_grid_blocks(int64_t n_out, int cin, int cout, int K) {
   const int64_t grid4 = (n_out + CONV_ROWS_PER_BLOCK - 1) / CONV_ROWS_PER_BLOCK;
@@ -466,6 +539,12 @@
   return grid4;
 }
 
+
+int64_t sgnn_conv_bn_fold_grid(int64_t n_out, int cin, int cout, int K) {
+  const int64_t grid4 = (n_out + CONV_ROWS_PER_BLOCK - 1) / CONV_ROWS_PER_BLOCK;
+  if (n_out <= 0 || grid4 >= CONV_SMALL_GRID || K > 28 || !g_tune.conv_small || cin > BN_FUSE_MAXC) return 0;
+  return sgnn_conv_epi_supported(cin, cout) ? (n_out + 15) / 16 : 0;
+}
 
 bool sgnn_conv_u_supported(int cin, int cout, int K);
 bool sgnn_conv_u_launch(const float *x, int64_t n_in, int cin, const float *w, int K, const int32_t *table, int64_t ld,
@@ -505,7 +584,7 @@
 int sgnn_conv_fwd_impl(const float *x, int64_t n_in, int cin, const float *w, int K, const int32_t *table, int64_t ld,
                        int64_t n_out, int cout, float *y, int flags, int in_shift, const int32_t *kmap,
                        const int32_t *kadd, int in_mul, int groups, int table_rows, const ConvEpi *epi_in,
-                       sgnn_stream_t stream) {
+                       sgnn_stream_t stream, const ConvBnFold *bnf) {
   SGNN_CHECK_ARG(cin >= 1 && cout >= 1 && K >= 1 && K <= 64 && n_out >= 0 && ld >= n_out && in_shift >= 0 &&
                  in_shift < 31 && in_mul >= 1 && groups >= 1 && groups <= 64 && table_rows >= 1 &&
                  table_rows <= 64 && (kmap || table_rows >= K));
@@ -534,6 +613,10 @@
     return SGNN_EOVERFLOW;
   }
   hipStream_t s = (hipStream_t)stream;
+  if (bnf) {
+    SGNN_CHECK_ARG(plain && flags == 0 && in_shift == 0 && n_in == n_out && bnf->fuse.partial && bnf->y && bnf->ldy >= cin &&
+                   sgnn_conv_bn_fold_grid(n_out, cin, cout, K) > 0 && n_out * bnf->ldy * 4 <= 0xFFFFF000ll);
+  }
   const ConvEx ex{kmap, kadd, in_mul, groups, table_rows};
   const unsigned grid4 = (unsigned)((n_out + CONV_ROWS_PER_BLOCK - 1) / CONV_ROWS_PER_BLOCK) * (unsigned)groups;
   const unsigned grid1 = (unsigned)((n_out + 63) / 64) * (unsigned)groups;
@@ -542,6 +625,14 @@
   const int prof = sgnn_prof_begin_launch(0, n_out * groups, cin, cout, K, flags, s);
 #define LAUNCH_FWD(CI, CO, EXV)                                                                         \
   do {                                                                                                  \
+    if constexpr (!EXV && CI <= BN_FUSE_MAXC) {                                                         \
+      if (bnf) {                                                                                        \
+        SGNN_LAUNCH((k_conv_small_bn<CI, CO>), dim3((unsigned)((n_out + 15) / 16)), dim3(256), 0, s,    \
+                    x, n_in, w, table, ld, K, n_out, y, flags, in_shift, epi, *bnf);                    \
+        done = true;                                                                                    \
+        break;                                                                                          \
+      }                                                                                                 \
+    }                                                                                                   \
     if (small && !EXV && K <= 28 && (g_tune.conv_small || epi.stats))                                      \
       SGNN_LAUNCH((k_conv_small<CI, CO>), dim3((unsigned)((n_out + 15) / 16)), dim3(256), 0, s,         \
                          x, n_in, w, table, ld, K, n_out, y, flags, in_shift, epi);                     \
@@ -552,7 +643,7 @@
       conv_launch_big<CI, CO, EXV>(grid4, s, x, n_in, w, table, ld, K, n_out, y, flags, in_shift, ex, epi); \
     done = true;                                                                                        \
   } while (0)
-  if (plain && !small && g_tune.conv_unrolled && sgnn_conv_u_supported(cin, cout, K))
+  if (!bnf && plain && !small && g_tune.conv_unrolled && sgnn_conv_u_supported(cin, cout, K))
     done = sgnn_conv_u_launch(x, n_in, cin, w, K, table, ld, n_out, cout, y, flags, in_shift, epi, s);
 #define X(CI, CO) \
   if (!done && plain && cin == CI && cout == CO) LAUNCH_FWD(CI, CO, false);
diff --git a/sgnn_amd/csrc/prog.hip b/sgnn_amd/csrc/prog.hip
--- a/sgnn_amd/csrc/prog.hip
+++ b/sgnn_amd/csrc/prog.hip
@@ -1,6 +1,7 @@
 #include <mutex>
 #include <vector>
 #include "common.h"
+#include "bn_fuse.h"
 
 enum {
   OP_CONV_SUBM = 0, OP_CONV_DOWN = 1, OP_UNPOOL = 2, OP_BN = 3, OP_ADD = 4, OP_JOIN = 5,
@@ -403,7 +404,7 @@
   return (need + 255) & ~int64_t(255);
 }
 
-int64_t ws_need(const View &v) { return ws_main(v) + ws_stats(v); }
+int64_t ws_need(const View &v) { return ws_main(v) + (g_tune.prog_bn_conv_fold ? 2 : 1) * ws_stats(v); }
 
 struct SideLane {
   hipStream_t stream = nullptr;
@@ -431,7 +432,8 @@
   Layout L;
   std::vector<const double *> pre;
   std::vector<int64_t> pre_nblk;
-  double *stats_ws;
+  double *stats_ws, *stats_ws2;
+  std::vector<ConvBnFold> fold;
 
   bool prepare(Kind kind, const int32_t *keep) {
     make_plan(v, keep, P, kind);
@@ -439,7 +441,15 @@
     pre = std::vector<const double *>(v.nops, nullptr);
     pre_nblk = std::vector<int64_t>(v.nops, 0);
     stats_ws = (double *)((char *)ws + ws_main(v));
+    stats_ws2 = g_tune.prog_bn_conv_fold ? (double *)((char *)stats_ws + ws_stats(v)) : nullptr;
+    fold = std::vector<ConvBnFold>(v.nops, ConvBnFold{});
     return true;
+  }
+  int64_t bn_conv_fold_grid(int i, const float *x, const float *y) const {
+    if (!g_tune.prog_bn_conv_fold || !g_fuse || !training || P.kind != TRAINING || i + 1 >= v.nops || !stats_ws2) return 0;
+    const Op &o = v.op(i), &cv = v.op(i + 1);
+    if (cv.type != OP_CONV_SUBM || cv.in0 != o.out || cv.lev != o.lev || cv.cin != o.cin || P.skip[i + 1] || x == y) return 0;
+    return sgnn_conv_bn_fold_grid(v.lev_n[o.lev], cv.cin, cv.cout, cv.K());
   }
   int ch(int b) const { return b < 0 ? 0 : v.bufs[2 * b + 1]; }
   int cls(int b) const { return v.bufs[2 * b]; }
@@ -671,19 +681,21 @@
           epi.ld_add = c.ld(PL.add_src[i]);
           dst_buf = PL.add_dst[i];
         }
+        const ConvBnFold *bnf = c.fold[i].fuse.partial ? &c.fold[i] : nullptr;
+        const int src = bnf ? v.op(i - 1).in0 : in0;
         const int j = i + 1 + (PL.add_dst[i] >= 0 ? 1 : 0);
         if (g_fuse && training && cs.n_out > 0 && j < nops && v.op(j).type == OP_BN && v.op(j).in0 == dst_buf &&
             sgnn_conv_epi_supported(cin, cout)) {
           epi.stats = 1;
-          epi.partial = c.stats_ws;
-          c.pre[j] = c.stats_ws;
+          epi.partial = (bnf && bnf->fuse.partial == c.stats_ws) ? c.stats_ws2 : c.stats_ws;
+          c.pre[j] = epi.partial;
           c.pre_nblk[j] = sgnn_conv_grid_blocks(cs.n_out, cin, cout, cs.K);
         }
-        epi.ldx = c.ld(in0);
+        epi.ldx = c.ld(src);
         epi.ldy = c.ld(dst_buf);
         epi.n_dev = c.count(cs.cnt_class);
-        PROG_TRY(sgnn_conv_fwd_impl(B(in0), n, cin, c.param(par), cs.K, cs.tab_f, cs.ld_f, cs.n_out, cout, B(dst_buf), 0, 0,
-                                    nullptr, nullptr, 1, 1, cs.K, &epi, stream));
+        PROG_TRY(sgnn_conv_fwd_impl(B(src), n, cin, c.param(par), cs.K, cs.tab_f, cs.ld_f, cs.n_out, cout, B(dst_buf), 0, 0,
+                                    nullptr, nullptr, 1, 1, cs.K, &epi, stream, bnf));
         break;
       }
       case OP_UNPOOL:
@@ -693,9 +705,11 @@
         break;
       case OP_BN: {
         float *save = arena + L.aux_off[i];
+        const int64_t fold_grid = c.bn_conv_fold_grid(i, B(in0), B(out));
         PROG_TRY(sgnn_bn_fwd_impl(B(in0), c.ld(in0), n, cin, c.param(par), c.param(par + 1), c.param(par + 2), c.param(par + 3),
                                   opf[4 * i], opf[4 * i + 1], training, opf[4 * i + 2], save, save + cin, B(out), c.ld(out),
-                                  c.pre[i], c.pre_nblk[i], ws, ws_bytes, stream, c.count(lev)));
+                                  c.pre[i], c.pre_nblk[i], ws, ws_bytes, stream, c.count(lev),
+                                  fold_grid > 0 ? &c.fold[i + 1] : nullptr, fold_grid));
         break;
       }
       case OP_ADD:
diff --git a/sgnn_amd/csrc/tune.hip b/sgnn_amd/csrc/tune.hip
--- a/sgnn_amd/csrc/tune.hip
+++ b/sgnn_amd/csrc/tune.hip
@@ -8,6 +8,7 @@
      1,
      1,
      256,
+     1,
      1,
      1,
      1,
@@ -40,6 +41,7 @@
     {"prog_lin_bn", &sgnn_tune::prog_lin_bn, 0, 1, true},
     {"prog_lin_add", &sgnn_tune::prog_lin_add, 0, 1, true},
     {"bn_fuse", &sgnn_tune::bn_fuse, 0, 1, true},
+    {"prog_bn_conv_fold", &sgnn_tune::prog_bn_conv_fold, 0, 1, true},
 };
 const Field *find(const char *name) {
   if (!name) return nullptr;
```
